# yangao07/LAMSA

Hardware: AMD Instinct MI355X
Metric: aligned Gbase/s, 10 kbp ONT-error reads (12%: sub/ins/del 4% each), -T ont2d vs GRCh37-sized stand-in; inputs resident in HBM when the timed region starts (upload excluded: see pcie_inclusive_*) (higher is better)
Workload: dtype int32

## Files before the change

### lamsa_amd/csrc/hp_align_api.hip

```cpp
#include <hip/hip_runtime.h>
#include <algorithm>
#include <atomic>
#include <map>
#include <mutex>
#include <stdlib.h>
#include <string.h>
#include <time.h>
#include "hp_phase.h"
#include "hp_handle.h"
#include "hp_hostprep.h"

using namespace hp;

#ifndef HP_WAVES_PER_SIMD
#define HP_WAVES_PER_SIMD 4
#endif
__global__ __launch_bounds__(64, HP_WAVES_PER_SIMD) void k_align_batch(AlignArgs a)
{
    __shared__ int32_t lds[HP_BOTH_LDS_WORDS];
    const int slot = blockIdx.x;
    for (;;) {
        int u = 0;
        if (wv::leader()) u = atomicAdd(a.counter, 1);
        u = wv::uni(u);
        if (u >= a.n_units) break;
        align_read(a, a.order ? a.order[u] : u, slot, (HP_L int32_t *)lds);
    }
}

#ifndef HP_CHAIN_WAVES_PER_SIMD
#define HP_CHAIN_WAVES_PER_SIMD 4
#endif
#ifndef HP_FILL_WAVES_PER_SIMD
#define HP_FILL_WAVES_PER_SIMD 7
#endif
template <int WORDS, int WPS>
__global__ __launch_bounds__(64, WPS) void k_chain1(const PhaseArgs *ap)
{
    const PhaseArgs &a = *ap;
    constexpr bool ctx_lds = ph_ctx_in_lds(WORDS, WPS);
    __shared__ alignas(16) int32_t lds[WORDS + (ctx_lds ? PH_CTX_BYTES / 4 : 0)];
    ReadCtx &r = *(ctx_lds ? (ReadCtx *)(lds + WORDS) : (ReadCtx *)(a.slab + (size_t)blockIdx.x * a.slab_per_wave));
    for (;;) {
        int u = 0;
        if (wv::leader()) u = atomicAdd(&a.ctl->q_head[0], 1);
        u = wv::uni(u);
        if (u >= a.n_reads) break;
        phase_chain1(a, a.order ? a.order[u] : u, blockIdx.x, (HP_L int32_t *)lds, WORDS, r);
    }
    drain_stamp(a, 0);
}
template <int WORDS, int WPS>
__global__ __launch_bounds__(64, WPS) void k_chain2(const PhaseArgs *ap)
{
    const PhaseArgs &a = *ap;
    constexpr bool ctx_lds = ph_ctx_in_lds(WORDS, WPS);
    __shared__ alignas(16) int32_t lds[WORDS + (ctx_lds ? PH_CTX_BYTES / 4 : 0)];
    ReadCtx &r = *(ctx_lds ? (ReadCtx *)(lds + WORDS) : (ReadCtx *)(a.slab + (size_t)blockIdx.x * a.slab_per_wave));
    for (;;) {
        int u = 0;
        if (wv::leader()) u = atomicAdd(&a.ctl->q_head[2], 1);
        u = wv::uni(u);
        if (u >= a.n_reads) break;
        phase_chain2(a, a.order ? a.order[u] : u, blockIdx.x, (HP_L int32_t *)lds, WORDS, r);
    }
    drain_stamp(a, 2);
}
typedef void (*ChainKernel)(const PhaseArgs *);
struct ChainShape { ChainKernel k1, k2; int lds_words, waves_per_simd; };
static const ChainShape g_chain_shapes[3] = {
    {k_chain1<HP_CHAIN_LDS_WORDS, HP_CHAIN_WAVES_PER_SIMD>, k_chain2<HP_CHAIN_LDS_WORDS, HP_CHAIN_WAVES_PER_SIMD>, HP_CHAIN_LDS_WORDS, HP_CHAIN_WAVES_PER_SIMD},
    {k_chain1<3392, 3>, k_chain2<3392, 3>, 3392, 3},
    {k_chain1<5120, 2>, k_chain2<5120, 2>, 5120, 2},
};
__global__ __launch_bounds__(64, HP_FILL_WAVES_PER_SIMD) void k_fill(const PhaseArgs *ap, int round)
{
    const PhaseArgs &a = *ap;
    __shared__ alignas(16) int32_t lds[HP_LDS_WORDS + PH_CTX_BYTES / 4];
    ReadCtx &r = *(ReadCtx *)(lds + HP_LDS_WORDS);
    int n = 0;
    for (int b = 0; b < PH_NBUCKET; ++b) n += a.ctl->bucket_n[round][b];
    n = wv::uni(n);
    for (;;) {
        int g = 0;
        if (wv::leader()) g = atomicAdd(&a.ctl->q_head[1 + 2 * round], 1);
        g = wv::uni(g);
        if (g >= n) break;
        int b = 0;
        while (b < PH_NBUCKET - 1 && g >= a.ctl->bucket_n[round][b]) { g -= a.ctl->bucket_n[round][b]; ++b; }
        const int u = wv::uni(a.bucket_q[((size_t)round * PH_NBUCKET + b) * a.unit_cap + g]);
        phase_fill(a, round, u, blockIdx.x, (HP_L int32_t *)lds, r);
    }
    drain_stamp(a, 1 + 2 * round);
}
#ifndef HP_FILLDP_WAVES_PER_SIMD
#define HP_FILLDP_WAVES_PER_SIMD 2
#endif
#ifndef HP_LIST_WAVES_PER_SIMD
#define HP_LIST_WAVES_PER_SIMD 4
#endif
__global__ __launch_bounds__(64, HP_LIST_WAVES_PER_SIMD) void k_filllist(const PhaseArgs *ap, int round)
{
    const PhaseArgs &a = *ap;
    __shared__ alignas(16) int32_t lds[PH_CTX_BYTES / 4];
    ReadCtx &r = *(ReadCtx *)lds;
    int n = 0;
    for (int b = 0; b < PH_NBUCKET; ++b) n += a.ctl->bucket_n[round][b];
    n = wv::uni(n);
    for (;;) {
        int g = 0;
        if (wv::leader()) g = atomicAdd(&a.ctl->q_head[5], 1);
        g = wv::uni(g);
        if (g >= n) break;
        int b = 0;
        while (b < PH_NBUCKET - 1 && g >= a.ctl->bucket_n[round][b]) { g -= a.ctl->bucket_n[round][b]; ++b; }
        const int u = wv::uni(a.bucket_q[((size_t)round * PH_NBUCKET + b) * a.unit_cap + g]);
        phase_filllist(a, round, u, blockIdx.x, (HP_L int32_t *)lds, r);
    }
}
__global__ __launch_bounds__(64, 2) void k_filldp_small(const PhaseArgs *ap, int round)
{
    __shared__ int32_t lds[HP_LJ_LDS_WORDS(HP_LJ_QSMALL)];
    const PhaseArgs &a = *ap;
    int n = 0;
    for (int b = 0; b < LJ_NBUCKET; ++b) n += (lj_queue_n(a, round, b) + 63) >> 6;
    n = wv::uni(n);
    for (;;) {
        int g = 0;
        if (wv::leader()) g = atomicAdd(&a.ctl->q_head[6], 1);
        g = wv::uni(g);
        if (g >= n) break;
        int b = 0;
        for (; b < LJ_NBUCKET - 1; ++b) { const int gb = (lj_queue_n(a, round, b) + 63) >> 6; if (g < gb) break; g -= gb; }
        phase_filldp(a, round, b, g * 64, blockIdx.x, (HP_L int32_t *)lds, HP_LJ_QSMALL);
    }
}
__global__ __launch_bounds__(64, HP_WJ_WAVES_PER_SIMD) void k_filldp_wave(const PhaseArgs *ap, int round)
{
    __shared__ int32_t lds[HP_WJ_LDS_WORDS];
    const PhaseArgs &a = *ap;
    int n = 0, n_big = 0;
    for (int b = 0; b < WJ_NBUCKET; ++b) { const int k = wj_queue_n(a, round, b); if (b < WJ_NBIG) n_big += k; else n += k; }
    n = wv::uni(n); n_big = wv::uni(n_big);
    bool own_big = (int)blockIdx.x < a.n_wjb;
    for (;;) {
        int g = 0;
        const bool big = own_big;
        if (wv::leader()) g = atomicAdd(&a.ctl->q_head[big ? 8 : 7], 1);
        g = wv::uni(g);
        if (g >= (big ? n_big : n)) { if (!big) break; own_big = false; continue; }
        phase_wavejob(a, round, g, big, blockIdx.x, (HP_L int32_t *)lds);
    }
}
__global__ __launch_bounds__(64) void k_publish(const PhaseArgs *ap)
{
    const PhaseArgs &a = *ap;
    if (blockIdx.x == 0) publish_diag(a);
    for (;;) {
        int u = 0;
        if (wv::leader()) u = atomicAdd(&a.ctl->q_head[4], 1);
        u = wv::uni(u);
        if (u >= a.n_reads) break;
        phase_publish(a, u);
    }
}

__global__ void k_cig8_expand(const uint8_t *src, int32_t *dst, int64_t n)
{
    for (int64_t i = (int64_t)blockIdx.x * blockDim.x + threadIdx.x; i < n; i += (int64_t)gridDim.x * blockDim.x) { const int b = src[i]; dst[i] = ((b & 63) << 4) | (b >> 6); }
}
__global__ void k_off_widen(const int32_t *src, int64_t *dst, int64_t n)
{
    for (int64_t i = (int64_t)blockIdx.x * blockDim.x + threadIdx.x; i < n; i += (int64_t)gridDim.x * blockDim.x) dst[i] = src[i];
}
#define HP_SCAN_BLOCK 4096
__global__ __launch_bounds__(256) void k_scan_sums(const uint8_t *src, int64_t n, int64_t *sums)
{
    __shared__ int part[256];
    const int64_t b0 = (int64_t)blockIdx.x * HP_SCAN_BLOCK;
    int s = 0;
    for (int i = threadIdx.x; i < HP_SCAN_BLOCK; i += 256) { const int64_t k = b0 + i; s += k < n ? src[k] : 0; }
    part[threadIdx.x] = s;
    __syncthreads();
    for (int st = 128; st > 0; st >>= 1) { if ((int)threadIdx.x < st) part[threadIdx.x] += part[threadIdx.x + st]; __syncthreads(); }
    if (threadIdx.x == 0) sums[blockIdx.x] = part[0];
}
__global__ __launch_bounds__(256) void k_scan_bases(int64_t *sums, int64_t nb)
{
    __shared__ long long tot[256];
    const int64_t per = (nb + 255) / 256, a = (int64_t)threadIdx.x * per, b = a + per < nb ? a + per : nb;
    long long s = 0;
    for (int64_t i = a; i < b; ++i) s += sums[i];
    tot[threadIdx.x] = s;
    __syncthreads();
    if (threadIdx.x == 0) { long long run = 0; for (int t = 0; t < 256; ++t) { const long long v = tot[t]; tot[t] = run; run += v; } }
    __syncthreads();
    long long run = tot[threadIdx.x];
    for (int64_t i = a; i < b; ++i) { const long long v = sums[i]; sums[i] = run; run += v; }
}
__global__ __launch_bounds__(256) void k_scan_apply(const uint8_t *src, int64_t n, const int64_t *bases, int64_t *dst)
{
    __shared__ int part[256];
    const int64_t b0 = (int64_t)blockIdx.x * HP_SCAN_BLOCK + (int64_t)threadIdx.x * 16;
    int v[16], s = 0;
#pragma unroll
    for (int i = 0; i < 16; ++i) { const int64_t k = b0 + i; v[i] = k < n ? src[k] : 0; s += v[i]; }
    part[threadIdx.x] = s;
    __syncthreads();
    if (threadIdx.x == 0) { int run = 0; for (int t = 0; t < 256; ++t) { const int x = part[t]; part[t] = run; run += x; } }
    __syncthreads();
    long long run = bases[blockIdx.x] + part[threadIdx.x];
#pragma unroll
    for (int i = 0; i < 16; ++i) { const int64_t k = b0 + i; if (k < n) dst[k] = run; run += v[i]; }
}

static double now_s() { timespec t; clock_gettime(CLOCK_MONOTONIC, &t); return t.tv_sec + 1e-9 * t.tv_nsec; }
static const bool g_trace = getenv("LAMSA_HP_TRACE") != nullptr;
static const bool g_noshare = getenv("LAMSA_HP_FULL_GRIDS") != nullptr;
static const bool g_nowave = getenv("LAMSA_HP_NO_WAVE_JOBS") != nullptr;
static const bool g_nolane = getenv("LAMSA_HP_NO_LANE_DP") != nullptr;
static const bool g_mono = getenv("LAMSA_HP_ONE_KERNEL") != nullptr;

struct HostBuf {
    void *p = nullptr, *dev = nullptr; size_t cap = 0;
    int ensure(size_t bytes) {
        if (bytes <= cap) return 0;
        if (p) hipHostFree(p);
        p = dev = nullptr; cap = 0;
        size_t want = bytes + bytes / 4 + 256;
        if (hipHostMalloc(&p, want, hipHostMallocMapped) != hipSuccess) { p = nullptr; return -1; }
        if (hipHostGetDevicePointer(&dev, p, 0) != hipSuccess) { hipHostFree(p); p = nullptr; return -1; }
        cap = want;
        return 0;
    }
    void release() { if (p) hipHostFree(p); p = dev = nullptr; cap = 0; }
};

struct OutDev {
    DevBuf buf; HostBuf host; int64_t stream_cap = 0; int n_cap = 0;
    static size_t hdr(int n) { return al256(8 * (size_t)n) + 3 * al256(4 * (size_t)n) + 256 + al256(16 * (size_t)n); }
    int ensure(int n, int64_t cap) { stream_cap = cap; n_cap = n; return buf.ensure(4 * (size_t)cap + 256) || host.ensure(hdr(n) + 256); }
    int64_t *off() const { return (int64_t *)host.dev; }
    int32_t *len(int n) const { return (int32_t *)((char *)host.dev + al256(8 * (size_t)n)); }
    int32_t *st(int n) const { return (int32_t *)((char *)host.dev + al256(8 * (size_t)n) + al256(4 * (size_t)n)); }
    int32_t *tb(int n) const { return (int32_t *)((char *)host.dev + al256(8 * (size_t)n) + 2 * al256(4 * (size_t)n)); }
    unsigned long long *diag(int n) const { return (unsigned long long *)((char *)host.dev + al256(8 * (size_t)n) + 3 * al256(4 * (size_t)n)); }
    const unsigned long long *h_diag(int n) const { return (const unsigned long long *)((const char *)host.p + al256(8 * (size_t)n) + 3 * al256(4 * (size_t)n)); }
    int32_t *work(int n) const { return (int32_t *)((char *)host.dev + al256(8 * (size_t)n) + 3 * al256(4 * (size_t)n) + 256); }
    const int32_t *h_work(int n) const { return (const int32_t *)((const char *)host.p + al256(8 * (size_t)n) + 3 * al256(4 * (size_t)n) + 256); }
    const int64_t *h_off() const { return (const int64_t *)host.p; }
    const int32_t *h_len(int n) const { return (const int32_t *)((const char *)host.p + al256(8 * (size_t)n)); }
    const int32_t *h_st(int n) const { return (const int32_t *)((const char *)host.p + al256(8 * (size_t)n) + al256(4 * (size_t)n)); }
    const int32_t *h_tb(int n) const { return (const int32_t *)((const char *)host.p + al256(8 * (size_t)n) + 2 * al256(4 * (size_t)n)); }
    int32_t *stream(int) const { return (int32_t *)buf.p; }
    void release() { buf.release(); host.release(); }
};

struct Slot {
    DevBuf bin, misc, slab, pers, prof; OutDev out1;
    HostBuf args_host;
    hipEvent_t ep[7] = {nullptr, nullptr, nullptr, nullptr, nullptr, nullptr, nullptr};
    hipStream_t cs = nullptr;
    bool valid = false;
    bool phased = false;
    int32_t n_reads = 0; int64_t n_bases = 0, n_cig = 0, n_hits = 0;
    BatchIn in; const int32_t *d_order = nullptr;
    std::vector<int32_t> order, h_len, h_H; std::vector<uint8_t> h_skip;
    int32_t max_L = 0, max_H = 0;
    int32_t sort_pb = 40, sort_cb = 24;
    hipEvent_t e0 = nullptr, e1 = nullptr;
};

struct AlignState {
    Slot slot[2];
    int fifo[2] = {0, 0}, n_fifo = 0;
    int res_fifo[2] = {0, 0}, n_res = 0;
    DevBuf retry_list;
    OutDev out2;
    HostBuf stream;
    std::vector<int32_t> r_len, r_st, r_tb, r_work; std::vector<int64_t> r_off;
};

static std::map<lamsa_hp_handle *, AlignState *> g_states;
static std::mutex g_states_lock;
static AlignState *state_of(lamsa_hp_handle *h)
{
    std::lock_guard<std::mutex> guard(g_states_lock);
    auto it = g_states.find(h);
    if (it != g_states.end()) return it->second;
    return g_states[h] = new AlignState();
}
extern "C" void lamsa_hp_release_state_(lamsa_hp_handle *h)
{
    AlignState *S = nullptr;
    {
        std::lock_guard<std::mutex> guard(g_states_lock);
        auto it = g_states.find(h);
        if (it == g_states.end()) return;
        S = it->second;
        g_states.erase(it);
    }
    if (h->stream) hipStreamSynchronize(h->stream);
    if (h->stream_b) hipStreamSynchronize(h->stream_b);
    for (Slot &T : S->slot) { T.bin.release(); T.misc.release(); T.slab.release(); T.pers.release(); T.prof.release(); T.args_host.release(); T.out1.release(); for (hipEvent_t e : {T.e0, T.e1, T.ep[0], T.ep[1], T.ep[2], T.ep[3], T.ep[4], T.ep[5], T.ep[6]}) if (e) hipEventDestroy(e); }
    S->retry_list.release(); S->out2.release(); S->stream.release();
    delete S;
}

static int grow(lamsa_hp_handle *h, DevBuf &b, size_t bytes)
{
    if (bytes <= b.cap) return 0;
    if (hipStreamSynchronize(h->stream) != hipSuccess || hipStreamSynchronize(h->stream_b) != hipSuccess) return -1;
    return b.ensure(bytes);
}


static int upload_into(lamsa_hp_handle *h, Slot *S, const lamsa_hp_batch *B)
{
    S->valid = false;
    const double t_0 = now_s();
    const int n = B->n_reads;
    const int64_t n_slots = n ? B->seed_off[n] : 0, n_hits = n_slots ? B->hit_off[n_slots] : 0, n_bases = n ? B->read_off[n] : 0;
    S->h_len.assign((size_t)n, 0); S->h_H.assign((size_t)n, 0); S->h_skip.assign((size_t)n + 1, 0); S->max_L = 0; S->max_H = 0;
    if (n && (B->seed_off[0] != 0 || B->read_off[0] != 0 || (n_slots && B->hit_off[0] != 0))) { h->err = "offsets must start at 0"; return LAMSA_HP_EINVAL; }
    const bool packed_off = B->h_cig_off == nullptr, cig_bytes = B->cig8 != nullptr;
    if (B->n_cig < 0 || (!packed_off && B->n_cig > 0x7fffffffll)) { h->err = "more than 2^31-1 seed CIGAR elements with 32-bit h_cig_off: pass h_cig_off = NULL (CIGARs back to back in hit order) or split the batch"; return LAMSA_HP_EINVAL; }
    if (!cig_bytes && !B->cig && B->n_cig > 0) { h->err = "neither cig nor cig8 given"; return LAMSA_HP_EINVAL; }
    {
        std::atomic<int> bad(0);
        const int64_t sl = h->para.seed_len, ss = h->para.seed_step > 0 ? h->para.seed_step : 1;
        std::atomic<long long> max_pos(0), sum_cig(0);
        hp_parallel_blocks(n, [&](int r0, int r1) {
            long long mp = 0, sc = 0;
            for (int r = r0; r < r1 && !bad.load(std::memory_order_relaxed); ++r) {
                const int64_t L = B->read_off[r + 1] - B->read_off[r], ns = B->seed_off[r + 1] - B->seed_off[r];
                if (L < 0 || L > (1 << 24) || ns < 0) { bad = 1; return; }
                if (ns > HP_MAX_SLOTS) S->h_skip[r] = 1;
                {
                    const int64_t sa = L < sl ? 0 : 1 + (L - sl) / ss;
                    if (B->seed_all[r] != sa || B->last_len[r] != L - sl - (sa - 1) * ss) { bad = 7; return; }
                    if (sa > 32767) S->h_skip[r] = 1;
                }
                int64_t H = 0;
                for (int64_t s = B->seed_off[r]; s < B->seed_off[r + 1]; ++s) {
                    const int64_t m = B->hit_off[s + 1] - B->hit_off[s];
                    if (m < 0 || (m > HP_MAX_HITS_PER_SEED && !S->h_skip[r])) { bad = 2; return; }
                    if (B->seed_id[s] < 1 || B->seed_id[s] > B->seed_all[r] || (s > B->seed_off[r] && B->seed_id[s] <= B->seed_id[s - 1])) { bad = 3; return; }
                    H += m;
                }
                if (H > (1 << 22) && !S->h_skip[r]) { bad = 4; return; }
                for (int64_t i = B->read_off[r]; i < B->read_off[r + 1]; ++i) if (B->read_seq[i] > 4) { bad = 5; return; }
                for (int64_t k = B->hit_off[B->seed_off[r]]; k < B->hit_off[B->seed_off[r + 1]]; ++k) {
                    mp = B->h_pos[k] > mp ? B->h_pos[k] : mp;
                    if (B->h_len_dif[k] < -127 || B->h_len_dif[k] > 127) S->h_skip[r] = 1;
                    if (B->h_chr[k] < 1 || B->h_chr[k] > h->n_seqs || (B->h_strand[k] != 1 && B->h_strand[k] != -1) || B->h_pos[k] < 0 || B->h_pos[k] >= (1ll << 40) ||
                        (!packed_off && (B->h_cig_off[k] < 0 || (int64_t)B->h_cig_off[k] + B->h_cig_n[k] > B->n_cig))) { bad = 6; return; }
                    sc += B->h_cig_n[k];
                }
                S->h_len[r] = (int32_t)L; S->h_H[r] = (int32_t)H;
            }
            long long seen = max_pos.load();
            while (mp > seen && !max_pos.compare_exchange_weak(seen, mp)) { }
            sum_cig += sc;
        });
        static const char *why[] = {"", "read longer than 2^24 bases", "too many hits in one seed", "seed ids must be ascending in [1, seed_all]",
                                    "too many hits in one read", "read base code > 4",
                                    "bad hit record (contig id, strand, position or seed CIGAR range)",
                                    "seed_all / last_len do not match the read length and the handle's seed length and step"};
        if (bad) { h->err = why[bad.load()]; return LAMSA_HP_EINVAL; }
        if (packed_off && sum_cig.load() != B->n_cig) { h->err = "h_cig_off is NULL but the h_cig_n do not add up to n_cig"; return LAMSA_HP_EINVAL; }
        for (int r = 0; r < n; ++r) { if (S->h_skip[r]) { S->h_len[r] = 0; S->h_H[r] = 0; } S->max_L = std::max(S->max_L, S->h_len[r]); S->max_H = std::max(S->max_H, S->h_H[r]); }
        auto bits = [](unsigned long long x) { int b = 0; while (x) { ++b; x >>= 1; } return b; };
        S->sort_pb = bits((unsigned long long)max_pos.load()); S->sort_cb = bits((unsigned long long)(2 * (long long)h->n_seqs + 1));
    }
    const double t_1 = now_s();
    S->order.resize((size_t)n);
    for (int r = 0; r < n; ++r) S->order[r] = r;
    {
        std::vector<double> cost((size_t)n);
        for (int r = 0; r < n; ++r) cost[r] = (double)S->h_H[r] * S->h_H[r] / 64.0 + (double)S->h_len[r] * (2.0 * h->para.band_w + 1) / 16.0;
        std::stable_sort(S->order.begin(), S->order.end(), [&](int x, int y) { return cost[x] > cost[y]; });
    }
    size_t off = 0;
    auto place = [&](size_t bytes) { size_t o = off; off = al256(off + bytes + 16); return o; };
    const size_t o_roff = place(8 * ((size_t)n + 1)), o_rseq = place((size_t)n_bases), o_sall = place(4 * (size_t)n), o_last = place(4 * (size_t)n),
                 o_soff = place(8 * ((size_t)n + 1)), o_sid = place(4 * (size_t)n_slots), o_hoff = place(8 * ((size_t)n_slots + 1)),
                 o_pos = place(8 * (size_t)n_hits), o_chr = place(4 * (size_t)n_hits), o_coff = place(8 * (size_t)n_hits), o_nm = place(2 * (size_t)n_hits),
                 o_ld = place(2 * (size_t)n_hits), o_st = place((size_t)n_hits), o_cn = place((size_t)n_hits), o_cig = place(4 * (size_t)B->n_cig), o_ord = place(4 * (size_t)n),
                 o_stage = place(packed_off ? 8 * ((size_t)n_hits / HP_SCAN_BLOCK + 2) : 4 * (size_t)n_hits), o_cig8 = place(cig_bytes ? (size_t)B->n_cig : 0), o_skip = place((size_t)n);
    const double t_3 = now_s();
    if (S->bin.ensure(off)) { h->err = "hipMalloc(batch)"; return LAMSA_HP_ENOMEM; }
    char *d = (char *)S->bin.p;
    hipStream_t s = h->copy_stream;
    static const int64_t zero64 = 0;
#define UP(o, src, bytes) do { if ((bytes) > 0) HIPCHK(h, hipMemcpyAsync(d + (o), (src), (bytes), hipMemcpyHostToDevice, s), LAMSA_HP_EKERNEL); } while (0)
    if (n) { UP(o_roff, B->read_off, 8 * ((size_t)n + 1)); UP(o_soff, B->seed_off, 8 * ((size_t)n + 1)); }
    else { UP(o_roff, &zero64, 8); UP(o_soff, &zero64, 8); }
    UP(o_rseq, B->read_seq, (size_t)n_bases); UP(o_sall, B->seed_all, 4 * (size_t)n); UP(o_last, B->last_len, 4 * (size_t)n);
    UP(o_sid, B->seed_id, 4 * (size_t)n_slots);
    if (n_slots) UP(o_hoff, B->hit_off, 8 * ((size_t)n_slots + 1)); else UP(o_hoff, &zero64, 8);
    UP(o_pos, B->h_pos, 8 * (size_t)n_hits); UP(o_chr, B->h_chr, 4 * (size_t)n_hits);
    if (!packed_off) UP(o_stage, B->h_cig_off, 4 * (size_t)n_hits);
    UP(o_nm, B->h_nm, 2 * (size_t)n_hits); UP(o_ld, B->h_len_dif, 2 * (size_t)n_hits); UP(o_st, B->h_strand, (size_t)n_hits); UP(o_cn, B->h_cig_n, (size_t)n_hits);
    if (cig_bytes) UP(o_cig8, B->cig8, (size_t)B->n_cig); else UP(o_cig, B->cig, 4 * (size_t)B->n_cig);
    UP(o_ord, S->order.data(), 4 * (size_t)n); UP(o_skip, S->h_skip.data(), (size_t)n);
#undef UP
    if (cig_bytes && B->n_cig > 0) hipLaunchKernelGGL(k_cig8_expand, dim3(2048), dim3(256), 0, s, (const uint8_t *)(d + o_cig8), (int32_t *)(d + o_cig), (int64_t)B->n_cig);
    if (n_hits > 0) {
        if (!packed_off) hipLaunchKernelGGL(k_off_widen, dim3(2048), dim3(256), 0, s, (const int32_t *)(d + o_stage), (int64_t *)(d + o_coff), (int64_t)n_hits);
        else {
            const int64_t nb = (n_hits + HP_SCAN_BLOCK - 1) / HP_SCAN_BLOCK;
            hipLaunchKernelGGL(k_scan_sums, dim3((unsigned)nb), dim3(256), 0, s, (const uint8_t *)(d + o_cn), (int64_t)n_hits, (int64_t *)(d + o_stage));
            hipLaunchKernelGGL(k_scan_bases, dim3(1), dim3(256), 0, s, (int64_t *)(d + o_stage), nb);
            hipLaunchKernelGGL(k_scan_apply, dim3((unsigned)nb), dim3(256), 0, s, (const uint8_t *)(d + o_cn), (int64_t)n_hits, (const int64_t *)(d + o_stage), (int64_t *)(d + o_coff));
        }
    }
    HIPCHK(h, hipGetLastError(), LAMSA_HP_EKERNEL);
    HIPCHK(h, hipStreamSynchronize(s), LAMSA_HP_EKERNEL);
    if (g_trace) fprintf(stderr, "[lamsa_hp] upload: validate %.1f ms, order %.1f ms, copy %.1f ms (%.2f GB on the device)\n", 1e3 * (t_1 - t_0), 1e3 * (t_3 - t_1), 1e3 * (now_s() - t_3), off / 1e9);
    BatchIn &in = S->in;
    in.n_reads = n; in.read_skip = (const uint8_t *)(d + o_skip); in.read_off = (const int64_t *)(d + o_roff); in.read_seq = (const uint8_t *)(d + o_rseq);
    in.seed_all = (const int32_t *)(d + o_sall); in.last_len = (const int32_t *)(d + o_last); in.seed_off = (const int64_t *)(d + o_soff);
    in.seed_id = (const int32_t *)(d + o_sid); in.hit_off = (const int64_t *)(d + o_hoff); in.h_pos = (const int64_t *)(d + o_pos);
    in.h_chr = (const int32_t *)(d + o_chr); in.h_cig_off = (const int64_t *)(d + o_coff); in.h_nm = (const int16_t *)(d + o_nm);
    in.h_len_dif = (const int16_t *)(d + o_ld); in.h_strand = (const int8_t *)(d + o_st); in.h_cig_n = (const uint8_t *)(d + o_cn);
    in.cig = (const int32_t *)(d + o_cig);
    S->d_order = (const int32_t *)(d + o_ord);
    S->n_reads = n; S->n_bases = n_bases; S->n_cig = B->n_cig; S->n_hits = n_hits;
    S->valid = true;
    return LAMSA_HP_OK;
}

static int cap_waves(int n_waves, size_t slab_per_wave, int n_cu)
{
    static const size_t budget = []() { size_t f = 0, t = 0; if (hipMemGetInfo(&f, &t) != hipSuccess || t == 0) { t = (size_t)288 << 30; f = t; } return std::min(t / 4, f / 3); }();
    if (slab_per_wave * (size_t)n_waves <= budget) return n_waves;
    size_t fit = budget / (slab_per_wave ? slab_per_wave : 1);
    if (n_cu > 0 && fit >= (size_t)n_cu) fit -= fit % (size_t)n_cu;
    return fit < 1 ? 1 : (int)fit;
}

#ifdef HP_PROF
static void prof_report(Slot &T, const long long *d_prof, int n)
{
    if (!d_prof) return;
    {
        std::vector<long long> pr((size_t)n * 64);
        hipMemcpy(pr.data(), d_prof, sizeof(long long) * pr.size(), hipMemcpyDeviceToHost);
        if (const char *dump = getenv("LAMSA_HP_PROF_DUMP")) {
            if (FILE *fp = fopen(dump, "wb")) {
                for (int r = 0; r < n; ++r) { long long hl[2] = {T.h_H[r], T.h_len[r]}; fwrite(hl, 8, 2, fp); fwrite(&pr[(size_t)r * 64], 8, 64, fp); }
                fclose(fp);
            }
        }
        std::vector<int> idx((size_t)n); for (int i = 0; i < n; ++i) idx[i] = i;
        auto tot = [&](int r) { long long t = 0; for (int k = 0; k < 6; ++k) t += pr[(size_t)r * 64 + k]; return t; };
        std::sort(idx.begin(), idx.end(), [&](int x, int y) { return tot(x) > tot(y); });
        long long sum[64] = {0}; for (int r = 0; r < n; ++r) for (int k = 0; k < 64; ++k) sum[k] += pr[(size_t)r * 64 + k];
        fprintf(stderr, "[HP_PROF] cycles: setup chain1 fill1 chain2 fill2 publish | in chain1: init+minext mainscan track pop-loop bound+flines | o_l H\n");
        fprintf(stderr, "[HP_PROF] SUM  "); for (int k = 0; k < 11; ++k) fprintf(stderr, " %lld", sum[k] / 1000000); fprintf(stderr, " (Mcycles) targets %lld trips %lld init_Mcyc %lld\n", sum[11], sum[12], sum[13] / 1000000);
#ifdef HP_PROF_TRACK
        fprintf(stderr, "[HP_PROF] branch tracking (-DHP_PROF_TRACK: the line_build stamps below are off): marking pass, image build and write-back %lld Mcyc; %lld seeds visited; %lld tracks, %lld Mcyc in them, %lld steps up; "
                        "%lld arrivals at a node with several sons, %lld Mcyc in cut_branch\n", sum[16] / 1000000, sum[19], sum[18], sum[17] / 1000000, sum[20], sum[21], sum[22] / 1000000);
#endif
#ifdef HP_PROF_EDGE
        fprintf(stderr, "[HP_PROF] main pass (-DHP_PROF_EDGE: the line_build stamps below are off), Mcyc: dp_cluster_lds load+pack %lld, MIN extension %lld, target loop %lld, write-back %lld; cluster_lane %lld; build_sons %lld\n",
                sum[16] / 1000000, sum[17] / 1000000, sum[18] / 1000000, sum[19] / 1000000, sum[20] / 1000000, sum[21] / 1000000);
#else
        fprintf(stderr, "[HP_PROF] line_build: %lld lines (%lld without a gap), %lld anchors, %lld gaps | Mcyc: anchor walk %lld, gap list %lld, gaps in lanes %lld, gaps one by one %lld, assembly %lld\n",
                sum[21], sum[22], sum[12], sum[23], sum[16] / 1000000, sum[17] / 1000000, sum[18] / 1000000, sum[19] / 1000000, sum[20] / 1000000);
#endif
        fprintf(stderr, "[HP_PROF] gaps: %lld in lines with fewer than HP_GAP_MIN gaps (%lld lines with gaps); lane gaps: %lld hits scanned, %lld refused (range too long or too many active hits)\n", sum[54], sum[55], sum[11], sum[13]);
        { const char *nm[] = {"ksw_global", "ksw_extend", "backtrack", "ref_fetch", "head_fix", "frag_extend", "split_mapping", "tail_fix", "res_split", "res_aux", "mini_line_regs", "sort index"};
          for (int k = 0; k < 12; ++k) fprintf(stderr, "[HP_PROF] %-16s %8lld Mcyc %10lld calls\n", nm[k], sum[24 + 2 * k] / 1000000, sum[25 + 2 * k]);
#ifdef HP_PROF_FILL
          fprintf(stderr, "[HP_PROF] in frags_merge: boundary repair (merge_cigar_full) %lld Mcyc %lld calls; junctions through split_mapping %lld Mcyc %lld calls; fragments of several seeds %lld Mcyc %lld calls; 64-step gathers %lld Mcyc %lld\n", sum[16] / 1000000, sum[17], sum[18] / 1000000, sum[19], sum[20] / 1000000, sum[21], sum[22] / 1000000, sum[23]);
#endif
          fprintf(stderr, "[HP_PROF] direction-matrix bytes in HBM %lld (%lld jobs); hits passed through nodes_per_init %lld (%lld calls)\n", sum[52], sum[53], sum[54], sum[55]);
          fprintf(stderr, "[HP_PROF] chain_first start: seed loop %lld, node_set loop %lld, min_extend %lld Mcyc (%lld reads with a MIN pass)\n", sum[56] / 1000000, sum[57] / 1000000, sum[58] / 1000000, sum[59]);
          fprintf(stderr, "[HP_PROF] query <= 62: ksw_extend %lld Mcyc %lld calls, ksw_global %lld Mcyc %lld calls\n", sum[60] / 1000000, sum[61], sum[62] / 1000000, sum[63]);
          const char *bn[] = {"[bi_extend total]", "[bi_extend after left ext]", "17-32", "33-64", "65-128", "129-256", "257-512", ">512"};
          for (int k = 0; k < 2; ++k) fprintf(stderr, "[HP_PROF] ksw_extend qlen %-8s %8lld Mcyc %10lld calls\n", bn[k], sum[48 + 2 * k] / 1000000, sum[49 + 2 * k]); }
        {
            std::vector<long long> pd((size_t)n * 64);
            hipMemcpy(pd.data(), d_prof + ((size_t)n + 1) * 64, sizeof(long long) * pd.size(), hipMemcpyDeviceToHost);
            long long sd[64] = {0}; for (int r = 0; r < n; ++r) for (int k = 0; k < 64; ++k) sd[k] += pd[(size_t)r * 64 + k];
            const char *cn[] = {"one set, q <= 62", "packed, one set", "packed, two sets", "band 1 set slides", "band 2 sets slides", "band 4 sets slides", "int32 sets", "LDS / HBM rows",
                                "band 1 set fixed", "band 2 sets fixed", "band 4 sets fixed"};
            for (int c = 0; c < 11; ++c) fprintf(stderr, "[HP_PROF] wave jobs, ksw_extend %-18s %8lld Mcyc %10lld Mcells %9lld calls %10lld rows\n", cn[c], sd[4 * c] / 1000000, sd[4 * c + 1] / 1000000, sd[4 * c + 2], sd[4 * c + 3]);
            fprintf(stderr, "[HP_PROF] wave jobs, junctions of the class 'band 2 sets fixed': %lld jobs, wj_run %lld Mcyc of which staging %lld; ksw_bi_extend %lld Mcyc of which after the left extension %lld; "
                            "in ksw_extend_band<2>: setup and first fill %lld, rows %lld, backtrack %lld Mcyc\n",
                    sd[51], sd[50] / 1000000, sd[49] / 1000000, sd[47] / 1000000, sd[48] / 1000000, sd[44] / 1000000, sd[45] / 1000000, sd[46] / 1000000);
        }
        for (int q = 0; q < 8 && q < n; ++q) { int r = idx[q]; fprintf(stderr, "[HP_PROF] read %d L=%d:", r, T.h_len[r]); for (int k = 0; k < 11; ++k) fprintf(stderr, " %lld", pr[(size_t)r * 64 + k] / 1000000); fprintf(stderr, " | o_l %lld H %lld | targets %lld trips %lld init_Mcyc %lld\n", pr[(size_t)r * 64 + 14], pr[(size_t)r * 64 + 15], pr[(size_t)r * 64 + 11], pr[(size_t)r * 64 + 12], pr[(size_t)r * 64 + 13] / 1000000); }
    }
}
#endif

struct PhasedLayout { size_t bytes, o[15]; int unit_cap, lj_cap, wj_cap; int64_t fl_cap, line_cap, job_cap; };
static PhasedLayout phased_layout(int n, int64_t n_hits, int64_t n_bases, int64_t stream_cap)
{
    PhasedLayout Y;
    const size_t n_ent = (size_t)n_hits + (size_t)n + 1;
    Y.unit_cap = 8 * n + 1024;
    Y.fl_cap = 4 * n_hits + 2304 * (int64_t)n + 4096; Y.line_cap = stream_cap + 64 * (int64_t)Y.unit_cap;
    Y.job_cap = std::min<int64_t>(0x7fffff00ll, 4096 + 256 * (int64_t)n + 2 * n_bases);
    Y.lj_cap = (int)std::min<int64_t>(0x3fffffffll, 1024 + 16 * (int64_t)n + n_bases / 100);
    Y.wj_cap = (int)std::min<int64_t>(0x3fffffffll, 1024 + 32 * (int64_t)n + n_bases / 200);
    size_t off = 0;
    auto place = [&](size_t bytes) { size_t o = off; off = al256(off + bytes + 16); return o; };
    const size_t sz[15] = {sizeof(PhaseArgs), sizeof(PhaseCtl), sizeof(RdMeta) * ((size_t)n + 1), sizeof(NodeS) * n_ent, 4 * n_ent, 8 * n_ent, sizeof(UnitRec) * 2 * (size_t)Y.unit_cap,
                           4 * 2 * (size_t)PH_NBUCKET * Y.unit_cap, 4 * (size_t)Y.fl_cap, 4 * (size_t)Y.line_cap, 4 * (size_t)Y.job_cap, sizeof(LjRec) * (size_t)Y.lj_cap, 4 * (size_t)LJ_NBUCKET * Y.lj_cap,
                           sizeof(WjRec) * (size_t)Y.wj_cap, 4 * (size_t)WJ_NBUCKET * Y.wj_cap};
    for (int k = 0; k < 15; ++k) Y.o[k] = place(sz[k]);
    Y.bytes = off;
    return Y;
}

struct SlabPlan { size_t chain, fill, wj, wjb, wjb_off; int w_chain, w_fill, w_dp, w_wj, n_wjb, shape; size_t bytes; };
static int chain_shape(const lamsa_hp_para &P, int64_t n_reads, int64_t n_bases)
{
    static const int force = getenv("LAMSA_HP_CHAIN_SHAPE") ? atoi(getenv("LAMSA_HP_CHAIN_SHAPE")) : -1;
    if (force >= 0 && force < 3) return force;
    const int64_t mean_L = n_reads > 0 ? n_bases / n_reads : 0, ss = P.seed_step > 0 ? P.seed_step : 1;
    const int64_t est = mean_L / ss * 2 / 3;
    for (int k = 0; k < 2; ++k) if (est <= g_chain_shapes[k].lds_words / 5) return k;
    return 2;
}
static SlabPlan slab_plan(lamsa_hp_handle *h, int max_L, int max_H, bool shared = false, int shape = 0)
{
    SlabPlan Q;
    Q.shape = shape;
    const lamsa_hp_para &P = h->para;
    Q.chain = al256(((size_t)256 << 10) + 128 * (size_t)max_L + 424 * (size_t)max_H);
    Q.fill = al256(fill_slab_bytes(max_L, h->result_tags, sizeof(cig_t) * 3 * HP_LJ_CIG * 64 + (size_t)HP_LJ_QSMALL * HP_LJ_TSMALL * 64 + 64));
    { static const int kb = getenv("LAMSA_HP_WJ_SLAB_KB") ? atoi(getenv("LAMSA_HP_WJ_SLAB_KB")) : 0;
      Q.wj = ((size_t)(kb > 0 ? kb : 1024) << 10) + 33 * 256; }
    Q.wjb = al256((size_t)wj_need(&P, WJ_HEAD, max_L, max_L + 2 * P.hash_step + 64) + ((size_t)64 << 10)) + 33 * 256;
    if (Q.wjb < Q.wj) Q.wjb = Q.wj;
    if (g_nowave) Q.fill = std::max(Q.fill, al256(read_slab_bytes(P.band_w, max_L, max_H, 1, h->result_tags)));
    if (h->scratch_limit) { const size_t lim = al256(h->scratch_limit); Q.chain = std::min(Q.chain, lim); Q.fill = std::min(Q.fill, lim); Q.wj = std::min(Q.wj, lim); Q.wjb = std::min(Q.wjb, lim); }
    int pc = 0, pf = 0, pd = 0, pw = 0;
    if (hipOccupancyMaxActiveBlocksPerMultiprocessor(&pc, g_chain_shapes[shape].k1, 64, 0) != hipSuccess || pc < 1) pc = 4 * g_chain_shapes[shape].waves_per_simd;
    if (hipOccupancyMaxActiveBlocksPerMultiprocessor(&pf, k_fill, 64, 0) != hipSuccess || pf < 1) pf = 4;
    if (hipOccupancyMaxActiveBlocksPerMultiprocessor(&pd, k_filldp_small, 64, 0) != hipSuccess || pd < 1) pd = 4;
    if (hipOccupancyMaxActiveBlocksPerMultiprocessor(&pw, k_filldp_wave, 64, 0) != hipSuccess || pw < 1) pw = 4;
    if (shared && !g_noshare) { pc = std::min(pc, 8); pf = std::min(pf, 16); pw = std::min(pw, 16); }
    { static const int cf = getenv("LAMSA_HP_FILL_PER_CU") ? atoi(getenv("LAMSA_HP_FILL_PER_CU")) : 0, cc = getenv("LAMSA_HP_CHAIN_PER_CU") ? atoi(getenv("LAMSA_HP_CHAIN_PER_CU")) : 0,
                       cw = getenv("LAMSA_HP_WJ_PER_CU") ? atoi(getenv("LAMSA_HP_WJ_PER_CU")) : 0;
      if (cf > 0 && cf < pf) pf = cf;
      if (cc > 0 && cc < pc) pc = cc;
      if (cw > 0 && cw < pw) pw = cw; }
    Q.w_chain = cap_waves(h->n_cu * pc, Q.chain, h->n_cu); Q.w_fill = cap_waves(h->n_cu * pf, Q.fill, h->n_cu);
    Q.w_dp = std::min(h->n_cu * pd, Q.w_fill); Q.w_wj = cap_waves(h->n_cu * pw, Q.wj, h->n_cu);
    { const size_t budget_big = (size_t)12 << 30; size_t nb = budget_big / Q.wjb; if (nb < 1) nb = 1; Q.n_wjb = (int)std::min<size_t>(nb, (size_t)Q.w_wj); }
    Q.wjb_off = al256(Q.wj * (size_t)Q.w_wj);
    const size_t wj_bytes = Q.wjb_off + Q.wjb * (size_t)Q.n_wjb;
    Q.bytes = std::max(std::max(Q.chain * (size_t)Q.w_chain, Q.fill * (size_t)Q.w_fill), wj_bytes);
    return Q;
}

static int launch_phased(lamsa_hp_handle *h, AlignState *S, Slot &T, Slot &Ln, OutDev &O, hipEvent_t e0, hipEvent_t e1)
{
    const int n = T.n_reads;
    const int64_t n_hits = T.n_hits;
    const SlabPlan Q = slab_plan(h, T.max_L, T.max_H, S->n_fifo + S->n_res > 0, chain_shape(h->para, T.n_reads, T.n_bases));
    const int w_chain = Q.w_chain, w_fill = Q.w_fill, w_dp = Q.w_dp, w_wj = Q.w_wj;
    const PhasedLayout Y = phased_layout(n, n_hits, T.n_bases, O.stream_cap);
    const int unit_cap = Y.unit_cap, lj_cap = Y.lj_cap; const int64_t fl_cap = Y.fl_cap, line_cap = Y.line_cap, job_cap = Y.job_cap;
    const size_t off = Y.bytes, o_args = Y.o[0], o_ctl = Y.o[1], o_meta = Y.o[2], o_nd = Y.o[3], o_ns = Y.o[4], o_sx = Y.o[5], o_un = Y.o[6], o_bq = Y.o[7], o_fl = Y.o[8], o_ln = Y.o[9],
                 o_jb = Y.o[10], o_lj = Y.o[11], o_lq = Y.o[12], o_wj = Y.o[13], o_wq = Y.o[14];
    if (grow(h, Ln.slab, Q.bytes) || grow(h, Ln.pers, off) || Ln.misc.ensure(256)) { h->err = "hipMalloc(slab)"; return LAMSA_HP_ENOMEM; }
    char *d = (char *)Ln.pers.p;
    PhaseArgs a;
    a.P = h->para;
    a.ref.pac = h->d_pac; a.ref.l_pac = h->l_pac; a.ref.n_seqs = h->n_seqs; a.ref.seq_off = h->d_seq_off; a.ref.seq_len = h->d_seq_len;
    a.in = T.in; a.in.tags = h->result_tags;
    a.out.read_out_off = O.off(); a.out.read_out_len = O.len(n); a.out.read_status = O.st(n); a.out.read_tbases = O.tb(n); a.out.read_work = O.work(n); a.out.stream = O.stream(n);
    a.out.stream_cap = O.stream_cap; a.out.cursor = (unsigned long long *)((char *)Ln.misc.p + 64); a.out.diag = O.diag(n);
    a.slab = (char *)Ln.slab.p; a.slab_per_wave = Q.chain; a.slab_fill = Q.fill; a.slab_wj = Q.wj; a.slab_wjb = Q.wjb; a.wjb_off = Q.wjb_off; a.n_wjb = Q.n_wjb; a.sort_pb = T.sort_pb; a.sort_cb = T.sort_cb;
    a.order = T.d_order; a.n_reads = n; a.prof = nullptr;
#ifdef HP_PROF
    if (Ln.prof.ensure(sizeof(long long) * 64 * 2 * ((size_t)n + 1))) { h->err = "hipMalloc(prof)"; return LAMSA_HP_ENOMEM; }
    a.prof = (long long *)Ln.prof.p;
    HIPCHK(h, hipMemsetAsync(Ln.prof.p, 0, sizeof(long long) * 64 * 2 * ((size_t)n + 1), Ln.cs), LAMSA_HP_EKERNEL);
#endif
    a.g_nd = (NodeS *)(d + o_nd); a.g_nseed = (int32_t *)(d + o_ns); a.g_sidx = (int32_t *)(d + o_sx); a.meta = (RdMeta *)(d + o_meta);
    a.units = (UnitRec *)(d + o_un); a.unit_cap = unit_cap; a.bucket_q = (int32_t *)(d + o_bq);
    a.fl_base = (int32_t *)(d + o_fl); a.fl_cap = fl_cap; a.line_base = (int32_t *)(d + o_ln); a.line_cap = line_cap; a.ctl = (PhaseCtl *)(d + o_ctl);
    a.job_base = (int32_t *)(d + o_jb); a.job_cap = job_cap;
    a.ljobs = (LjRec *)(d + o_lj); a.lj_bucket = (int32_t *)(d + o_lq); a.lj_cap = g_nolane ? 0 : lj_cap;
    a.wjobs = (WjRec *)(d + o_wj); a.wj_bucket = (int32_t *)(d + o_wq); a.wj_cap = g_nowave ? 0 : Y.wj_cap;
    const bool list = !g_nolane || !g_nowave;
    hipStream_t s = Ln.cs;
    HIPCHK(h, hipMemsetAsync(Ln.misc.p, 0, 128, s), LAMSA_HP_EKERNEL);
    HIPCHK(h, hipMemsetAsync(d + o_ctl, 0, (o_meta - o_ctl) + sizeof(RdMeta) * ((size_t)n + 1), s), LAMSA_HP_EKERNEL);
    if (Ln.args_host.ensure(sizeof a)) { h->err = "hipHostMalloc(args)"; return LAMSA_HP_ENOMEM; }
    memcpy(Ln.args_host.p, &a, sizeof a);
    HIPCHK(h, hipMemcpyAsync(d + o_args, Ln.args_host.p, sizeof a, hipMemcpyHostToDevice, s), LAMSA_HP_EKERNEL);
    const PhaseArgs *da = (const PhaseArgs *)(d + o_args);
    HIPCHK(h, hipEventRecord(e0, s), LAMSA_HP_EKERNEL);
    hipLaunchKernelGGL(g_chain_shapes[Q.shape].k1, dim3(std::min(w_chain, n)), dim3(64), 0, s, da);
    HIPCHK(h, hipEventRecord(Ln.ep[0], s), LAMSA_HP_EKERNEL);
    if (list) {
        hipLaunchKernelGGL(k_filllist, dim3(w_fill), dim3(64), 0, s, da, 0);
        HIPCHK(h, hipEventRecord(Ln.ep[5], s), LAMSA_HP_EKERNEL);
        if (!g_nowave) hipLaunchKernelGGL(k_filldp_wave, dim3(w_wj), dim3(64), 0, s, da, 0);
        HIPCHK(h, hipEventRecord(Ln.ep[6], s), LAMSA_HP_EKERNEL);
        if (!g_nolane) hipLaunchKernelGGL(k_filldp_small, dim3(w_dp), dim3(64), 0, s, da, 0);
    } else { HIPCHK(h, hipEventRecord(Ln.ep[5], s), LAMSA_HP_EKERNEL); HIPCHK(h, hipEventRecord(Ln.ep[6], s), LAMSA_HP_EKERNEL); }
    HIPCHK(h, hipEventRecord(Ln.ep[4], s), LAMSA_HP_EKERNEL);
    hipLaunchKernelGGL(k_fill, dim3(w_fill), dim3(64), 0, s, da, 0);
    HIPCHK(h, hipEventRecord(Ln.ep[1], s), LAMSA_HP_EKERNEL);
    hipLaunchKernelGGL(g_chain_shapes[Q.shape].k2, dim3(std::min(w_chain, n)), dim3(64), 0, s, da);
    HIPCHK(h, hipEventRecord(Ln.ep[2], s), LAMSA_HP_EKERNEL);
    if (list) {
        HIPCHK(h, hipMemsetAsync(&((PhaseCtl *)(d + o_ctl))->q_head[5], 0, 16, s), LAMSA_HP_EKERNEL);
        hipLaunchKernelGGL(k_filllist, dim3(w_fill), dim3(64), 0, s, da, 1);
        if (!g_nowave) hipLaunchKernelGGL(k_filldp_wave, dim3(w_wj), dim3(64), 0, s, da, 1);
        if (!g_nolane) hipLaunchKernelGGL(k_filldp_small, dim3(w_dp), dim3(64), 0, s, da, 1);
    }
    hipLaunchKernelGGL(k_fill, dim3(w_fill), dim3(64), 0, s, da, 1);
    HIPCHK(h, hipEventRecord(Ln.ep[3], s), LAMSA_HP_EKERNEL);
    hipLaunchKernelGGL(k_publish, dim3(std::min(h->n_cu * 8, n)), dim3(64), 0, s, da);
    HIPCHK(h, hipGetLastError(), LAMSA_HP_EKERNEL);
    HIPCHK(h, hipEventRecord(e1, s), LAMSA_HP_EKERNEL);
    Ln.phased = true;
    return LAMSA_HP_OK;
}

static int launch_align(lamsa_hp_handle *h, AlignState *S, Slot &T, Slot &Ln, OutDev &O, const int32_t *d_order, int n_units, int scale, int max_L, int max_H,
                        hipEvent_t e0, hipEvent_t e1, bool wait)
{
    size_t slab_per_wave = al256(read_slab_bytes(h->para.band_w, max_L, max_H, scale, h->result_tags));
    if (scale == 1 && h->scratch_limit && slab_per_wave > h->scratch_limit) slab_per_wave = al256(h->scratch_limit);
    int per_cu = 0;
    if (hipOccupancyMaxActiveBlocksPerMultiprocessor(&per_cu, k_align_batch, 64, 0) != hipSuccess || per_cu < 1) per_cu = 4;
    int n_waves = h->n_cu * per_cu;
    if (n_waves > n_units) n_waves = n_units;
    n_waves = cap_waves(n_waves, slab_per_wave, h->n_cu);
    if (grow(h, Ln.slab, slab_per_wave * (size_t)n_waves) || Ln.misc.ensure(256)) { h->err = "hipMalloc(slab)"; return LAMSA_HP_ENOMEM; }
    const int n = T.n_reads;
    AlignArgs a;
    a.P = h->para;
    a.ref.pac = h->d_pac; a.ref.l_pac = h->l_pac; a.ref.n_seqs = h->n_seqs; a.ref.seq_off = h->d_seq_off; a.ref.seq_len = h->d_seq_len;
    a.in = T.in; a.in.tags = h->result_tags;
    a.out.read_out_off = O.off(); a.out.read_out_len = O.len(n); a.out.read_status = O.st(n); a.out.read_tbases = O.tb(n); a.out.read_work = O.work(n); a.out.stream = O.stream(n);
    a.out.stream_cap = O.stream_cap; a.out.cursor = (unsigned long long *)((char *)Ln.misc.p + 64); a.out.diag = nullptr;
    a.slab = (char *)Ln.slab.p; a.slab_per_wave = slab_per_wave; a.counter = (int32_t *)Ln.misc.p;
    a.order = d_order; a.n_units = n_units; a.scale = scale; a.prof = nullptr; a.sort_pb = T.sort_pb; a.sort_cb = T.sort_cb;
    hipStream_t s = Ln.cs;
    HIPCHK(h, hipMemsetAsync(Ln.misc.p, 0, 128, s), LAMSA_HP_EKERNEL);
    HIPCHK(h, hipEventRecord(e0, s), LAMSA_HP_EKERNEL);
    hipLaunchKernelGGL(k_align_batch, dim3(n_waves), dim3(64), 0, s, a);
    HIPCHK(h, hipGetLastError(), LAMSA_HP_EKERNEL);
    HIPCHK(h, hipEventRecord(e1, s), LAMSA_HP_EKERNEL);
    if (wait) HIPCHK(h, hipStreamSynchronize(s), LAMSA_HP_EKERNEL);
#ifdef HP_PROF
    prof_report(T, a.prof, n);
#endif
    return LAMSA_HP_OK;
}

static int slot_events(lamsa_hp_handle *h, Slot &Ln)
{
    Ln.cs = &Ln == &state_of(h)->slot[1] ? h->stream_b : h->stream;
    if (!Ln.e0) HIPCHK(h, hipEventCreate(&Ln.e0), LAMSA_HP_EKERNEL);
    if (!Ln.e1) HIPCHK(h, hipEventCreate(&Ln.e1), LAMSA_HP_EKERNEL);
    for (hipEvent_t &e : Ln.ep) if (!e) HIPCHK(h, hipEventCreate(&e), LAMSA_HP_EKERNEL);
    return LAMSA_HP_OK;
}

static int start_main(lamsa_hp_handle *h, AlignState *S, Slot &T, Slot &Ln)
{
    int rc = slot_events(h, Ln);
    if (rc) return rc;
    const int n = T.n_reads;
    if (n == 0) return LAMSA_HP_OK;
    if (Ln.out1.ensure(n, batch_out_cap(n, T.n_bases, h->result_tags))) { h->err = "hipMalloc(out)"; return LAMSA_HP_ENOMEM; }
    Ln.phased = false;
    if (!g_mono) return launch_phased(h, S, T, Ln, Ln.out1, Ln.e0, Ln.e1);
    return launch_align(h, S, T, Ln, Ln.out1, T.d_order, n, 1, T.max_L, T.max_H, Ln.e0, Ln.e1, false);
}

#define DL(dst, src, bytes) HIPCHK(h, hipMemcpyAsync((dst), (src), (bytes), hipMemcpyDeviceToHost, h->copy_stream), LAMSA_HP_EKERNEL)
#define DLSYNC() HIPCHK(h, hipStreamSynchronize(h->copy_stream), LAMSA_HP_EKERNEL)

static int finish_main(lamsa_hp_handle *h, AlignState *S, Slot &T, Slot &Ln, lamsa_hp_result *R)
{
    const int n = T.n_reads;
    for (float &v : h->kernel_ms) v = 0;
    S->r_st.assign((size_t)n + 1, 0); S->r_off.assign((size_t)n + 1, 0); S->r_len.assign((size_t)n + 1, 0); S->r_tb.assign((size_t)n + 1, 0); S->r_work.assign(4 * (size_t)n + 4, 0);
    if (S->stream.ensure(64)) { h->err = "hipHostMalloc(results)"; return LAMSA_HP_ENOMEM; }
    if (n == 0) {
        if (R) { R->stream = (const int32_t *)S->stream.p; R->stream_words = 0; R->read_off = S->r_off.data(); R->read_len = S->r_len.data(); R->read_status = S->r_st.data(); R->read_tbases = S->r_tb.data(); R->read_work = S->r_work.data(); }
        return LAMSA_HP_OK;
    }
    const double t_0 = now_s();
    HIPCHK(h, hipEventSynchronize(Ln.e1), LAMSA_HP_EKERNEL);
    const double t_1 = now_s();
    hipEventElapsedTime(&h->kernel_ms[0], Ln.e0, Ln.e1);
    if (Ln.phased) {
        hipEvent_t ev[6] = {Ln.e0, Ln.ep[0], Ln.ep[1], Ln.ep[2], Ln.ep[3], Ln.e1};
        for (int k = 0; k < 5; ++k) hipEventElapsedTime(&h->kernel_ms[2 + k], ev[k], ev[k + 1]);
        const unsigned long long *dg = Ln.out1.h_diag(n);
        for (int k = 0; k < 4; ++k) h->kernel_ms[7 + k] = dg[2 * k + 1] >= dg[2 * k] && dg[2 * k + 1] ? (float)((double)(dg[2 * k + 1] - dg[2 * k]) * 1e-5) : 0.f;
        h->kernel_ms[11] = (float)dg[8]; h->kernel_ms[12] = (float)dg[9];
        hipEventElapsedTime(&h->kernel_ms[13], Ln.ep[0], Ln.ep[4]);
        hipEventElapsedTime(&h->kernel_ms[14], Ln.ep[0], Ln.ep[5]);
        hipEventElapsedTime(&h->kernel_ms[15], Ln.ep[5], Ln.ep[6]);
        h->kernel_ms[16] = (float)dg[12]; h->kernel_ms[17] = (float)((double)dg[13] * 1e-6); h->kernel_ms[18] = (float)dg[14]; h->kernel_ms[19] = (float)((double)dg[15] * 4e-6); h->kernel_ms[20] = (float)((double)dg[16] * 1e-6);
#ifdef HP_PROF
        prof_report(T, (const long long *)Ln.prof.p, n);
#endif
    }
    memcpy(S->r_off.data(), Ln.out1.h_off(), 8 * (size_t)n); memcpy(S->r_len.data(), Ln.out1.h_len(n), 4 * (size_t)n);
    memcpy(S->r_st.data(), Ln.out1.h_st(n), 4 * (size_t)n); memcpy(S->r_tb.data(), Ln.out1.h_tb(n), 4 * (size_t)n); memcpy(S->r_work.data(), Ln.out1.h_work(n), 16 * (size_t)n);
    unsigned long long used1 = 0;
    for (int r = 0; r < n; ++r) if (S->r_off[r] >= 0 && (unsigned long long)(S->r_off[r] + S->r_len[r]) > used1) used1 = (unsigned long long)(S->r_off[r] + S->r_len[r]);
    if ((int64_t)used1 > Ln.out1.stream_cap) used1 = (unsigned long long)Ln.out1.stream_cap;
    std::vector<int32_t> again;
    for (int r = 0; r < n; ++r) if ((S->r_st[r] & LAMSA_HP_ST_OVERFLOW) || S->r_off[r] < 0) again.push_back(r);
#ifdef HP_CHAIN_STOP
    again.clear();
#endif
    unsigned long long used2 = 0;
    if (!again.empty()) {
        int mL = 0, mH = 0; int64_t cap2 = 1024;
        for (int r : again) { mL = std::max(mL, T.h_len[r]); mH = std::max(mH, T.h_H[r]); cap2 += read_out_cap(T.h_len[r], 8, h->result_tags); }
        if (grow(h, S->out2.buf, 4 * (size_t)cap2 + 256) || S->out2.host.ensure(OutDev::hdr(n) + 256) || grow(h, S->retry_list, 4 * again.size())) { h->err = "hipMalloc(retry)"; return LAMSA_HP_ENOMEM; }
        S->out2.stream_cap = cap2;
        HIPCHK(h, hipMemcpyAsync(S->retry_list.p, again.data(), 4 * again.size(), hipMemcpyHostToDevice, Ln.cs), LAMSA_HP_EKERNEL);
        int rc = launch_align(h, S, T, Ln, S->out2, (const int32_t *)S->retry_list.p, (int)again.size(), 8, mL, mH, h->ev0, h->ev1, true);
        if (rc) return rc;
        hipEventElapsedTime(&h->kernel_ms[1], h->ev0, h->ev1);
        const int64_t *off2 = S->out2.h_off(); const int32_t *len2 = S->out2.h_len(n), *st2 = S->out2.h_st(n), *tb2 = S->out2.h_tb(n), *wk2 = S->out2.h_work(n);
        for (int r : again) if (off2[r] >= 0 && (unsigned long long)(off2[r] + len2[r]) > used2) used2 = (unsigned long long)(off2[r] + len2[r]);
        if ((int64_t)used2 > cap2) used2 = (unsigned long long)cap2;
        for (int r : again) { S->r_st[r] = st2[r]; S->r_len[r] = len2[r]; S->r_tb[r] = tb2[r]; for (int q = 0; q < 4; ++q) S->r_work[4 * r + q] = wk2[4 * r + q]; S->r_off[r] = off2[r] < 0 ? -1 : (int64_t)used1 + off2[r]; }
    }
    for (int r = 0; r < n; ++r) if (S->r_off[r] < 0) { S->r_off[r] = 0; S->r_len[r] = 0; S->r_st[r] |= LAMSA_HP_ST_OVERFLOW; }
    if (!R) return LAMSA_HP_OK;
    if (S->stream.ensure(4 * (size_t)(used1 + used2) + 64)) { h->err = "hipHostMalloc(results)"; return LAMSA_HP_ENOMEM; }
    int32_t *hs = (int32_t *)S->stream.p;
    if (used1) DL(hs, Ln.out1.stream(n), 4 * (size_t)used1);
    if (used2) DL(hs + used1, S->out2.stream(n), 4 * (size_t)used2);
    DLSYNC();
    if (g_trace) fprintf(stderr, "[lamsa_hp] collect: waited %.1f ms for the kernel (%.1f ms), results %.1f ms (%.2f GB)\n", 1e3 * (t_1 - t_0), h->kernel_ms[0], 1e3 * (now_s() - t_1), 4e-9 * (double)(used1 + used2));
    R->stream = hs; R->stream_words = (int64_t)(used1 + used2); R->read_off = S->r_off.data(); R->read_len = S->r_len.data(); R->read_status = S->r_st.data(); R->read_tbases = S->r_tb.data(); R->read_work = S->r_work.data();
    return LAMSA_HP_OK;
}
#undef DL
#undef DLSYNC

static int check_batch_args(lamsa_hp_handle *h, const lamsa_hp_batch *B)
{
    if (!h || !B || B->n_reads < 0) return LAMSA_HP_EINVAL;
    if (!h->d_pac) { h->err = "handle was created without a reference"; return LAMSA_HP_EINVAL; }
    HIPCHK(h, hipSetDevice(h->device), LAMSA_HP_ENODEV);
    return LAMSA_HP_OK;
}

extern "C" int lamsa_hp_upload_batch(lamsa_hp_handle *h, const lamsa_hp_batch *B)
{
    int rc = check_batch_args(h, B);
    if (rc) return rc;
    AlignState *S = state_of(h);
    if (S->n_fifo || S->n_res) { h->err = "batches are in flight: collect them first"; return LAMSA_HP_EINVAL; }
    return upload_into(h, &S->slot[0], B);
}

extern "C" int lamsa_hp_run_uploaded(lamsa_hp_handle *h, lamsa_hp_result *R)
{
    if (!h) return LAMSA_HP_EINVAL;
    AlignState *S = state_of(h);
    if (S->n_fifo) { h->err = "submitted batches are in flight: collect them first"; return LAMSA_HP_EINVAL; }
    if (!S->slot[0].valid) { h->err = "no batch uploaded"; return LAMSA_HP_EINVAL; }
    HIPCHK(h, hipSetDevice(h->device), LAMSA_HP_ENODEV);
    if (S->n_res) { h->err = "runs of the resident batch are in flight: finish them first"; return LAMSA_HP_EINVAL; }
    int rc = start_main(h, S, S->slot[0], S->slot[0]);
    if (rc) return rc;
    return finish_main(h, S, S->slot[0], S->slot[0], R);
}

extern "C" int lamsa_hp_start_uploaded(lamsa_hp_handle *h)
{
    if (!h) return LAMSA_HP_EINVAL;
    AlignState *S = state_of(h);
    if (S->n_fifo) { h->err = "submitted batches are in flight: collect them first"; return LAMSA_HP_EINVAL; }
    if (!S->slot[0].valid) { h->err = "no batch uploaded"; return LAMSA_HP_EINVAL; }
    if (S->n_res >= 2) { h->err = "two runs are already in flight: finish one first"; return LAMSA_HP_EINVAL; }
    HIPCHK(h, hipSetDevice(h->device), LAMSA_HP_ENODEV);
    const int k = S->n_res == 1 ? 1 - S->res_fifo[0] : 0;
    S->slot[1].valid = false;
    const int rc = start_main(h, S, S->slot[0], S->slot[k]);
    if (rc) return rc;
    S->res_fifo[S->n_res++] = k;
    return LAMSA_HP_OK;
}

extern "C" int lamsa_hp_finish_uploaded(lamsa_hp_handle *h, lamsa_hp_result *R)
{
    if (!h) return LAMSA_HP_EINVAL;
    AlignState *S = state_of(h);
    if (S->n_res == 0) { h->err = "no run in flight"; return LAMSA_HP_EINVAL; }
    HIPCHK(h, hipSetDevice(h->device), LAMSA_HP_ENODEV);
    const int k = S->res_fifo[0];
    S->res_fifo[0] = S->res_fifo[1]; --S->n_res;
    return finish_main(h, S, S->slot[0], S->slot[k], R);
}

extern "C" int lamsa_hp_align_batch(lamsa_hp_handle *h, const lamsa_hp_batch *B, lamsa_hp_result *R)
{
    int rc = lamsa_hp_upload_batch(h, B);
    if (rc) return rc;
    return lamsa_hp_run_uploaded(h, R);
}

extern "C" int lamsa_hp_submit_batch(lamsa_hp_handle *h, const lamsa_hp_batch *B)
{
    int rc = check_batch_args(h, B);
    if (rc) return rc;
    AlignState *S = state_of(h);
    if (S->n_res) { h->err = "runs of the resident batch are in flight: finish them first"; return LAMSA_HP_EINVAL; }
    if (S->n_fifo >= 2) { h->err = "two batches are already in flight: collect one first"; return LAMSA_HP_EINVAL; }
    const int k = S->n_fifo == 1 ? 1 - S->fifo[0] : 0;
    rc = upload_into(h, &S->slot[k], B);
    if (rc) return rc;
    const double t_s = now_s();
    rc = start_main(h, S, S->slot[k], S->slot[k]);
    if (g_trace) fprintf(stderr, "[lamsa_hp] submit: launch queued in %.1f ms (scratch and output buffers are allocated on first use)\n", 1e3 * (now_s() - t_s));
    if (rc) { S->slot[k].valid = false; return rc; }
    S->fifo[S->n_fifo++] = k;
    return LAMSA_HP_OK;
}

extern "C" int lamsa_hp_collect_batch(lamsa_hp_handle *h, lamsa_hp_result *R)
{
    if (!h) return LAMSA_HP_EINVAL;
    AlignState *S = state_of(h);
    if (S->n_fifo == 0) { h->err = "no batch in flight"; return LAMSA_HP_EINVAL; }
    HIPCHK(h, hipSetDevice(h->device), LAMSA_HP_ENODEV);
    const int k = S->fifo[0];
    S->fifo[0] = S->fifo[1]; --S->n_fifo;
    const int rc = finish_main(h, S, S->slot[k], S->slot[k], R);
    S->slot[k].valid = false;
    return rc;
}

extern "C" void *lamsa_hp_host_alloc(size_t bytes)
{
    void *p = nullptr;
    if (hipHostMalloc(&p, bytes ? bytes : 1, hipHostMallocDefault) != hipSuccess) return nullptr;
    return p;
}
extern "C" void lamsa_hp_host_free(void *p) { if (p) hipHostFree(p); }

extern "C" int lamsa_hp_reserve(lamsa_hp_handle *h, int32_t n_reads, int64_t n_bases, int64_t n_hits, int64_t n_cig, int32_t max_read_len, int32_t max_hits_per_read)
{
    if (!h || n_reads < 0 || n_bases < 0 || n_hits < 0 || n_cig < 0) return LAMSA_HP_EINVAL;
    HIPCHK(h, hipSetDevice(h->device), LAMSA_HP_ENODEV);
    AlignState *S = state_of(h);
    if (S->n_fifo || S->n_res) { h->err = "batches are in flight"; return LAMSA_HP_EINVAL; }
    const SlabPlan Q = slab_plan(h, max_read_len, max_hits_per_read, false, chain_shape(h->para, n_reads, n_bases));
    const int64_t cap = batch_out_cap(n_reads, n_bases, h->result_tags);
    const PhasedLayout Y = phased_layout(n_reads, n_hits, n_bases, cap);
    const size_t in_bytes = (size_t)n_bases + 16 * (size_t)n_reads * 4 + 32 * ((size_t)n_hits + n_reads) + 8 * (size_t)n_hits + 5 * (size_t)n_cig + 64 * 256 + 4096;
    for (Slot &T : S->slot) {
        int rc = slot_events(h, T);
        if (rc) return rc;
        if (T.slab.ensure(Q.bytes) || T.pers.ensure(Y.bytes) || T.misc.ensure(256) || T.bin.ensure(in_bytes) || T.out1.ensure(n_reads, cap)) {
            for (Slot &U : S->slot) { U.slab.release(); U.pers.release(); U.bin.release(); U.out1.release(); }
            h->err = "hipMalloc(reserve)"; return LAMSA_HP_ENOMEM;
        }
    }
    return LAMSA_HP_OK;
}

extern "C" int lamsa_hp_set_scratch_limit(lamsa_hp_handle *h, size_t bytes)
{
    if (!h || (bytes && bytes < ((size_t)64 << 10))) return LAMSA_HP_EINVAL;
    h->scratch_limit = bytes;
    return LAMSA_HP_OK;
}

extern "C" int lamsa_hp_set_result_tags(lamsa_hp_handle *h, int flags)
{
    if (!h) return LAMSA_HP_EINVAL;
    if (!result_tags_valid(flags)) { h->err = "result tags: an unknown item, or LAMSA_HP_TAG_SUMMARY (no CIGAR is shipped) with an item that lists or splits"; return LAMSA_HP_EINVAL; }
    AlignState *S = state_of(h);
    if (S->n_fifo || S->n_res) { h->err = "batches are in flight: collect them first"; return LAMSA_HP_EINVAL; }
    h->result_tags = flags;
    return LAMSA_HP_OK;
}
```

### lamsa_amd/csrc/hp_api.hip

```cpp
#include <hip/hip_runtime.h>
#include <stdio.h>
#include <stdlib.h>
#include <string.h>
#include <math.h>
#include <vector>
#include <string>
#include "hp_dp_batch.h"
#include "hp_wavejob.h"

using namespace hp;

__global__ __launch_bounds__(64) void k_dp_batch(DpBatchArgs a)
{
    __shared__ int32_t lds[HP_LDS_WORDS];
    const int slot = blockIdx.x;
    for (;;) {
        int job = 0;
        if (wv::leader()) job = atomicAdd(a.counter, 1);
        job = wv::uni(job);
        if (job >= a.n_jobs) break;
        dp_run_job(a, job, slot, (HP_L int32_t *)lds);
    }
}

__global__ __launch_bounds__(64, 1) void k_dp_batch_lane(DpBatchArgs a, const uint8_t *pac, const int64_t *tk)
{
    __shared__ int32_t lds[HP_LJ_LDS_WORDS(HP_LJ_QCAP)];
    const lamsa_hp_para *P = &a.P;
    char *slab = a.slab + (size_t)blockIdx.x * a.slab_per_wave;
    cig_t *cbuf = (cig_t *)slab;
    uint8_t *zbuf = (uint8_t *)(slab + sizeof(cig_t) * 3 * HP_LJ_CIG * 64);
    for (;;) {
        int g = 0;
        if (wv::leader()) g = atomicAdd(a.counter, 1);
        g = wv::uni(g);
        if (g * 64 >= a.n_jobs) break;
        wv::sync();
        WAVE_FOR(l) {
            const int job = g * 64 + l;
            if (job < a.n_jobs) {
                LaneJob J;
                J.q = (const HP_G uint8_t *)(a.seq + a.q_off[job]); J.qs = 1; J.qcomp = 0; J.qlen = a.qlen[job]; J.pac = (const HP_G uint8_t *)pac; J.tk = tk[job]; J.ts = 1; J.tlen = a.tlen[job];
                J.z = (HP_G uint8_t *)zbuf; J.zl = l; J.zs = HP_LJ_QCAP; J.cells = 0; J.row = (HP_L int32_t *)lds + l; J.qrow = (HP_L uint8_t *)((HP_L int32_t *)lds + (HP_LJ_QCAP + 2) * 64) + l; J.rev = 0;
                lj_stage_query(J);
                LCig out, Lc, Rc;
                out.c = cbuf + (size_t)l * 3 * HP_LJ_CIG; out.n = 0; Lc.c = out.c + HP_LJ_CIG; Lc.n = 0; Rc.c = Lc.c + HP_LJ_CIG; Rc.n = 0;
                int sc = 0, qle = 0, tle = 0;
                const int kind = a.kind[job];
                if (kind == 4) sc = lj_global(P, J, P->del_gapo, P->del_gape, P->ins_gapo, P->ins_gape, a.w[job], &out);
                else if (kind == 5) sc = lj_extend(P, J, a.w[job], a.h0[job], &qle, &tle, &out);
                else sc = lj_bi_extend(P, J, a.h0[job], a.h0[job], Lc, Rc, out);
                a.score[job] = sc; a.qle[job] = qle; a.tle[job] = tle; a.status[job] = 0; a.cig_n[job] = out.n;
                cig_t *dst = a.cig + a.cig_cap_off[job];
                for (int k = 0; k < out.n; ++k) dst[k] = out.c[k];
            }
        }
        wv::sync();
    }
}
__global__ __launch_bounds__(64, HP_WJ_WAVES_PER_SIMD) void k_dp_batch_wave(DpBatchArgs a, const uint8_t *pac, const int64_t *tk)
{
    __shared__ int32_t lds[HP_WJ_LDS_WORDS];
    for (;;) {
        int job = 0;
        if (wv::leader()) job = atomicAdd(a.counter, 1);
        job = wv::uni(job);
        if (job >= a.n_jobs) break;
        Ctx cx;
        cx.P = &a.P; cx.lds = (HP_L int32_t *)lds; cx.lds_words = HP_WJ_LDS_WORDS; cx.status = 0; cx.n_cells = 0; cx.lds_epoch = 0; cx.prof = nullptr;
        arena_init(cx.tmp, a.slab + (size_t)blockIdx.x * a.slab_per_wave, a.slab_per_wave);
        const int type = wv::uni(a.kind[job]) - 7, qlen = wv::uni(a.qlen[job]), tlen = wv::uni(a.tlen[job]);
        const bool back = type == WJ_HEAD;
        CigV out; cig_bind(out, a.cig + a.cig_cap_off[job], (int)(a.cig_cap_off[job + 1] - a.cig_cap_off[job]));
        WjOut o;
        wj_run(cx, a.seq, pac, type, 0, a.q_off[job] + (back && qlen > 0 ? qlen - 1 : 0), back ? -1 : 1, qlen, tk[job] + (back && tlen > 0 ? tlen - 1 : 0), back ? -1 : 1, tlen,
               wv::uni(a.w[job]), wv::uni(a.h0[job]), out, o);
        if (wv::leader()) { a.score[job] = o.score; a.qle[job] = o.qle; a.tle[job] = o.tle; a.status[job] = cx.status; a.cig_n[job] = out.n; }
        wv::sync();
    }
}

#include "hp_handle.h"

#include "hp_para.h"

extern "C" int lamsa_hp_create(lamsa_hp_handle **out, const lamsa_hp_para *para, const lamsa_hp_ref *ref, int device_id)
{
    if (!out || !para) return LAMSA_HP_EINVAL;
    *out = nullptr;
    int n_dev = 0;
    if (hipGetDeviceCount(&n_dev) != hipSuccess || n_dev <= 0 || device_id < 0 || device_id >= n_dev) return LAMSA_HP_ENODEV;
    if (hipSetDevice(device_id) != hipSuccess) return LAMSA_HP_ENODEV;
    lamsa_hp_handle *h = new lamsa_hp_handle();
    h->device = device_id; h->para = *para;
    hipDeviceProp_t prop;
    if (hipGetDeviceProperties(&prop, device_id) == hipSuccess) h->n_cu = prop.multiProcessorCount;
    if (hipStreamCreateWithFlags(&h->stream, hipStreamNonBlocking) != hipSuccess || hipStreamCreateWithFlags(&h->copy_stream, hipStreamNonBlocking) != hipSuccess || hipStreamCreateWithFlags(&h->stream_b, hipStreamNonBlocking) != hipSuccess || hipEventCreate(&h->ev0) != hipSuccess || hipEventCreate(&h->ev1) != hipSuccess) { delete h; return LAMSA_HP_ENODEV; }
    if (ref && ref->pac) {
        size_t pb = (size_t)(ref->l_pac / 4 + 1);
        h->l_pac = ref->l_pac; h->n_seqs = ref->n_seqs;
        if (hipMalloc((void **)&h->d_pac, pb + 16) != hipSuccess ||
            hipMalloc((void **)&h->d_seq_off, sizeof(int64_t) * (size_t)(ref->n_seqs + 1)) != hipSuccess ||
            hipMalloc((void **)&h->d_seq_len, sizeof(int32_t) * (size_t)(ref->n_seqs + 1)) != hipSuccess) { lamsa_hp_destroy(h); return LAMSA_HP_ENOMEM; }
        hipMemcpy(h->d_pac, ref->pac, pb, hipMemcpyHostToDevice);
        hipMemcpy(h->d_seq_off, ref->seq_offset, sizeof(int64_t) * (size_t)ref->n_seqs, hipMemcpyHostToDevice);
        hipMemcpy(h->d_seq_len, ref->seq_len, sizeof(int32_t) * (size_t)ref->n_seqs, hipMemcpyHostToDevice);
    }
    *out = h;
    return LAMSA_HP_OK;
}

extern "C" void lamsa_hp_release_state_(lamsa_hp_handle *h);
extern "C" void lamsa_hp_destroy(lamsa_hp_handle *h)
{
    if (!h) return;
    hipSetDevice(h->device);
    lamsa_hp_release_state_(h);
    if (h->d_pac) hipFree(h->d_pac);
    if (h->d_seq_off) hipFree(h->d_seq_off);
    if (h->d_seq_len) hipFree(h->d_seq_len);
    h->in.release(); h->out.release(); h->slab.release(); h->misc.release(); h->pac2.release();
    if (h->ev0) hipEventDestroy(h->ev0);
    if (h->ev1) hipEventDestroy(h->ev1);
    if (h->stream) hipStreamDestroy(h->stream);
    if (h->copy_stream) hipStreamDestroy(h->copy_stream);
    if (h->stream_b) hipStreamDestroy(h->stream_b);
    delete h;
}

extern "C" const char *lamsa_hp_last_error(const lamsa_hp_handle *h) { return h ? h->err.c_str() : "null handle"; }
extern "C" float lamsa_hp_last_kernel_ms(const lamsa_hp_handle *h, int which) { return (h && which >= 0 && which < 24) ? h->kernel_ms[which] : -1.f; }


extern "C" int lamsa_hp_dp_batch(lamsa_hp_handle *h, const lamsa_hp_dp_jobs *J, lamsa_hp_dp_out *O)
{
    if (!h || !J || !O || J->n_jobs < 0) return LAMSA_HP_EINVAL;
    HIPCHK(h, hipSetDevice(h->device), LAMSA_HP_ENODEV);
    const int n = J->n_jobs;
    std::vector<int64_t> cap_off((size_t)n + 1, 0);
    size_t z_need = 4096;
    for (int i = 0; i < n; ++i) {
        int ql = J->qlen[i], tl = J->tlen[i];
        if (ql < 0) ql = 0;
        if (tl < 0) tl = 0;
        if (J->q_off[i] < 0 || J->t_off[i] < 0 || J->q_off[i] + ql > J->seq_bytes || J->t_off[i] + tl > J->seq_bytes) { h->err = "dp job sequence out of range"; return LAMSA_HP_EINVAL; }
        cap_off[i + 1] = cap_off[i] + ql + tl + (J->kind[i] >= 8 ? 72 : 8);
        size_t wmax = (size_t)(abs(ql - tl) + 3 > (J->kind[i] == 2 ? h->para.band_w : J->w[i]) ? abs(ql - tl) + 3 : (J->kind[i] == 2 ? h->para.band_w : J->w[i]));
        size_t ncol = (size_t)ql < 2 * wmax + 1 ? (size_t)ql : 2 * wmax + 1;
        if (ql <= HP_PK_QMAX(2) && ncol < 128) ncol = 128;
        size_t need = 2 * 4 * ((size_t)ql + 18) + 8 * ((size_t)tl + 17) + ncol * tl + 64 + 3 * 4 * ((size_t)ql + tl + 24) + 1024;
        if (need > z_need) z_need = need;
    }
    int cls = 0;
    std::vector<int32_t> kind_v;
    std::vector<uint8_t> pac; std::vector<int64_t> tkv;
    if (n > 0 && J->kind[0] >= 4) {
        cls = J->kind[0] >= 8 ? 2 : 1;
        for (int i = 0; i < n; ++i) {
            const int k = J->kind[i];
            if (k < 4 || k == 7 || k > 11 || (k >= 8) != (cls == 2)) { h->err = "dp batch mixes job classes"; return LAMSA_HP_EINVAL; }
            if (cls == 1 && (J->qlen[i] < 0 || J->qlen[i] > HP_LJ_QCAP || J->tlen[i] < 0 || J->tlen[i] > HP_LJ_TCAP || (k != 4 && J->h0[i] <= 0))) { h->err = "dp job beyond the lane routines' buffers"; return LAMSA_HP_EINVAL; }
            if (cls == 2 && (J->qlen[i] < 0 || J->tlen[i] < 0 || (k != 9 && J->h0[i] <= 0))) { h->err = "dp job with a negative length or without a start score"; return LAMSA_HP_EINVAL; }
        }
        if (cls == 1 && !lj_params_ok(&h->para)) {
            kind_v.assign(J->kind, J->kind + n);
            for (int i = 0; i < n; ++i) kind_v[i] -= 4;
            cls = 0;
        } else {
            int64_t tot = 0;
            for (int i = 0; i < n; ++i) tot += J->tlen[i];
            pac.assign((size_t)tot / 4 + 16, 0); tkv.assign((size_t)n + 1, 0);
            int64_t k = 0;
            for (int i = 0; i < n; ++i) {
                tkv[i] = k;
                for (int j = 0; j < J->tlen[i]; ++j, ++k) {
                    const uint8_t b = J->seq[J->t_off[i] + j];
                    if (b > 3) { h->err = "these routines read the target 2 bits per base: no N"; return LAMSA_HP_EINVAL; }
                    pac[(size_t)(k >> 2)] |= (uint8_t)(b << ((~k & 3) << 1));
                }
            }
            if (cls == 1) z_need = sizeof(cig_t) * 3 * HP_LJ_CIG * 64 + (size_t)HP_LJ_QCAP * HP_LJ_TCAP * 64 + 64;
        }
    }
    const int32_t *kind_src = kind_v.empty() ? J->kind : kind_v.data();
    size_t slab_per_wave = al256(z_need);
    int n_waves = h->n_cu * (cls == 1 ? 3 : (cls == 2 ? 16 : 8));
    if (cls == 2) {
        size_t zz = 4096;
        for (int i = 0; i < n; ++i) {
            const size_t ql = (size_t)J->qlen[i], tl = (size_t)J->tlen[i];
            const size_t wmax = std::max<size_t>((size_t)abs((int)ql - (int)tl) + 3, (size_t)std::max(J->w[i], h->para.band_w));
            const size_t ncol = std::max<size_t>(std::min(ql, 2 * wmax + 1), 256);
            zz = std::max(zz, 2 * (ql + tl + 64) + 2 * 4 * (ql + 18) + 8 * (tl + 17) + ncol * tl + 64 + 4 * 4 * (ql + tl + 72) + 4096);
        }
        slab_per_wave = al256(zz);
    }
    if (n_waves > n) n_waves = n > 0 ? n : 1;
    while (n_waves > 1 && slab_per_wave * (size_t)n_waves > ((size_t)64 << 30)) n_waves /= 2;

    size_t o_seq = 0, o_qoff = al256((size_t)J->seq_bytes + 16), o_toff = o_qoff + al256(8 * (size_t)n), o_cap = o_toff + al256(8 * (size_t)n),
           o_ql = o_cap + al256(8 * ((size_t)n + 1)), o_tl = o_ql + al256(4 * (size_t)n), o_kind = o_tl + al256(4 * (size_t)n),
           o_w = o_kind + al256(4 * (size_t)n), o_h0 = o_w + al256(4 * (size_t)n), in_bytes = o_h0 + al256(4 * (size_t)n);
    if (h->in.ensure(in_bytes)) { h->err = "hipMalloc(in)"; return LAMSA_HP_ENOMEM; }
    size_t o_score = 0, o_qle = al256(4 * (size_t)n), o_tle = 2 * o_qle, o_st = 3 * o_qle, o_cn = 4 * o_qle, o_cig = 5 * o_qle, out_bytes = o_cig + al256(4 * (size_t)cap_off[n] + 16);
    if (h->out.ensure(out_bytes)) { h->err = "hipMalloc(out)"; return LAMSA_HP_ENOMEM; }
    if (h->slab.ensure(slab_per_wave * (size_t)n_waves)) { h->err = "hipMalloc(slab)"; return LAMSA_HP_ENOMEM; }
    if (h->misc.ensure(256)) { h->err = "hipMalloc(misc)"; return LAMSA_HP_ENOMEM; }
    char *din = (char *)h->in.p, *dout = (char *)h->out.p;
    hipStream_t s = h->stream;
    if (n > 0) {
        HIPCHK(h, hipMemcpyAsync(din + o_seq, J->seq, (size_t)J->seq_bytes, hipMemcpyHostToDevice, s), LAMSA_HP_EKERNEL);
        HIPCHK(h, hipMemcpyAsync(din + o_qoff, J->q_off, 8 * (size_t)n, hipMemcpyHostToDevice, s), LAMSA_HP_EKERNEL);
        HIPCHK(h, hipMemcpyAsync(din + o_toff, J->t_off, 8 * (size_t)n, hipMemcpyHostToDevice, s), LAMSA_HP_EKERNEL);
        HIPCHK(h, hipMemcpyAsync(din + o_cap, cap_off.data(), 8 * ((size_t)n + 1), hipMemcpyHostToDevice, s), LAMSA_HP_EKERNEL);
        HIPCHK(h, hipMemcpyAsync(din + o_ql, J->qlen, 4 * (size_t)n, hipMemcpyHostToDevice, s), LAMSA_HP_EKERNEL);
        HIPCHK(h, hipMemcpyAsync(din + o_tl, J->tlen, 4 * (size_t)n, hipMemcpyHostToDevice, s), LAMSA_HP_EKERNEL);
        HIPCHK(h, hipMemcpyAsync(din + o_kind, kind_src, 4 * (size_t)n, hipMemcpyHostToDevice, s), LAMSA_HP_EKERNEL);
        HIPCHK(h, hipMemcpyAsync(din + o_w, J->w, 4 * (size_t)n, hipMemcpyHostToDevice, s), LAMSA_HP_EKERNEL);
        HIPCHK(h, hipMemcpyAsync(din + o_h0, J->h0, 4 * (size_t)n, hipMemcpyHostToDevice, s), LAMSA_HP_EKERNEL);
    }
    HIPCHK(h, hipMemsetAsync(h->misc.p, 0, 256, s), LAMSA_HP_EKERNEL);

    DpBatchArgs a;
    a.P = h->para; a.n_jobs = n;
    a.seq = (const uint8_t *)(din + o_seq); a.q_off = (const int64_t *)(din + o_qoff); a.t_off = (const int64_t *)(din + o_toff);
    a.qlen = (const int32_t *)(din + o_ql); a.tlen = (const int32_t *)(din + o_tl); a.kind = (const int32_t *)(din + o_kind);
    a.w = (const int32_t *)(din + o_w); a.h0 = (const int32_t *)(din + o_h0);
    a.score = (int32_t *)(dout + o_score); a.qle = (int32_t *)(dout + o_qle); a.tle = (int32_t *)(dout + o_tle);
    a.status = (int32_t *)(dout + o_st); a.cig_n = (int32_t *)(dout + o_cn);
    a.cig_cap_off = (const int64_t *)(din + o_cap); a.cig = (cig_t *)(dout + o_cig);
    a.slab = (char *)h->slab.p; a.slab_per_wave = slab_per_wave; a.counter = (int32_t *)h->misc.p;

    HIPCHK(h, hipEventRecord(h->ev0, s), LAMSA_HP_EKERNEL);
    if (n > 0 && cls == 0) hipLaunchKernelGGL(k_dp_batch, dim3(n_waves), dim3(64), 0, s, a);
    else if (n > 0) {
        const size_t pb = al256(pac.size()), tb = al256(8 * ((size_t)n + 1));
        if (h->pac2.ensure(pb + tb)) { h->err = "hipMalloc(pac)"; return LAMSA_HP_ENOMEM; }
        HIPCHK(h, hipMemcpy(h->pac2.p, pac.data(), pac.size(), hipMemcpyHostToDevice), LAMSA_HP_EKERNEL);
        HIPCHK(h, hipMemcpy((char *)h->pac2.p + pb, tkv.data(), 8 * ((size_t)n + 1), hipMemcpyHostToDevice), LAMSA_HP_EKERNEL);
        if (cls == 1) hipLaunchKernelGGL(k_dp_batch_lane, dim3(n_waves), dim3(64), 0, s, a, (const uint8_t *)h->pac2.p, (const int64_t *)((char *)h->pac2.p + pb));
        else hipLaunchKernelGGL(k_dp_batch_wave, dim3(n_waves), dim3(64), 0, s, a, (const uint8_t *)h->pac2.p, (const int64_t *)((char *)h->pac2.p + pb));
    }
    HIPCHK(h, hipGetLastError(), LAMSA_HP_EKERNEL);
    HIPCHK(h, hipEventRecord(h->ev1, s), LAMSA_HP_EKERNEL);

    h->h_score.assign((size_t)n, 0); h->h_qle.assign((size_t)n, 0); h->h_tle.assign((size_t)n, 0); h->h_status.assign((size_t)n, 0);
    std::vector<int32_t> cn((size_t)n, 0), raw((size_t)cap_off[n] + 4, 0);
    if (n > 0) {
        HIPCHK(h, hipMemcpyAsync(h->h_score.data(), dout + o_score, 4 * (size_t)n, hipMemcpyDeviceToHost, s), LAMSA_HP_EKERNEL);
        HIPCHK(h, hipMemcpyAsync(h->h_qle.data(), dout + o_qle, 4 * (size_t)n, hipMemcpyDeviceToHost, s), LAMSA_HP_EKERNEL);
        HIPCHK(h, hipMemcpyAsync(h->h_tle.data(), dout + o_tle, 4 * (size_t)n, hipMemcpyDeviceToHost, s), LAMSA_HP_EKERNEL);
        HIPCHK(h, hipMemcpyAsync(h->h_status.data(), dout + o_st, 4 * (size_t)n, hipMemcpyDeviceToHost, s), LAMSA_HP_EKERNEL);
        HIPCHK(h, hipMemcpyAsync(cn.data(), dout + o_cn, 4 * (size_t)n, hipMemcpyDeviceToHost, s), LAMSA_HP_EKERNEL);
        HIPCHK(h, hipMemcpyAsync(raw.data(), dout + o_cig, 4 * (size_t)cap_off[n], hipMemcpyDeviceToHost, s), LAMSA_HP_EKERNEL);
    }
    HIPCHK(h, hipStreamSynchronize(s), LAMSA_HP_EKERNEL);
    hipEventElapsedTime(&h->kernel_ms[0], h->ev0, h->ev1);
    h->h_i64.assign((size_t)n + 1, 0);
    h->h_cig.clear();
    for (int i = 0; i < n; ++i) {
        h->h_i64[i] = (int64_t)h->h_cig.size();
        h->h_cig.insert(h->h_cig.end(), raw.begin() + cap_off[i], raw.begin() + cap_off[i] + cn[i]);
    }
    h->h_i64[n] = (int64_t)h->h_cig.size();
    if (h->h_cig.empty()) h->h_cig.push_back(0);
    O->score = h->h_score.data(); O->qle = h->h_qle.data(); O->tle = h->h_tle.data(); O->status = h->h_status.data();
    O->cig_off = h->h_i64.data(); O->cigar = h->h_cig.data();
    return LAMSA_HP_OK;
}
```

### lamsa_amd/csrc/hp_core.h

```cpp
#pragma once
#include <hp/wave.h>
#include "../../include/lamsa_hp.h"

namespace hp {

typedef int32_t cig_t;
enum { C_M = 0, C_I = 1, C_D = 2, C_N = 3, C_S = 4, C_H = 5, C_EQ = 7, C_X = 8 };
enum { ST_OVERFLOW = LAMSA_HP_ST_OVERFLOW, ST_REFEXIT = LAMSA_HP_ST_REFEXIT, ST_UNSUPPORTED = LAMSA_HP_ST_UNSUPPORTED,
       ST_DEAD = ST_OVERFLOW | ST_REFEXIT | ST_UNSUPPORTED };

#define HP_NEG_INF (-0x40000000)

struct Arena {
    char *base; size_t cap, top;
};
HP_INL void arena_init(Arena &a, void *base, size_t cap) { a.base = (char *)base; a.cap = cap; a.top = 0; }
HP_INL size_t arena_mark(const Arena &a) { return a.top; }
HP_INL void arena_release(Arena &a, size_t m) { a.top = m; }

#ifndef HP_LDS_CELLS
#define HP_LDS_CELLS 512
#endif
#ifndef HP_LDS_Z_BYTES
#define HP_LDS_Z_BYTES 512
#endif
#define HP_LDS_WORDS (2 * HP_LDS_CELLS + HP_LDS_CELLS / 4 + HP_LDS_Z_BYTES / 4)
#ifndef HP_CHAIN_LDS_WORDS
#define HP_CHAIN_LDS_WORDS 2432
#endif
#define HP_BOTH_LDS_WORDS (HP_CHAIN_LDS_WORDS > HP_LDS_WORDS ? HP_CHAIN_LDS_WORDS : HP_LDS_WORDS)
#define HP_LANE_STRIP_WORDS HP_CHAIN_LDS_WORDS

struct Ctx {
    const lamsa_hp_para *P;
    HP_L int32_t *lds;
    int lds_words;
    Arena tmp;
    int status;
    long long n_cells;
    long long *prof;
    long long *prof_dp = nullptr;
    int lds_epoch;
};
#if defined(HP_PROF_EDGE) && (defined(HP_PROF_TRACK) || defined(HP_PROF_FILL))
#error "-DHP_PROF_EDGE, -DHP_PROF_TRACK and -DHP_PROF_FILL all use prof slots 16 .. 23: one of them per build"
#endif
#ifdef HP_PROF_FILL
#define HP_PROF_CHAIN_ON 0
#define HP_TADD_FILL(cx, slot, v) HP_TADD(cx, slot, v)
#else
#define HP_PROF_CHAIN_ON 1
#define HP_TADD_FILL(cx, slot, v) do { } while (0)
#endif
#ifdef HP_PROF
#define HP_T0(v) const long long v = wv::clock()
#define HP_TADD(cx, slot, v) do { if ((cx).prof) { (cx).prof[slot] += wv::clock() - (v); (cx).prof[(slot) + 1] += 1; } } while (0)
#else
#define HP_T0(v) do { } while (0)
#define HP_TADD(cx, slot, v) do { } while (0)
#endif

#ifndef HP_DPLOG
#define HP_DPLOG(kind, qlen, tlen, w, cells) do { } while (0)
#endif
#ifndef HP_STAT
#define HP_STAT(i) do { } while (0)
#endif
#ifndef HP_STAT_ADD
#define HP_STAT_ADD(i, n) ((void)0)
#endif
#ifndef HP_STAT_MAX
#define HP_STAT_MAX(i, v) ((void)0)
#endif
#ifdef HP_STAT_SLOTS
static_assert(HP_STAT_SLOTS >= 97, "the array of the path counters ends before the last slot the device sources use");
#define HP_STATX_ADD(i, n) HP_STAT_ADD(i, n)
#define HP_STATX_MAX(i, v) HP_STAT_MAX(i, v)
#else
#define HP_STATX_ADD(i, n) ((void)0)
#define HP_STATX_MAX(i, v) ((void)0)
#endif

HP_INL void *arena_alloc(Ctx &cx, size_t bytes) {
    size_t b = (bytes + 15) & ~(size_t)15;
    if (cx.tmp.top + b > cx.tmp.cap) { cx.status |= ST_OVERFLOW; return nullptr; }
    void *p = cx.tmp.base + cx.tmp.top;
    cx.tmp.top += b;
    return p;
}

struct CigV { cig_t *c; int n, cap; };
HP_INL void cig_bind(CigV &v, cig_t *mem, int cap) { v.c = mem; v.n = 0; v.cap = mem ? cap : 0; }
HP_INL bool cig_alloc(Ctx &cx, CigV &v, int cap) {
    cig_t *m = (cig_t *)arena_alloc(cx, (size_t)cap * sizeof(cig_t));
    cig_bind(v, m, cap);
    return m != nullptr;
}
HP_INL void cig_raw_push(Ctx &cx, CigV &v, cig_t w) {
    if (v.n >= v.cap) { cx.status |= ST_OVERFLOW; return; }
    v.c[v.n++] = w;
}
HP_INL void cig_push0(Ctx &cx, CigV &v, cig_t w) {
    if (v.n > 0 && (v.c[v.n - 1] & 0xf) == (w & 0xf)) { v.c[v.n - 1] += (w >> 4) << 4; return; }
    cig_raw_push(cx, v, w);
}
HP_INL void cig_push1(Ctx &cx, CigV &v, cig_t w) { if ((w >> 4) == 0) return; cig_push0(cx, v, w); }
HP_FN void cig_pushv(Ctx &cx, CigV &v, const cig_t *c, int n) {
    if (n == 0) return;
    const HP_G cig_t *src = (const HP_G cig_t *)c;
    HP_G cig_t *dst = (HP_G cig_t *)v.c;
    const int vn = v.n;
    int j = 0;
    if (vn > 0) {
        const cig_t last = dst[vn - 1], c0 = src[0];
        if ((last & 0xf) == (c0 & 0xf)) { dst[vn - 1] = last + ((c0 >> 4) << 4); j = 1; }
        else if (((last & 0xf) == C_I && (c0 & 0xf) == C_S) || ((last & 0xf) == C_S && (c0 & 0xf) == C_I)) {
            dst[vn - 1] = (((last >> 4) + (c0 >> 4)) << 4) | C_S; j = 1;
        }
    }
    const int m = n - j;
    if (vn + m > v.cap) { cx.status |= ST_OVERFLOW; return; }
    for (int b0 = 0; b0 < m; b0 += 64) { WAVE_FOR(l) { const int i = b0 + l; if (i < m) dst[vn + i] = src[j + i]; } }
    v.n = vn + m;
    wv::sync();
}
HP_FN void cig_pushw(Ctx &cx, CigV &v, cig_t w) {
    if (v.n > 0) {
        const cig_t last = v.c[v.n - 1];
        if ((last & 0xf) == (w & 0xf)) { v.c[v.n - 1] = last + ((w >> 4) << 4); return; }
        if (((last & 0xf) == C_I && (w & 0xf) == C_S) || ((last & 0xf) == C_S && (w & 0xf) == C_I)) { v.c[v.n - 1] = (((last >> 4) + (w >> 4)) << 4) | C_S; return; }
    }
    if (v.n + 1 > v.cap) { cx.status |= ST_OVERFLOW; return; }
    v.c[v.n++] = w;
}
HP_FN void cig_invert(cig_t *c, int n) {
    HP_G cig_t *g = (HP_G cig_t *)c;
    for (int b0 = 0; b0 < n / 2; b0 += 64) {
        WAVE_FOR(l) { const int a = b0 + l; if (a < n / 2) { const cig_t x = g[a], y = g[n - 1 - a]; g[a] = y; g[n - 1 - a] = x; } }
    }
    wv::sync();
}
HP_FN int cig_readlen(const cig_t *c, int n) {
    const HP_G cig_t *g = (const HP_G cig_t *)c;
    int tot = 0;
    for (int b0 = 0; b0 < n; b0 += 64) {
        wv::Lane<int> x;
        WAVE_FOR(l) { const int i = b0 + l; int v = 0; if (i < n) { const cig_t w = g[i]; const int op = w & 0xf; if (op == C_M || op == C_I || op == C_S) v = w >> 4; } x[l] = v; }
        tot += wv::reduce_sum(x);
    }
    return tot;
}
HP_FN int cig_reflen(const cig_t *c, int n) {
    const HP_G cig_t *g = (const HP_G cig_t *)c;
    int tot = 0;
    for (int b0 = 0; b0 < n; b0 += 64) {
        wv::Lane<int> x;
        WAVE_FOR(l) { const int i = b0 + l; int v = 0; if (i < n) { const cig_t w = g[i]; const int op = w & 0xf; if (op == C_M || op == C_D || op == C_H) v = w >> 4; } x[l] = v; }
        tot += wv::reduce_sum(x);
    }
    return tot;
}

struct Seq { const uint8_t *p; int stride; };
HP_INL int seq_at(const Seq &s, int i) { return s.p[(long)i * s.stride]; }
HP_INL Seq seq_fwd(const uint8_t *p) { Seq s; s.p = p; s.stride = 1; return s; }
HP_INL Seq seq_rev(const uint8_t *p, int len) { Seq s; s.p = p + (len > 0 ? len - 1 : 0); s.stride = -1; return s; }

HP_INL int sub_score(const lamsa_hp_para *P, int t, int q) { return (t > 3 || q > 3) ? -1 : (t == q ? P->match : -P->mis); }

HP_INL int iabs(int x) { return x < 0 ? -x : x; }
HP_INL int imin(int a, int b) { return a < b ? a : b; }
HP_INL int imax(int a, int b) { return a > b ? a : b; }

}
```

### lamsa_amd/csrc/hp_lanedp.h

```cpp
#pragma once
#include "hp_fill.h"

namespace hp {

#define HP_LJ_QCAP 160
#define HP_LJ_TCAP 256
#define HP_LJ_QSMALL 64
#define HP_LJ_TSMALL 160
#define HP_LJ_CIG  (HP_LJ_QCAP + HP_LJ_TCAP + 8)
#define HP_LJ_LDS_WORDS(qcap) (((qcap) + 2) * 64 + ((qcap) + 2) * 16)
#define HP_LJ_NEG (-20000)

struct LCig { cig_t *c; int n; };
HP_INL void lc_push0(LCig &v, cig_t w) { if (v.n > 0 && (v.c[v.n - 1] & 0xf) == (w & 0xf)) v.c[v.n - 1] += (w >> 4) << 4; else v.c[v.n++] = w; }
HP_INL void lc_push1(LCig &v, cig_t w) { if ((w >> 4) != 0) lc_push0(v, w); }
HP_INL void lc_pushv(LCig &v, const cig_t *c, int n)
{
    if (n == 0) return;
    int j = 0;
    if (v.n > 0) {
        const cig_t last = v.c[v.n - 1], c0 = c[0];
        if ((last & 0xf) == (c0 & 0xf)) { v.c[v.n - 1] = last + ((c0 >> 4) << 4); j = 1; }
        else if (((last & 0xf) == C_I && (c0 & 0xf) == C_S) || ((last & 0xf) == C_S && (c0 & 0xf) == C_I)) { v.c[v.n - 1] = (((last >> 4) + (c0 >> 4)) << 4) | C_S; j = 1; }
    }
    for (; j < n; ++j) v.c[v.n++] = c[j];
}
HP_INL void lc_invert(LCig &v) { for (int a = 0, b = v.n - 1; a < b; ++a, --b) { const cig_t t = v.c[a]; v.c[a] = v.c[b]; v.c[b] = t; } }

struct LaneJob {
    const HP_G uint8_t *q; int qs, qcomp, qlen;
    const HP_G uint8_t *pac; int64_t tk; int ts, tlen;
    HP_G uint8_t *z; int zl, zs;
    HP_L int32_t *row; HP_L uint8_t *qrow;
    int rev;
    long long cells;
};
HP_INL int lj_qbase(const LaneJob &J, int j) { const int c = J.q[(long)j * J.qs]; return J.qcomp ? (c < 4 ? 3 - c : 4) : c; }
HP_INL int lj_t(const LaneJob &J, int i) { const int64_t k = J.tk + (int64_t)i * J.ts; return J.pac[k >> 2] >> ((~k & 3) << 1) & 3; }
HP_INL void lj_stage_query(LaneJob &J) { for (int j = 0; j < J.qlen; ++j) J.qrow[j * 64] = (uint8_t)lj_qbase(J, j); J.rev = 0; }
HP_INL int lj_q(const LaneJob &J, int j) { return J.qrow[(J.rev ? J.qlen - 1 - j : j) * 64]; }
HP_INL LaneJob lj_rev(const LaneJob &J)
{
    LaneJob R = J;
    R.rev = !J.rev;
    R.tk = J.tk + (int64_t)(J.tlen > 0 ? J.tlen - 1 : 0) * J.ts; R.ts = -J.ts;
    return R;
}
HP_INL int lj_sub(int sc_match, int sc_mis, int t, int q) { const int v = t == q ? sc_match : sc_mis; return q > 3 ? -1 : v; }
HP_INL int lj_pack(int h, int e) { return (int)(((unsigned)e << 16) | ((unsigned)h & 0xffffu)); }
HP_INL int lj_h(int w) { return (int)(short)(w & 0xffff); }
HP_INL int lj_e(int w) { return w >> 16; }

HP_INL void lj_backtrack(const LaneJob &J, int n_col, int w, int i, int k, LCig &out)
{
    int which = 0;
    out.n = 0;
    while (i >= 0 && k >= 0) {
        const int off = i > w ? i - w : 0;
        which = J.z[((size_t)i * J.zs + (k - off)) * 64 + J.zl] >> (which << 1) & 3;
        if (which == 0) { lc_push0(out, 1 << 4 | C_M); --i; --k; }
        else if (which == 1) { lc_push0(out, 1 << 4 | C_D); --i; }
        else { lc_push0(out, 1 << 4 | C_I); --k; }
    }
    if (i >= 0) lc_push0(out, (i + 1) << 4 | C_D);
    if (k >= 0) lc_push0(out, (k + 1) << 4 | C_I);
    lc_invert(out);
}

HP_HD bool lj_params_ok(const lamsa_hp_para *P)
{
    int mx = P->match;
    const int v[] = {P->mis, P->ins_gapo, P->ins_gape, P->del_gapo, P->del_gape, P->ins_ext_o, P->ins_ext_e, P->del_ext_o, P->del_ext_e, 1};
    for (int i = 0; i < 10; ++i) mx = v[i] > mx ? v[i] : mx;
    return mx > 0 && mx * (HP_LJ_QCAP + HP_LJ_TCAP + 8) < 10000 && P->match > 0 && P->mis >= 0;
}

HP_INL int lj_global(const lamsa_hp_para *P, LaneJob &J, int o_del, int e_del, int o_ins, int e_ins, int w, LCig *out)
{
    const int qlen = J.qlen, tlen = J.tlen;
    { const int d = iabs(qlen - tlen) + 3; if (w < d) w = d; }
    const int oe_del = o_del + e_del, oe_ins = o_ins + e_ins;
    const int n_col = qlen < 2 * w + 1 ? qlen : 2 * w + 1;
    const int sc_match = P->match, sc_mis = 0 - P->mis;
    HP_L int32_t *row = J.row;
    int i, j;
    row[0] = lj_pack(0, HP_LJ_NEG);
    for (j = 1; j <= qlen && j <= w; ++j) row[j * 64] = lj_pack(-(o_ins + e_ins * j), HP_LJ_NEG);
    for (; j <= qlen; ++j) row[j * 64] = lj_pack(HP_LJ_NEG, HP_LJ_NEG);
    int t_next = tlen > 0 ? lj_t(J, 0) : 0;
    for (i = 0; i < tlen; ++i) {
        int f = HP_LJ_NEG, h1;
        const int ti = t_next;
        if (i + 1 < tlen) t_next = lj_t(J, i + 1);
        const int beg = i > w ? i - w : 0;
        const int end = i + w + 1 < qlen ? i + w + 1 : qlen;
        h1 = beg == 0 ? -(o_del + e_del * (i + 1)) : HP_LJ_NEG;
        J.cells += end > beg ? end - beg : 0;
        int wj = beg < end ? row[beg * 64] : 0, qj = beg < end ? lj_q(J, beg) : 0;
        for (j = beg; j < end; ++j) {
            const int wn = row[(j + 1) * 64], qn = lj_q(J, j + 1 < qlen ? j + 1 : j);
            int m = lj_h(wj), e = lj_e(wj), h, t, dir;
            m += lj_sub(sc_match, sc_mis, ti, qj);
            dir = m >= e ? 0 : 1; h = m >= e ? m : e;
            dir = h >= f ? dir : 2; h = h >= f ? h : f;
            t = m - oe_del; e -= e_del;
            if (e > t) dir |= 1 << 2; else e = t;
            row[j * 64] = lj_pack(h1, e);
            h1 = h;
            t = m - oe_ins; f -= e_ins;
            if (f > t) dir |= 2 << 4; else f = t;
            if (out) J.z[((size_t)i * J.zs + (j - beg)) * 64 + J.zl] = (uint8_t)dir;
            wj = wn; qj = qn;
        }
        row[end * 64] = lj_pack(h1, HP_LJ_NEG);
    }
    const int score = lj_h(row[qlen * 64]);
    if (out) {
        i = tlen - 1;
        const int k = (i + w + 1 < qlen ? i + w + 1 : qlen) - 1;
        lj_backtrack(J, n_col, w, i, k, *out);
    }
    return score;
}

HP_INL int lj_extend(const lamsa_hp_para *P, LaneJob &J, int w, int h0, int *qle, int *tle, LCig *out)
{
    const int qlen = J.qlen, tlen = J.tlen;
    const int o_ins = P->ins_ext_o, e_ins = P->ins_ext_e, o_del = P->del_ext_o, e_del = P->del_ext_e;
    const int end_bonus = P->end_bonus, zdrop = P->zdrop;
    const int oe_del = o_del + e_del, oe_ins = o_ins + e_ins;
    const int sc_match = P->match, sc_mis = 0 - P->mis;
    int i, j, k, beg, end, max, max_i, max_j, max_ie, gscore;
    HP_L int32_t *row = J.row;
    {
        int hp = h0;
        row[0] = lj_pack(h0, 0);
        for (j = 1; j <= qlen + 1; ++j) {
            int hv = 0;
            if (j == 1) hv = h0 > oe_ins ? h0 - oe_ins : 0;
            else if (j <= qlen && hp > e_ins) hv = hp - e_ins;
            row[j * 64] = lj_pack(hv, 0);
            hp = hv;
        }
    }
    {
        int mx = P->match > 0 ? P->match : 0;
        if (-P->mis > mx) mx = -P->mis;
        int max_ins = (int)((double)(qlen * mx + end_bonus - o_ins) / e_ins + 1.);
        max_ins = max_ins > 1 ? max_ins : 1;
        w = w < max_ins ? w : max_ins;
        int max_del = (int)((double)(qlen * mx + end_bonus - o_del) / e_del + 1.);
        max_del = max_del > 1 ? max_del : 1;
        w = w < max_del ? w : max_del;
    }
    const int n_col = qlen < 2 * w + 1 ? qlen : 2 * w + 1;
    max = h0; max_i = max_j = -1; max_ie = -1; gscore = -1;
    beg = 0; end = qlen;
    int t_next = tlen > 0 ? lj_t(J, 0) : 0;
    for (i = 0; i < tlen; ++i) {
        int t, f = 0, h1, m = 0, mj = -1;
        const int ti = t_next;
        if (i + 1 < tlen) t_next = lj_t(J, i + 1);
        const int d_beg = i > w ? i - w : 0;
        if (beg < i - w) beg = i - w;
        if (end > i + w + 1) end = i + w + 1;
        if (end > qlen) end = qlen;
        if (beg == 0) { h1 = h0 - (o_del + e_del * (i + 1)); if (h1 < 0) h1 = 0; }
        else h1 = 0;
        J.cells += end > beg ? end - beg : 0;
        if (out) {
            const int c_hi = d_beg + n_col;
            for (j = d_beg; j < beg && j < c_hi; ++j) J.z[((size_t)i * J.zs + (j - d_beg)) * 64 + J.zl] = 255;
            for (j = end > d_beg ? end : d_beg; j < c_hi; ++j) J.z[((size_t)i * J.zs + (j - d_beg)) * 64 + J.zl] = 255;
        }
        int wj = beg < end ? row[beg * 64] : 0, qj = beg < end ? lj_q(J, beg) : 0;
        for (j = beg; j < end; ++j) {
            const int wn = row[(j + 1) * 64], qn = lj_q(J, j + 1 < qlen ? j + 1 : j);
            int M = lj_h(wj), e = lj_e(wj), h, dir;
            M = M ? M + lj_sub(sc_match, sc_mis, ti, qj) : 0;
            dir = M > e ? 0 : 1; h = M > e ? M : e;
            dir = h > f ? dir : 2; h = h > f ? h : f;
            mj = m > h ? mj : j;
            m = m > h ? m : h;
            t = M - oe_del; t = t > 0 ? t : 0; e -= e_del;
            if (e > t) dir |= 1 << 2; else e = t;
            row[j * 64] = lj_pack(h1, e);
            h1 = h;
            t = M - oe_ins; t = t > 0 ? t : 0; f -= e_ins;
            if (f > t) dir |= 2 << 4; else f = t;
            if (out) J.z[((size_t)i * J.zs + (j - d_beg)) * 64 + J.zl] = (uint8_t)dir;
            wj = wn; qj = qn;
        }
        row[end * 64] = lj_pack(h1, 0);
        if (j == qlen) {
            max_ie = gscore > h1 ? max_ie : i;
            gscore = gscore > h1 ? gscore : h1;
        }
        if (m == 0) break;
        if (m > max) { max = m; max_i = i; max_j = mj; }
        else if (zdrop > 0) {
            if (i - max_i > mj - max_j) { if (max - m - ((i - max_i) - (mj - max_j)) * e_del > zdrop) break; }
            else { if (max - m - ((mj - max_j) - (i - max_i)) * e_ins > zdrop) break; }
        }
        for (j = beg; j < end && row[j * 64] == 0; ++j) { }
        beg = j;
        for (j = end; j >= beg && row[j * 64] == 0; --j) { }
        end = j + 2 < qlen ? j + 2 : qlen;
    }
    if (gscore <= 0 || gscore <= max - end_bonus) { i = max_i; k = max_j; }
    else { i = max_ie; k = qlen - 1; }
    *qle = k + 1; *tle = i + 1;
    if (out) lj_backtrack(J, n_col, w, i, k, *out);
    return max;
}

HP_INL int lj_bi_extend(const lamsa_hp_para *P, LaneJob &J, int lh0, int rh0, LCig &L, LCig &R, LCig &out)
{
    const int qlen = J.qlen, tlen = J.tlen;
    int res, lqe, lte, rqe, rte;
    out.n = 0; L.n = 0; R.n = 0;
    const int w = iabs(qlen - tlen) + 3 > P->band_w ? iabs(qlen - tlen) + 3 : P->band_w;
    lj_extend(P, J, w, lh0, &lqe, &lte, &L);
    res = lqe == qlen ? 0 : (lte == tlen ? 1 : 2);
    if (res < 2) {
        lc_pushv(out, L.c, L.n);
        lc_push1(out, res == 0 ? ((tlen - lte) << 4) | C_D : ((qlen - lqe) << 4) | C_I);
        return 0;
    }
    if (bi_near_diag(P, qlen, tlen) && ((lqe << 1 > qlen) || (lte << 1 > tlen))) {
        lj_global(P, J, P->del_gapo, P->del_gape, P->ins_gapo, P->ins_gape, P->band_w, &out);
        return 0;
    }
    LaneJob Rj = lj_rev(J);
    lj_extend(P, Rj, w, rh0, &rqe, &rte, &R);
    J.cells = Rj.cells;
    res = rqe == qlen ? 0 : (rte == tlen ? 1 : 2);
    if (res < 2) {
        lc_push1(R, res == 0 ? ((tlen - rte) << 4) | C_D : ((qlen - rqe) << 4) | C_I);
        lc_invert(R);
        lc_pushv(out, R.c, R.n);
        return 0;
    }
    if (bi_near_diag(P, qlen, tlen) && ((rqe << 1 > qlen) || (rte << 1 > tlen))) {
        lj_global(P, J, P->del_gapo, P->del_gape, P->ins_gapo, P->ins_gape, P->band_w, &out);
        return 0;
    }
    lc_invert(R);
    {
        const int Sn = qlen - lqe - rqe, Hn = tlen - lte - rte, half = P->split_len / 2;
        if (iabs(Sn) >= half || iabs(Hn) >= half || iabs(Sn - Hn) >= half) {
            lc_pushv(out, L.c, L.n);
            lc_push0(out, (cig_t)((uint32_t)Sn << 4) | C_S);
            lc_push0(out, (cig_t)((uint32_t)Hn << 4) | C_H);
            lc_pushv(out, R.c, R.n);
        } else {
            LCig g; g.c = L.c; g.n = 0;
            lj_global(P, J, P->del_gapo, P->del_gape, P->ins_gapo, P->ins_gape, P->band_w, &g);
            lc_pushv(out, g.c, g.n);
        }
    }
    return (qlen - lqe - rqe) >= P->split_len ? 1 : 0;
}

}
```

### lamsa_amd/csrc/hp_phase.h

```cpp
#pragma once
#include "hp_align.h"
#include "hp_lanedp.h"
#include "hp_wavejob.h"

namespace hp {

struct RdMeta {
    int64_t fl_off[2];
    int32_t fl_n[2], fl_tot[2], fl_nfrag[2];
    int32_t unit_base[2];
    int32_t status;
    int32_t tbases;
    int32_t cells, pairs;
    int32_t cs_words, pad_;
};

struct UnitRec {
    int32_t read, line;
    int64_t out_off;
    int32_t out_len, n_reg;
    int32_t pad[2];
};

enum { PH_NBUCKET = 8 };

struct alignas(128) PhaseCtl {
    alignas(128) int32_t q_head[12];
    alignas(128) int32_t n_units[2];
    int32_t bucket_n[2][PH_NBUCKET];
    alignas(128) unsigned long long fl_cursor;
    alignas(128) unsigned long long line_cursor;
    alignas(128) unsigned long long job_cursor;
    alignas(128) int32_t lj_n[2]; int32_t lj_bucket_n[2][24];
    alignas(128) int32_t wj_n[2]; int32_t wj_bucket_n[2][WJ_NBUCKET];
    alignas(128) unsigned long long wj_bytes;
    alignas(128) unsigned long long wj_cells;
    alignas(128) unsigned long long t_first_inv[4], t_last[4];
};

struct LjRec;
struct PhaseArgs {
    lamsa_hp_para P;
    RefView ref;
    BatchIn in;
    BatchOut out;
    char *slab; size_t slab_per_wave;
    int32_t sort_pb, sort_cb;
    const int32_t *order;
    int32_t n_reads;
    long long *prof;
    NodeS *g_nd; int32_t *g_nseed; int32_t *g_sidx;
    RdMeta *meta;
    UnitRec *units; int32_t unit_cap;
    int32_t *bucket_q;
    int32_t *fl_base; int64_t fl_cap;
    int32_t *line_base; int64_t line_cap;
    int32_t *job_base; int64_t job_cap;
    struct LjRec *ljobs; int32_t *lj_bucket; int32_t lj_cap;
    WjRec *wjobs; int32_t *wj_bucket; int32_t wj_cap;
    size_t slab_fill, slab_wj;
    size_t slab_wjb, wjb_off; int32_t n_wjb;
    PhaseCtl *ctl;
};

HP_INL void drain_stamp(const PhaseArgs &a, int k)
{
    if (wv::leader()) { const unsigned long long now = wv::wall(); atomicMax(&a.ctl->t_first_inv[k], ~now); atomicMax(&a.ctl->t_last[k], now); }
}

HP_INL void meta_flag(const PhaseArgs &a, int rd, const ReadCtx &r)
{
    if (wv::leader()) {
        const long long tb = r.t_bases, nc = r.cx.n_cells, np = r.n_pairs, cw = r.cs_words;
        if (r.cx.status) atomicOr(&a.meta[rd].status, r.cx.status);
        if (tb > 0) atomicAdd(&a.meta[rd].tbases, (int)(tb > 0x3fffffffLL ? 0x3fffffffLL : tb));
        if (nc > 0) atomicAdd(&a.meta[rd].cells, (int)(nc > 0x3fffffffLL ? 0x3fffffffLL : nc));
        if (np > 0) atomicAdd(&a.meta[rd].pairs, (int)(np > 0x3fffffffLL ? 0x3fffffffLL : np));
        if (cw > 0) atomicAdd(&a.meta[rd].cs_words, (int)(cw > 0x3fffffffLL ? 0x3fffffffLL : cw));
    }
}

HP_FN void units_push(const PhaseArgs &a, ReadCtx &r, int rd, int round, const FLines &F, const FlStore &fs)
{
    RdMeta &M = a.meta[rd];
    int base = 0;
    if (wv::leader()) base = atomicAdd(&a.ctl->n_units[round], F.n);
    base = wv::uni(base);
    if (base + F.n > a.unit_cap) { r.cx.status |= ST_OVERFLOW; return; }
    M.fl_off[round] = fs.got_off; M.fl_n[round] = F.n; M.fl_tot[round] = fs.got_tot; M.fl_nfrag[round] = F.nfrag; M.unit_base[round] = base;
    const lamsa_hp_para *P = r.cx.P;
    const int tiles = (2 * P->band_w + 1 + 63) / 64;
    for (int j = 0; j < F.n; ++j) {
        const int f0 = F.frag_off[j], f1 = F.frag_off[j + 1];
        const int n_seed = F.fr_seed_off[f1] - F.fr_seed_off[f0];
        const int sa = r.seed_id[r.n_seed[F.fr_seed[F.fr_seed_off[f0]]]], sb = r.seed_id[r.n_seed[F.fr_seed[F.fr_seed_off[f1] - 1]]];
        const int s_lo = sa < sb ? sa : sb, s_hi = sa < sb ? sb : sa;
        long long ext = (long long)(s_lo - 1 + r.seed_all - s_hi) * P->seed_step;
        if (ext < 0) ext = 0;
        const long long cost = ext * tiles * 8 + (long long)n_seed * 64;
        int b = 0;
        for (long long c = cost >> 10; c > 0 && b < PH_NBUCKET - 1; c >>= 1) ++b;
        const int bucket = PH_NBUCKET - 1 - b;
        UnitRec &U = a.units[(size_t)round * a.unit_cap + base + j];
        U.read = rd; U.line = j; U.out_off = 0; U.out_len = 0; U.n_reg = 0;
        int at = 0;
        if (wv::leader()) at = atomicAdd(&a.ctl->bucket_n[round][bucket], 1);
        at = wv::uni(at);
        a.bucket_q[((size_t)round * PH_NBUCKET + bucket) * a.unit_cap + at] = base + j;
    }
}

HP_INL void pers_bind(ReadCtx &r, const PhaseArgs &a, int rd)
{
    const int64_t pb = r.hb + rd;
    r.nd = a.g_nd + pb; r.n_seed = a.g_nseed + pb;
    r.srt = a.g_sidx + 2 * pb; r.rnk = a.g_sidx + 2 * pb + (r.H + 1);
}

#ifdef HP_PROF
#define PH_T0() const long long ph_t0_ = wv::clock()
#define PH_TADD(k) do { if (r.prof) r.prof[k] += wv::clock() - ph_t0_; } while (0)
#define PH_TMID(k, v) do { if (r.prof) { const long long now_ = wv::clock(); r.prof[k] += now_ - v; v = now_; } } while (0)
#else
#define PH_T0() do { } while (0)
#define PH_TADD(k) do { } while (0)
#define PH_TMID(k, v) do { } while (0)
#endif

enum { PH_CTX_BYTES = 512 };
static_assert(sizeof(ReadCtx) <= PH_CTX_BYTES, "the read context must fit its per-wave block");
constexpr bool ph_ctx_in_lds(int words, int waves_per_simd)
{
    return 4 * waves_per_simd * (((size_t)words * 4 + PH_CTX_BYTES + 511) / 512 * 512) <= 160 * 1024;
}
static_assert(PH_CTX_BYTES % 512 == 0, "the LDS block of a wave is sized in units of 512 bytes");
static_assert(28 * (4 * HP_LDS_WORDS + PH_CTX_BYTES) <= 160 * 1024, "DP rows + read context of 7 waves per SIMD must fit the CU's LDS");
struct ChainOut { FLines F; FlStore fs; };

HP_NOINL void phase_chain1(const PhaseArgs &a, int rd, int wave_slot, HP_L int32_t *lds, int lds_words, ReadCtx &r)
{
#ifdef HP_PROF
    long long ph_t_ = wv::clock();
#endif
    if (a.in.read_skip && a.in.read_skip[rd]) { if (wv::leader()) atomicOr(&a.meta[rd].status, ST_UNSUPPORTED); return; }
    read_bind(r, a.P, a.ref, a.in, rd, a.slab + (size_t)wave_slot * a.slab_per_wave + PH_CTX_BYTES, a.slab_per_wave - PH_CTX_BYTES, lds, a.prof, lds_words);
    pers_bind(r, a, rd);
    Ctx &cx = r.cx;
    const int H = r.H, c = H + 1;
    ChainOut *co = (ChainOut *)arena_alloc(cx, sizeof(ChainOut));
    int32_t *nm = (int32_t *)arena_alloc(cx, sizeof(int32_t) * 10 * (size_t)c);
    const size_t sort_mark = arena_mark(cx.tmp);
    uint64_t *sort_work = (uint64_t *)arena_alloc(cx, sizeof(uint64_t) * (size_t)c);
    if (co && nm && sort_work) {
        int32_t *sidx = a.g_sidx + 2 * (r.hb + rd);
        { HP_T0(t_sort_);
        sort_read_hits(r.h_pos, r.h_chr, r.h_strand, H, sidx, sidx + c, sort_work, (HP_L uint64_t *)lds, lds_words / 2, a.sort_pb, a.sort_cb);
        HP_TADD(cx, 46, t_sort_); }
        arena_release(cx.tmp, sort_mark);
        aux_bind(r, nm);
        nodes_fill(r);
        PH_TMID(0, ph_t_);
        FLines &F = co->F;
        FlStore &fs = co->fs; fs.base = a.fl_base; fs.cap = a.fl_cap; fs.cursor = &a.ctl->fl_cursor; fs.got_off = 0; fs.got_tot = 0;
#if defined(HP_CHAIN_STOP) && HP_CHAIN_STOP == 0
        const bool ok1 = true; F.n = 0; F.nfrag = 0;
#else
        const bool ok1 = chain_first(r, F, &fs);
#endif
        PH_TMID(1, ph_t_);
        if (ok1 && F.n > 0) units_push(a, r, rd, 0, F, fs);
        else if (!ok1 && !(cx.status & (ST_REFEXIT | ST_OVERFLOW))) cx.status |= ST_OVERFLOW;
    }
    meta_flag(a, rd, r);
}

#ifdef HP_PH_CTX_SHARED
HP_INL ReadCtx &ph_frame_ctx()
{
    alignas(16) static thread_local unsigned char blk[PH_CTX_BYTES];
    static thread_local bool born = false;
    if (!born) { for (int i = 0; i < PH_CTX_BYTES; ++i) blk[i] = 0xa5; born = true; }
    return *reinterpret_cast<ReadCtx *>(blk);
}
#define PH_FRAME_CTX(r) ReadCtx &r = ph_frame_ctx()
#else
#define PH_FRAME_CTX(r) ReadCtx r##_frame_; ReadCtx &r = r##_frame_
#endif
HP_FN void phase_chain1(const PhaseArgs &a, int rd, int wave_slot, HP_L int32_t *lds, int lds_words = HP_CHAIN_LDS_WORDS)
{
    PH_FRAME_CTX(r);
    phase_chain1(a, rd, wave_slot, lds, lds_words, r);
}

struct FillLoc { FLines F; OutBuf o; Regs G; };

HP_NOINL void phase_fill(const PhaseArgs &a, int round, int u, int wave_slot, HP_L int32_t *lds, ReadCtx &r)
{
    UnitRec &U = a.units[(size_t)round * a.unit_cap + u];
    const int rd = U.read, line = U.line;
    RdMeta &M = a.meta[rd];
    if (*(volatile int32_t *)&M.status & ST_DEAD) return;
    PH_T0();
    read_bind(r, a.P, a.ref, a.in, rd, a.slab + (size_t)wave_slot * a.slab_fill, a.slab_fill, lds, a.prof, HP_LDS_WORDS);
    pers_bind(r, a, rd);
    Ctx &cx = r.cx;
    FillLoc *fl = (FillLoc *)arena_alloc(cx, sizeof(FillLoc));
    if (!fl) { meta_flag(a, rd, r); return; }
    FLines &F = fl->F;
    F.n = M.fl_n[round]; F.nfrag = M.fl_nfrag[round];
    flines_bind(F, a.fl_base + M.fl_off[round], F.n, M.fl_tot[round]);
    F.jarena = a.job_base;
    const int tags = fill_tags(a.in.tags);
    OutBuf &o = fl->o; o.n = 0; o.cap = line_out_cap(r.L, tags);
    o.w = (int32_t *)arena_alloc(cx, sizeof(int32_t) * (size_t)o.cap);
    r.rc_read = (uint8_t *)arena_alloc(cx, (size_t)r.L + 16);
    const LineBufs b = line_bufs(cx, r.L, 1, tags);
    LineRes *la = b.la;
    int n_reg = 0;
    if (o.w && r.rc_read && la) {
        const bool ok = fill_line(r, F, line, *la, b.cur_buf, b.cur_cap, b.rec_buf, b.rec_cap);
        if (!ok && !(cx.status & (ST_REFEXIT | ST_OVERFLOW))) cx.status |= ST_OVERFLOW;
        if (ok) {
            out_line(cx, o, *la);
            if (round == 0 && la->tol_score >= 0) {
                Regs &G = fl->G; G.n = 0; G.m = 0;
                const size_t mark = arena_mark(cx.tmp);
                G.beg = (int32_t *)arena_alloc(cx, sizeof(int32_t) * 2 * HP_REC_MAX); G.end = G.beg ? G.beg + HP_REC_MAX : nullptr;
                G.rb = (RegB *)arena_alloc(cx, sizeof(RegB) * 2 * HP_REC_MAX); G.re = G.rb ? G.rb + HP_REC_MAX : nullptr;
                if (G.beg && G.rb) {
                    for (int k = 0; k <= la->cur_res_n; ++k) regs_push(r, G, HP_REC_MAX, la->rec[k]);
                    for (int k = 0; k < G.n; ++k) out_reg(cx, o, G, k);
                    n_reg = G.n;
                }
                arena_release(cx.tmp, mark);
            }
        }
    }
    if (!(cx.status & (ST_REFEXIT | ST_OVERFLOW))) {
        unsigned long long off = 0;
        if (wv::leader()) off = atomicAdd(&a.ctl->line_cursor, (unsigned long long)o.n);
        off = (unsigned long long)wv::uni64((long long)off);
        if ((int64_t)(off + (unsigned long long)o.n) <= a.line_cap) {
            wv::sync();
            out_copy((HP_G int32_t *)(a.line_base + off), (const HP_G int32_t *)o.w, o.n);
            U.out_off = (int64_t)off; U.out_len = o.n; U.n_reg = n_reg;
        } else cx.status |= ST_OVERFLOW;
    }
    PH_TADD(round == 0 ? 2 : 4);
    meta_flag(a, rd, r);
}

HP_FN void phase_fill(const PhaseArgs &a, int round, int u, int wave_slot, HP_L int32_t *lds)
{
    PH_FRAME_CTX(r);
    phase_fill(a, round, u, wave_slot, lds, r);
}

struct LjRec { int64_t qaddr, tk, slot; int32_t rd; uint16_t tlen; uint8_t qlen; int8_t type_comp; };
enum { LJ_NCLS = HP_LJ_QSMALL / 16, LJ_NBUCKET = 2 * LJ_NCLS };
HP_INL int lj_bucket_of(int type, int qlen)
{
    const int cls = (qlen > 0 ? qlen - 1 : 0) >> 4;
    return (type == 1 ? 0 : LJ_NCLS) + (LJ_NCLS - 1 - cls);
}

HP_NOINL void phase_filllist(const PhaseArgs &a, int round, int u, int wave_slot, HP_L int32_t *lds, ReadCtx &r)
{
    UnitRec &U = a.units[(size_t)round * a.unit_cap + u];
    const int rd = U.read, line = U.line;
    RdMeta &M = a.meta[rd];
    if (*(volatile int32_t *)&M.status & ST_DEAD) return;
    read_bind(r, a.P, a.ref, a.in, rd, a.slab + (size_t)wave_slot * a.slab_fill, a.slab_fill, lds, a.prof, 0);
    pers_bind(r, a, rd);
    const lamsa_hp_para *P = r.cx.P;
    const bool lane_ok = lj_params_ok(P) && a.lj_cap > 0, wave_ok = a.wj_cap > 0;
    if (!lane_ok && !wave_ok) return;
    FLines F;
    F.n = M.fl_n[round]; F.nfrag = M.fl_nfrag[round];
    flines_bind(F, a.fl_base + M.fl_off[round], F.n, M.fl_tot[round]);
    const int f0 = F.frag_off[line], nfr = F.frag_off[line + 1] - f0;
    const int p0 = F.fr_seed_off[f0], np = F.fr_seed_off[f0 + nfr] - p0;
    const int strand = r.h_strand[F.fr_seed[p0]];
    const int n_junc = (nfr - 1) + np, n_cand = n_junc + 2;
    r.flip = strand != 1;
    const int64_t rbase = a.in.read_off[rd];
    long long tb = 0;
    int32_t *frag_of = (int32_t *)arena_alloc(r.cx, sizeof(int32_t) * (size_t)(np + 1));
    if (!frag_of) { r.flip = false; return; }
    {
        HP_G int32_t *g_fo = (HP_G int32_t *)frag_of;
        const HP_G int32_t *g_so = (const HP_G int32_t *)F.fr_seed_off;
        for (int b0 = 0; b0 < nfr; b0 += 64) { WAVE_FOR(l) { const int f = f0 + b0 + l; if (b0 + l < nfr) { for (int q = g_so[f]; q < g_so[f + 1]; ++q) g_fo[q - p0] = f; } } }
        wv::sync();
    }
    long long *cand = (long long *)arena_alloc(r.cx, sizeof(long long) * 4 * (size_t)(n_cand + 64));
    if (!cand) { r.flip = false; return; }
    int n_lb[LJ_NBUCKET], n_wb[WJ_NBUCKET];
#pragma unroll
    for (int b = 0; b < LJ_NBUCKET; ++b) n_lb[b] = 0;
#pragma unroll
    for (int b = 0; b < WJ_NBUCKET; ++b) n_wb[b] = 0;
    for (int c0 = 0; c0 < n_cand; c0 += 64) {
        wv::Lane<int> ty, qo, ql, tl, qrev; wv::Lane<long long> tk, sl;
        WAVE_FOR(l) {
            const int c = c0 + l;
            int type = 0, qoff = 0, qlen = 0, tlen = 0, rev = 0; long long k0 = 0, slot = 0;
            if (c < nfr - 1) {
                const int jf = f0 + c;
                JGeo G; junction_geo(r, F, strand == 1 ? jf + 1 : jf, strand == 1 ? jf : jf + 1, G);
                if (G.cls == JC_MIS) { type = 1; qoff = G.qoff; qlen = G.s_qlen; tlen = G.tl; slot = (F.jt + GS_WORDS * jf) - a.fl_base; k0 = r.ref.seq_off[G.at1_chr - 1] + G.start0; }
            } else if (c < n_junc) {
                const int p = p0 + (c - (nfr - 1));
                const int lo = ((const HP_G int32_t *)frag_of)[p - p0];
                const int fb = F.fr_seed_off[lo], seed_n = F.fr_seed_off[lo + 1] - fb;
                const int ip = p - fb + (strand == 1 ? 1 : -1);
                GapGeo G;
                if (seed_n > 1 && ip >= 0 && ip < seed_n && gap_geo(r, strand == 1, F.fr_seed[fb + ip], F.fr_seed[p], G)) {
                    type = 2; qoff = G.qoff; qlen = G.qlen; tlen = G.tlen; slot = (F.gt + GS_WORDS * p) - a.fl_base; k0 = r.ref.seq_off[G.chr - 1] + G.start0;
                }
            } else if (c < n_cand && wave_ok) {
                const bool head = c == n_junc;
                EndGeo G;
                if (end_geo(r, F, line, strand, head, G) == EG_JOB && G.read_len > 0 && G.ref_len > 0 && G.read_start >= 0 && G.read_start + G.read_len <= r.L) {
                    type = head ? 3 : 4; qlen = G.read_len; tlen = G.ref_len; slot = (F.ht + ES_LINE * line + (head ? 0 : ES_WORDS)) - a.fl_base;
                    qoff = head ? G.read_start + G.read_len - 1 : G.read_start; rev = head;
                    k0 = r.ref.seq_off[G.chr - 1] + G.start0 + (head ? G.ref_len - 1 : 0);
                }
            }
            const bool small = type != 0 && type <= 2 && qlen <= HP_LJ_QSMALL && tlen <= HP_LJ_TSMALL;
            if (type != 0 && !(small ? lane_ok : wave_ok)) type = 0;
            if (type != 0 && !small) type |= 16;
            ty[l] = type; qo[l] = qoff; ql[l] = qlen; tl[l] = tlen; sl[l] = slot; tk[l] = k0; qrev[l] = rev;
        }
        WAVE_FOR(l) {
            const int c = c0 + l;
            if (c < n_cand) { HP_G int32_t *cw = (HP_G int32_t *)cand + 8 * (size_t)c; cw[0] = ty[l]; cw[1] = qo[l]; cw[2] = ql[l]; cw[3] = tl[l] | (qrev[l] << 30); *(HP_G long long *)(cw + 4) = tk[l]; *(HP_G long long *)(cw + 6) = sl[l]; }
        }
#pragma unroll
        for (int b = 0; b < LJ_NBUCKET; ++b) { wv::Lane<int> inb; WAVE_FOR(l) inb[l] = ty[l] != 0 && !(ty[l] & 16) && lj_bucket_of(ty[l], ql[l]) == b; n_lb[b] += __builtin_popcountll(wv::ballot(inb)); }
        { wv::Lane<int> wb; WAVE_FOR(l) wb[l] = (ty[l] & 16) ? wj_bucket_of(P, ty[l] & 15, ql[l], tl[l], wj_need(P, ty[l] & 15, ql[l], tl[l]) > (long long)a.slab_wj) : -1;
#pragma unroll
          for (int b = 0; b < WJ_NBUCKET; ++b) { wv::Lane<int> inb; WAVE_FOR(l) inb[l] = wb[l] == b; n_wb[b] += __builtin_popcountll(wv::ballot(inb)); } }
    }
    int n_l = 0, n_w = 0;
#pragma unroll
    for (int b = 0; b < LJ_NBUCKET; ++b) n_l += n_lb[b];
#pragma unroll
    for (int b = 0; b < WJ_NBUCKET; ++b) n_w += n_wb[b];
    if (n_l + n_w > 0) {
        wv::Lane<int> got;
        WAVE_FOR(l) {
            int v = 0, add = 0; int32_t *ctr = nullptr;
#pragma unroll
            for (int b = 0; b < LJ_NBUCKET; ++b) if (l == b) { add = n_lb[b]; ctr = &a.ctl->lj_bucket_n[round][b]; }
#pragma unroll
            for (int b = 0; b < WJ_NBUCKET; ++b) if (l == LJ_NBUCKET + b) { add = n_wb[b]; ctr = &a.ctl->wj_bucket_n[round][b]; }
            if (l == LJ_NBUCKET + WJ_NBUCKET) { add = n_l; ctr = &a.ctl->lj_n[round]; }
            if (l == LJ_NBUCKET + WJ_NBUCKET + 1) { add = n_w; ctr = &a.ctl->wj_n[round]; }
            if (ctr && add > 0) v = atomicAdd(ctr, add);
            got[l] = v;
        }
        int base_l = wv::bcast(got, LJ_NBUCKET + WJ_NBUCKET), base_w = wv::bcast(got, LJ_NBUCKET + WJ_NBUCKET + 1);
        bool ok_l = n_l > 0 && base_l + n_l <= a.lj_cap, ok_w = n_w > 0 && base_w + n_w <= a.wj_cap;
        int pos_lb[LJ_NBUCKET], pos_wb[WJ_NBUCKET];
#pragma unroll
        for (int b = 0; b < LJ_NBUCKET; ++b) { pos_lb[b] = wv::bcast(got, b); if (n_lb[b] > 0 && pos_lb[b] + n_lb[b] > a.lj_cap) ok_l = false; }
#pragma unroll
        for (int b = 0; b < WJ_NBUCKET; ++b) { pos_wb[b] = wv::bcast(got, LJ_NBUCKET + b); if (n_wb[b] > 0 && pos_wb[b] + n_wb[b] > a.wj_cap) ok_w = false; }
#pragma unroll
        for (int b = 0; b < LJ_NBUCKET; ++b) if (!ok_l && n_lb[b] > 0) { for (int k0 = 0; k0 < n_lb[b]; k0 += 64) { WAVE_FOR(l) { const int k = pos_lb[b] + k0 + l; if (k0 + l < n_lb[b] && k < a.lj_cap) a.lj_bucket[(size_t)b * a.lj_cap + k] = -1; } } }
#pragma unroll
        for (int b = 0; b < WJ_NBUCKET; ++b) if (!ok_w && n_wb[b] > 0) { for (int k0 = 0; k0 < n_wb[b]; k0 += 64) { WAVE_FOR(l) { const int k = pos_wb[b] + k0 + l; if (k0 + l < n_wb[b] && k < a.wj_cap) a.wj_bucket[(size_t)b * a.wj_cap + k] = -1; } } }
        wv::sync();
        for (int c0 = 0; c0 < n_cand && (ok_l || ok_w); c0 += 64) {
            wv::Lane<int> ty, qo, ql, tl, qrev; wv::Lane<long long> tk, sl;
            WAVE_FOR(l) {
                const int c = c0 + l;
                ty[l] = 0; qo[l] = 0; ql[l] = 0; tl[l] = 0; qrev[l] = 0; tk[l] = 0; sl[l] = 0;
                if (c < n_cand) { const HP_G int32_t *cw = (const HP_G int32_t *)cand + 8 * (size_t)c; ty[l] = cw[0]; qo[l] = cw[1]; ql[l] = cw[2]; tl[l] = cw[3] & 0x3fffffff; qrev[l] = (cw[3] >> 30) & 1; tk[l] = *(const HP_G long long *)(cw + 4); sl[l] = *(const HP_G long long *)(cw + 6); }
            }
            wv::Lane<int> has, big, tbl;
            WAVE_FOR(l) { has[l] = ok_l && ty[l] != 0 && !(ty[l] & 16); big[l] = ok_w && (ty[l] & 16) != 0; tbl[l] = (has[l] || big[l]) ? tl[l] : 0; }
            const unsigned long long m = wv::ballot(has), mw = wv::ballot(big);
            if (m) {
                wv::Lane<int> at;
                WAVE_FOR(l) {
                    at[l] = base_l + __builtin_popcountll(m & ((1ull << l) - 1));
                    if (has[l]) {
                        LjRec &J = a.ljobs[at[l]];
                        J.qaddr = strand == 1 ? rbase + qo[l] : rbase + (r.L - 1 - qo[l]);
                        J.tk = tk[l]; J.slot = sl[l]; J.rd = rd; J.qlen = (uint8_t)ql[l]; J.tlen = (uint16_t)tl[l]; J.type_comp = (int8_t)(ty[l] | (strand == 1 ? 0 : 16));
                    }
                }
                base_l += __builtin_popcountll(m);
#pragma unroll
                for (int b = 0; b < LJ_NBUCKET; ++b) {
                    wv::Lane<int> inb;
                    WAVE_FOR(l) inb[l] = has[l] && lj_bucket_of(ty[l], ql[l]) == b;
                    const unsigned long long mb = wv::ballot(inb);
                    if (!mb) continue;
                    WAVE_FOR(l) { if (inb[l]) a.lj_bucket[(size_t)b * a.lj_cap + pos_lb[b] + __builtin_popcountll(mb & ((1ull << l) - 1))] = at[l]; }
                    pos_lb[b] += __builtin_popcountll(mb);
                }
            }
            if (mw) {
                wv::Lane<int> at, bk;
                WAVE_FOR(l) {
                    at[l] = base_w + __builtin_popcountll(mw & ((1ull << l) - 1)); bk[l] = -1;
                    if (big[l]) {
                        const int type = ty[l] & 15;
                        WjRec &J = a.wjobs[at[l]];
                        const int back = qrev[l] ? 1 : 0, comp = strand == 1 ? 0 : 1;
                        J.qaddr = strand == 1 ? rbase + qo[l] : rbase + (r.L - 1 - qo[l]);
                        J.tk = tk[l]; J.slot = sl[l]; J.rd = rd; J.qlen = ql[l]; J.tlen = tl[l];
                        J.type_comp = type | (comp << 4) | ((back ^ comp) << 5) | (back << 6);
                        bk[l] = wj_bucket_of(P, type, ql[l], tl[l], wj_need(P, type, ql[l], tl[l]) > (long long)a.slab_wj);
                    }
                }
                base_w += __builtin_popcountll(mw);
#pragma unroll
                for (int b = 0; b < WJ_NBUCKET; ++b) {
                    wv::Lane<int> inb;
                    WAVE_FOR(l) inb[l] = bk[l] == b;
                    const unsigned long long mb = wv::ballot(inb);
                    if (!mb) continue;
                    WAVE_FOR(l) { if (inb[l]) a.wj_bucket[(size_t)b * a.wj_cap + pos_wb[b] + __builtin_popcountll(mb & ((1ull << l) - 1))] = at[l]; }
                    pos_wb[b] += __builtin_popcountll(mb);
                }
            }
            tb += wv::reduce_sum(tbl);
        }
    }
    r.flip = false;
    r.t_bases = tb;
    meta_flag(a, rd, r);
}

HP_FN void phase_filllist(const PhaseArgs &a, int round, int u, int wave_slot, HP_L int32_t *lds)
{
    PH_FRAME_CTX(r);
    phase_filllist(a, round, u, wave_slot, lds, r);
}

HP_INL int lj_queue_n(const PhaseArgs &a, int round, int b) { const int n = a.ctl->lj_bucket_n[round][b]; return n < a.lj_cap ? n : a.lj_cap; }
HP_INL int wj_queue_n(const PhaseArgs &a, int round, int b) { const int n = a.ctl->wj_bucket_n[round][b]; return n < a.wj_cap ? n : a.wj_cap; }

HP_INL void phase_filldp(const PhaseArgs &a, int round, int bucket, int off, int wave_slot, HP_L int32_t *lds, int qcap)
{
    const lamsa_hp_para *P = &a.P;
    const int n_in = lj_queue_n(a, round, bucket);
    const int cnt = n_in - off < 64 ? n_in - off : 64;
    char *slab = a.slab + (size_t)wave_slot * a.slab_fill;
    cig_t *cbuf = (cig_t *)slab;
    uint8_t *zbuf = (uint8_t *)(slab + sizeof(cig_t) * 3 * HP_LJ_CIG * 64);
    if (sizeof(cig_t) * 3 * HP_LJ_CIG * 64 + (size_t)qcap * HP_LJ_TSMALL * 64 + 64 > a.slab_fill) return;
    const int32_t *bq = a.lj_bucket + (size_t)bucket * a.lj_cap + off;
    wv::Lane<int> nw, rdl, cel; wv::Lane<long long> slotl;
    wv::sync();
    WAVE_FOR(l) {
        nw[l] = 0; rdl[l] = -1; cel[l] = 0; slotl[l] = 0;
        if (l < cnt && bq[l] >= 0) {
            const LjRec R = a.ljobs[bq[l]];
            LaneJob J;
            const int comp = (R.type_comp >> 4) & 1, type = R.type_comp & 15;
            J.q = (const HP_G uint8_t *)(a.in.read_seq + R.qaddr); J.qs = comp ? -1 : 1; J.qcomp = comp; J.qlen = R.qlen; J.pac = (const HP_G uint8_t *)a.ref.pac; J.tk = R.tk; J.ts = 1; J.tlen = R.tlen;
            J.z = (HP_G uint8_t *)zbuf; J.zl = l; J.zs = qcap; J.cells = 0; J.row = lds + l; J.qrow = (HP_L uint8_t *)(lds + (qcap + 2) * 64) + l; J.rev = 0;
            lj_stage_query(J);
            LCig out, Lc, Rc;
            out.c = cbuf + (size_t)l * 3 * HP_LJ_CIG; out.n = 0; Lc.c = out.c + HP_LJ_CIG; Lc.n = 0; Rc.c = Lc.c + HP_LJ_CIG; Rc.n = 0;
            if (type == 1) lj_bi_extend(P, J, 100, 100, Lc, Rc, out);
            else lj_global(P, J, P->del_gapo, P->del_gape, P->ins_gapo, P->ins_gape, P->band_w, &out);
            nw[l] = out.n; rdl[l] = R.rd; cel[l] = (int)J.cells; slotl[l] = R.slot | ((long long)R.tlen << 48);
        }
    }
    wv::Lane<int> pre = nw;
    wv::scan_add_excl(pre);
    const int total = wv::reduce_sum(nw);
    unsigned long long base = 0;
    if (wv::leader()) base = atomicAdd(&a.ctl->job_cursor, (unsigned long long)total);
    base = (unsigned long long)wv::uni64((long long)base);
    if ((int64_t)(base + (unsigned long long)total) > a.job_cap) return;
    WAVE_FOR(l) {
        if (l < cnt && bq[l] >= 0) {
            const cig_t *src = cbuf + (size_t)l * 3 * HP_LJ_CIG;
            int32_t *dst = a.job_base + base + pre[l];
            for (int k = 0; k < nw[l]; ++k) dst[k] = src[k];
            int32_t *slot = a.fl_base + (slotl[l] & 0xffffffffffffll);
            slot[GS_OFF] = (int32_t)(base + pre[l]); slot[GS_N] = nw[l]; slot[GS_TLEN] = (int32_t)(slotl[l] >> 48); slot[GS_HAS] = 1;
            if (cel[l] > 0) atomicAdd(&a.meta[rdl[l]].cells, cel[l]);
        }
    }
    wv::sync();
}

#ifdef HP_WJ_NOINL
HP_NOINL
#else
HP_INL
#endif
void phase_wavejob(const PhaseArgs &a, int round, int g, bool big, int wave_slot, HP_L int32_t *lds)
{
    const int b1 = big ? WJ_NBIG : WJ_NBUCKET;
    int b = big ? 0 : WJ_NBIG;
    for (; b < b1 - 1; ++b) { const int nb = wj_queue_n(a, round, b); if (g < nb) break; g -= nb; }
    const int ji = wv::uni(a.wj_bucket[(size_t)b * a.wj_cap + g]);
    if (ji < 0) return;
    const WjRec R = a.wjobs[ji];
    const int rd = wv::uni(R.rd), type = wv::uni(R.type_comp) & 15, comp = (wv::uni(R.type_comp) >> 4) & 1;
    const int qs = (wv::uni(R.type_comp) >> 5) & 1 ? -1 : 1, ts = (wv::uni(R.type_comp) >> 6) & 1 ? -1 : 1;
    const int qlen = wv::uni(R.qlen), tlen = wv::uni(R.tlen);
    if (*(volatile int32_t *)&a.meta[rd].status & ST_DEAD) return;
    Ctx cx;
    cx.P = &a.P; cx.lds = lds; cx.lds_words = HP_WJ_LDS_WORDS; cx.status = 0; cx.n_cells = 0; cx.lds_epoch = 0; cx.prof = a.prof ? a.prof + (size_t)rd * 64 : nullptr;
    cx.prof_dp = a.prof ? a.prof + ((size_t)a.n_reads + 1 + rd) * 64 : nullptr;
    if (big) arena_init(cx.tmp, a.slab + a.wjb_off + (size_t)wave_slot * a.slab_wjb, a.slab_wjb);
    else arena_init(cx.tmp, a.slab + (size_t)wave_slot * a.slab_wj, a.slab_wj);
    CigV out;
    if (!cig_alloc(cx, out, qlen + tlen + 64)) return;
    WjOut o;
    const lamsa_hp_para *P = &a.P;
    const bool ok = wj_run(cx, a.in.read_seq, a.ref.pac, type, comp, wv::uni64(R.qaddr), qs, qlen, wv::uni64(R.tk), ts, tlen,
                           P->band_w, type == WJ_BI ? 100 : P->seed_len * P->match, out, o);
    if (cx.n_cells > 0 && wv::leader()) { atomicAdd(&a.meta[rd].cells, (int)(cx.n_cells > 0x3fffffffLL ? 0x3fffffffLL : cx.n_cells)); atomicAdd(&a.ctl->wj_cells, (unsigned long long)cx.n_cells); }
    if (!ok) return;
    unsigned long long base = 0;
    if (wv::leader()) base = atomicAdd(&a.ctl->job_cursor, (unsigned long long)out.n);
    base = (unsigned long long)wv::uni64((long long)base);
    if ((int64_t)(base + (unsigned long long)out.n) > a.job_cap) return;
    {
        HP_G int32_t *dst = (HP_G int32_t *)(a.job_base + base);
        const HP_G cig_t *src = (const HP_G cig_t *)out.c;
        for (int b0 = 0; b0 < out.n; b0 += 64) { WAVE_FOR(l) { const int i = b0 + l; if (i < out.n) dst[i] = src[i]; } }
        HP_G int32_t *slot = (HP_G int32_t *)(a.fl_base + wv::uni64(R.slot));
        WAVE_FOR(l) {
            if (type == WJ_BI || type == WJ_GLOBAL) { if (l < GS_WORDS) slot[l] = l == GS_OFF ? (int32_t)base : (l == GS_N ? out.n : (l == GS_TLEN ? tlen : 1)); }
            else if (l < ES_WORDS) slot[l] = l == ES_OFF ? (int32_t)base : (l == ES_N ? out.n : (l == ES_REFLEN ? o.reflen : (l == ES_READLEN ? o.readlen : (l == ES_HAS ? 1 : 0))));
        }
    }
    if (wv::leader()) atomicAdd(&a.ctl->wj_bytes, (unsigned long long)(qlen + (tlen + 3) / 4 + 4 * out.n + 32));
    HP_STAT(9);
    wv::sync();
}

HP_NOINL void phase_chain2(const PhaseArgs &a, int rd, int wave_slot, HP_L int32_t *lds, int lds_words, ReadCtx &r)
{
    RdMeta &M = a.meta[rd];
    if (M.status & ST_DEAD) return;
    PH_T0();
    read_bind(r, a.P, a.ref, a.in, rd, a.slab + (size_t)wave_slot * a.slab_per_wave + PH_CTX_BYTES, a.slab_per_wave - PH_CTX_BYTES, lds, a.prof, lds_words);
    pers_bind(r, a, rd);
    Ctx &cx = r.cx;
    const int H = r.H, c = H + 1;
    ChainOut *co = (ChainOut *)arena_alloc(cx, sizeof(ChainOut));
    Regs *gp = (Regs *)arena_alloc(cx, sizeof(Regs));
    if (!co || !gp) { meta_flag(a, rd, r); return; }
    int32_t *nm = (int32_t *)arena_alloc(cx, sizeof(int32_t) * 10 * (size_t)c);
    const int reg_cap = 256;
    Regs &G = *gp; G.n = 0; G.m = 0;
    G.beg = (int32_t *)arena_alloc(cx, sizeof(int32_t) * 2 * (size_t)reg_cap); G.end = G.beg + reg_cap;
    G.rb = (RegB *)arena_alloc(cx, sizeof(RegB) * 2 * (size_t)reg_cap); G.re = G.rb + reg_cap;
    G.r_beg = (int32_t *)arena_alloc(cx, sizeof(int32_t) * 6 * (size_t)(reg_cap + 2));
    G.r_end = G.r_beg + (reg_cap + 2); G.r_bs = G.r_end + (reg_cap + 2); G.r_bn = G.r_bs + (reg_cap + 2); G.r_es = G.r_bn + (reg_cap + 2); G.r_en = G.r_es + (reg_cap + 2);
    if (nm && G.beg && G.rb && G.r_beg) {
        aux_bind(r, nm);
        for (int j = 0; j < M.fl_n[0]; ++j) {
            const UnitRec &U = a.units[M.unit_base[0] + j];
            const int32_t *w = a.line_base + U.out_off + (U.out_len - PH_REG_WORDS * U.n_reg);
            for (int k = 0; k < U.n_reg; ++k, w += PH_REG_WORDS) {
                if (G.n >= reg_cap) { cx.status |= ST_OVERFLOW; break; }
                reg_read(w, G, G.n++);
            }
        }
        wv::sync();
        if (!(cx.status & ST_OVERFLOW)) {
            regs_remain(r, G, a.P.seed_len, r.L);
            FLines &F = co->F;
            FlStore &fs = co->fs; fs.base = a.fl_base; fs.cap = a.fl_cap; fs.cursor = &a.ctl->fl_cursor; fs.got_off = 0; fs.got_tot = 0;
            const bool ok2 = chain_remain(r, G, F, &fs);
            if (ok2 && F.n > 0) units_push(a, r, rd, 1, F, fs);
            else if (!ok2 && !(cx.status & (ST_REFEXIT | ST_OVERFLOW))) cx.status |= ST_OVERFLOW;
        }
    }
    PH_TADD(3);
    meta_flag(a, rd, r);
}

HP_FN void phase_chain2(const PhaseArgs &a, int rd, int wave_slot, HP_L int32_t *lds, int lds_words = HP_CHAIN_LDS_WORDS)
{
    ReadCtx r;
    phase_chain2(a, rd, wave_slot, lds, lds_words, r);
}

HP_NOINL void phase_publish(const PhaseArgs &a, int rd)
{
    const RdMeta &M = a.meta[rd];
    const int st = M.status;
    const bool dead = (st & ST_DEAD) != 0;
    int n_words = 3;
    if (!dead)
        for (int round = 0; round < 2; ++round)
            for (int j = 0; j < M.fl_n[round]; ++j) { const UnitRec &U = a.units[(size_t)round * a.unit_cap + M.unit_base[round] + j]; n_words += U.out_len - PH_REG_WORDS * U.n_reg; }
    unsigned long long off = 0;
    if (wv::leader()) off = atomicAdd(a.out.cursor, (unsigned long long)n_words);
    off = (unsigned long long)wv::uni64((long long)off);
    if ((int64_t)(off + (unsigned long long)n_words) <= a.out.stream_cap) {
        HP_G int32_t *dst = (HP_G int32_t *)(a.out.stream + off);
        dst[0] = st; dst[1] = dead ? 0 : M.fl_n[0]; dst[2] = dead ? 0 : M.fl_n[1];
        int at = 3;
        if (!dead)
            for (int round = 0; round < 2; ++round)
                for (int j = 0; j < M.fl_n[round]; ++j) {
                    const UnitRec &U = a.units[(size_t)round * a.unit_cap + M.unit_base[round] + j];
                    const int n = U.out_len - PH_REG_WORDS * U.n_reg;
                    out_copy(dst + at, (const HP_G int32_t *)(a.line_base + U.out_off), n);
                    at += n;
                }
        a.out.read_out_off[rd] = (int64_t)off; a.out.read_out_len[rd] = n_words;
    } else { a.out.read_out_off[rd] = -1; a.out.read_out_len[rd] = 0; }
    a.out.read_status[rd] = st;
    if (a.out.read_tbases) a.out.read_tbases[rd] = M.tbases;
    if (a.out.read_work) { a.out.read_work[4 * rd] = M.cells; a.out.read_work[4 * rd + 1] = M.pairs; a.out.read_work[4 * rd + 2] = M.cs_words; a.out.read_work[4 * rd + 3] = 0; }
}

HP_INL void publish_diag(const PhaseArgs &a)
{
    if (a.out.diag && wv::leader()) {
        for (int k = 0; k < 4; ++k) { a.out.diag[2 * k] = ~a.ctl->t_first_inv[k]; a.out.diag[2 * k + 1] = a.ctl->t_last[k]; }
        a.out.diag[8] = (unsigned long long)a.ctl->n_units[0]; a.out.diag[9] = (unsigned long long)a.ctl->n_units[1];
        a.out.diag[10] = a.ctl->fl_cursor; a.out.diag[11] = a.ctl->line_cursor;
        a.out.diag[12] = (unsigned long long)(a.ctl->wj_n[0] + a.ctl->wj_n[1]); a.out.diag[13] = a.ctl->wj_bytes; a.out.diag[14] = (unsigned long long)(a.ctl->lj_n[0] + a.ctl->lj_n[1]);
        a.out.diag[15] = a.ctl->job_cursor; a.out.diag[16] = a.ctl->wj_cells;
    }
}

}
```

Measured before the change: 4.342.

## Split lane DP bi-extend jobs into two stages with deferred re-bucketing

Lane-DP jobs now run in two kernels. The first stage runs only the left extension of bi-extend jobs and finishes the ones that reach an end. Jobs that need more work are re-bucketed into new queues and handled by a second kernel, either as global DP or as the full bi-extend. The aim is to cut SIMD divergence, where a few long lanes hold up a whole wave of 64. In exchange it adds an extra kernel launch, queue atomics, and recomputation for deferred jobs.

```diff
diff --git a/lamsa_amd/csrc/hp_align_api.hip b/lamsa_amd/csrc/hp_align_api.hip
--- a/lamsa_amd/csrc/hp_align_api.hip
+++ b/lamsa_amd/csrc/hp_align_api.hip
@@ -118,22 +118,31 @@
         phase_filllist(a, round, u, blockIdx.x, (HP_L int32_t *)lds, r);
     }
 }
+template <int MODE>
 __global__ __launch_bounds__(64, 2) void k_filldp_small(const PhaseArgs *ap, int round)
 {
     __shared__ int32_t lds[HP_LJ_LDS_WORDS(HP_LJ_QSMALL)];
     const PhaseArgs &a = *ap;
+    constexpr int b0 = MODE == LJ_STAGE2 ? LJ_NORD : 0, b1 = MODE == LJ_STAGE2 ? LJ_NBUCKET : LJ_NORD, head = MODE == LJ_STAGE2 ? 9 : 6;
     int n = 0;
-    for (int b = 0; b < LJ_NBUCKET; ++b) n += (lj_queue_n(a, round, b) + 63) >> 6;
+    for (int b = b0; b < b1; ++b) n += (lj_queue_n(a, round, b) + 63) >> 6;
     n = wv::uni(n);
     for (;;) {
         int g = 0;
-        if (wv::leader()) g = atomicAdd(&a.ctl->q_head[6], 1);
+        if (wv::leader()) g = atomicAdd(&a.ctl->q_head[head], 1);
         g = wv::uni(g);
         if (g >= n) break;
-        int b = 0;
-        for (; b < LJ_NBUCKET - 1; ++b) { const int gb = (lj_queue_n(a, round, b) + 63) >> 6; if (g < gb) break; g -= gb; }
-        phase_filldp(a, round, b, g * 64, blockIdx.x, (HP_L int32_t *)lds, HP_LJ_QSMALL);
-    }
+        int b = b0;
+        for (; b < b1 - 1; ++b) { const int gb = (lj_queue_n(a, round, b) + 63) >> 6; if (g < gb) break; g -= gb; }
+        if (MODE == LJ_STAGE2 && b < LJ_NORD + LJ_NCLS) phase_filldp_run<LJ_STAGE2G>(a, round, b, g * 64, blockIdx.x, (HP_L int32_t *)lds, HP_LJ_QSMALL);
+        else phase_filldp_run<MODE>(a, round, b, g * 64, blockIdx.x, (HP_L int32_t *)lds, HP_LJ_QSMALL);
+    }
+}
+static void launch_filldp(bool stages, int w_dp, hipStream_t s, const PhaseArgs *da, int round)
+{
+    if (!stages) { hipLaunchKernelGGL(k_filldp_small<LJ_ONE>, dim3(w_dp), dim3(64), 0, s, da, round); return; }
+    hipLaunchKernelGGL(k_filldp_small<LJ_STAGE1>, dim3(w_dp), dim3(64), 0, s, da, round);
+    hipLaunchKernelGGL(k_filldp_small<LJ_STAGE2>, dim3(w_dp), dim3(64), 0, s, da, round);
 }
 __global__ __launch_bounds__(64, HP_WJ_WAVES_PER_SIMD) void k_filldp_wave(const PhaseArgs *ap, int round)
 {
@@ -219,6 +228,7 @@
 static const bool g_noshare = getenv("LAMSA_HP_FULL_GRIDS") != nullptr;
 static const bool g_nowave = getenv("LAMSA_HP_NO_WAVE_JOBS") != nullptr;
 static const bool g_nolane = getenv("LAMSA_HP_NO_LANE_DP") != nullptr;
+static const bool g_lane_stages = !(getenv("LAMSA_HP_LANE_STAGES") && atoi(getenv("LAMSA_HP_LANE_STAGES")) == 0);
 static const bool g_mono = getenv("LAMSA_HP_ONE_KERNEL") != nullptr;
 
 struct HostBuf {
@@ -263,6 +273,9 @@
     hipStream_t cs = nullptr;
     bool valid = false;
     bool phased = false;
+#ifdef HP_LJ_STATS
+    const PhaseCtl *ctl_dev = nullptr;
+#endif
     int32_t n_reads = 0; int64_t n_bases = 0, n_cig = 0, n_hits = 0;
     BatchIn in; const int32_t *d_order = nullptr;
     std::vector<int32_t> order, h_len, h_H; std::vector<uint8_t> h_skip;
@@ -543,7 +556,7 @@
     int pc = 0, pf = 0, pd = 0, pw = 0;
     if (hipOccupancyMaxActiveBlocksPerMultiprocessor(&pc, g_chain_shapes[shape].k1, 64, 0) != hipSuccess || pc < 1) pc = 4 * g_chain_shapes[shape].waves_per_simd;
     if (hipOccupancyMaxActiveBlocksPerMultiprocessor(&pf, k_fill, 64, 0) != hipSuccess || pf < 1) pf = 4;
-    if (hipOccupancyMaxActiveBlocksPerMultiprocessor(&pd, k_filldp_small, 64, 0) != hipSuccess || pd < 1) pd = 4;
+    if (hipOccupancyMaxActiveBlocksPerMultiprocessor(&pd, g_lane_stages ? k_filldp_small<LJ_STAGE2> : k_filldp_small<LJ_ONE>, 64, 0) != hipSuccess || pd < 1) pd = 4;
     if (hipOccupancyMaxActiveBlocksPerMultiprocessor(&pw, k_filldp_wave, 64, 0) != hipSuccess || pw < 1) pw = 4;
     if (shared && !g_noshare) { pc = std::min(pc, 8); pf = std::min(pf, 16); pw = std::min(pw, 16); }
     { static const int cf = getenv("LAMSA_HP_FILL_PER_CU") ? atoi(getenv("LAMSA_HP_FILL_PER_CU")) : 0, cc = getenv("LAMSA_HP_CHAIN_PER_CU") ? atoi(getenv("LAMSA_HP_CHAIN_PER_CU")) : 0,
@@ -598,6 +611,7 @@
     if (Ln.args_host.ensure(sizeof a)) { h->err = "hipHostMalloc(args)"; return LAMSA_HP_ENOMEM; }
     memcpy(Ln.args_host.p, &a, sizeof a);
     HIPCHK(h, hipMemcpyAsync(d + o_args, Ln.args_host.p, sizeof a, hipMemcpyHostToDevice, s), LAMSA_HP_EKERNEL);
+    if (!g_lane_stages) HIPCHK(h, hipMemsetAsync(&((PhaseCtl *)(d + o_ctl))->lj_one_stage, 1, 4, s), LAMSA_HP_EKERNEL);
     const PhaseArgs *da = (const PhaseArgs *)(d + o_args);
     HIPCHK(h, hipEventRecord(e0, s), LAMSA_HP_EKERNEL);
     hipLaunchKernelGGL(g_chain_shapes[Q.shape].k1, dim3(std::min(w_chain, n)), dim3(64), 0, s, da);
@@ -607,7 +621,7 @@
         HIPCHK(h, hipEventRecord(Ln.ep[5], s), LAMSA_HP_EKERNEL);
         if (!g_nowave) hipLaunchKernelGGL(k_filldp_wave, dim3(w_wj), dim3(64), 0, s, da, 0);
         HIPCHK(h, hipEventRecord(Ln.ep[6], s), LAMSA_HP_EKERNEL);
-        if (!g_nolane) hipLaunchKernelGGL(k_filldp_small, dim3(w_dp), dim3(64), 0, s, da, 0);
+        if (!g_nolane) launch_filldp(g_lane_stages, w_dp, s, da, 0);
     } else { HIPCHK(h, hipEventRecord(Ln.ep[5], s), LAMSA_HP_EKERNEL); HIPCHK(h, hipEventRecord(Ln.ep[6], s), LAMSA_HP_EKERNEL); }
     HIPCHK(h, hipEventRecord(Ln.ep[4], s), LAMSA_HP_EKERNEL);
     hipLaunchKernelGGL(k_fill, dim3(w_fill), dim3(64), 0, s, da, 0);
@@ -615,10 +629,10 @@
     hipLaunchKernelGGL(g_chain_shapes[Q.shape].k2, dim3(std::min(w_chain, n)), dim3(64), 0, s, da);
     HIPCHK(h, hipEventRecord(Ln.ep[2], s), LAMSA_HP_EKERNEL);
     if (list) {
-        HIPCHK(h, hipMemsetAsync(&((PhaseCtl *)(d + o_ctl))->q_head[5], 0, 16, s), LAMSA_HP_EKERNEL);
+        HIPCHK(h, hipMemsetAsync(&((PhaseCtl *)(d + o_ctl))->q_head[5], 0, 20, s), LAMSA_HP_EKERNEL);
         hipLaunchKernelGGL(k_filllist, dim3(w_fill), dim3(64), 0, s, da, 1);
         if (!g_nowave) hipLaunchKernelGGL(k_filldp_wave, dim3(w_wj), dim3(64), 0, s, da, 1);
-        if (!g_nolane) hipLaunchKernelGGL(k_filldp_small, dim3(w_dp), dim3(64), 0, s, da, 1);
+        if (!g_nolane) launch_filldp(g_lane_stages, w_dp, s, da, 1);
     }
     hipLaunchKernelGGL(k_fill, dim3(w_fill), dim3(64), 0, s, da, 1);
     HIPCHK(h, hipEventRecord(Ln.ep[3], s), LAMSA_HP_EKERNEL);
@@ -626,6 +640,9 @@
     HIPCHK(h, hipGetLastError(), LAMSA_HP_EKERNEL);
     HIPCHK(h, hipEventRecord(e1, s), LAMSA_HP_EKERNEL);
     Ln.phased = true;
+#ifdef HP_LJ_STATS
+    Ln.ctl_dev = (const PhaseCtl *)(d + o_ctl);
+#endif
     return LAMSA_HP_OK;
 }
 
@@ -713,6 +730,16 @@
 #ifdef HP_PROF
         prof_report(T, (const long long *)Ln.prof.p, n);
 #endif
+#ifdef HP_LJ_STATS
+        if (Ln.ctl_dev) {
+            unsigned long long v[LJS_N];
+            if (hipMemcpy(v, Ln.ctl_dev->lj_stat, sizeof v, hipMemcpyDeviceToHost) == hipSuccess) {
+                fprintf(stderr, "lj_stats stages=%d", g_lane_stages ? 1 : 0);
+                for (int k = 0; k < LJS_N; ++k) fprintf(stderr, " %llu", v[k]);
+                fprintf(stderr, "\n");
+            }
+        }
+#endif
     }
     memcpy(S->r_off.data(), Ln.out1.h_off(), 8 * (size_t)n); memcpy(S->r_len.data(), Ln.out1.h_len(n), 4 * (size_t)n);
     memcpy(S->r_st.data(), Ln.out1.h_st(n), 4 * (size_t)n); memcpy(S->r_tb.data(), Ln.out1.h_tb(n), 4 * (size_t)n); memcpy(S->r_work.data(), Ln.out1.h_work(n), 16 * (size_t)n);
@@ -893,3 +920,87 @@
     h->result_tags = flags;
     return LAMSA_HP_OK;
 }
+
+extern "C" int lamsa_hp_dp_batch_staged_(lamsa_hp_handle *h, const lamsa_hp_dp_jobs *J, lamsa_hp_dp_out *O)
+{
+    const int n = J->n_jobs;
+    if (!lj_params_ok(&h->para)) { h->err = "the handle's penalties do not keep the lane routines' 16-bit cells exact"; return LAMSA_HP_EINVAL; }
+    int64_t tot = 0;
+    for (int i = 0; i < n; ++i) {
+        if (J->kind[i] != 12 && J->kind[i] != 13) { h->err = "dp batch mixes job classes"; return LAMSA_HP_EINVAL; }
+        if (J->qlen[i] < 1 || J->qlen[i] > HP_LJ_QSMALL || J->tlen[i] < 0 || J->tlen[i] > HP_LJ_TSMALL) { h->err = "dp job beyond the lane routines' buffers"; return LAMSA_HP_EINVAL; }
+        if (J->q_off[i] < 0 || J->t_off[i] < 0 || J->q_off[i] + J->qlen[i] > J->seq_bytes || J->t_off[i] + J->tlen[i] > J->seq_bytes) { h->err = "dp job sequence out of range"; return LAMSA_HP_EINVAL; }
+        tot += J->tlen[i];
+    }
+    const int lj_cap = n + 1;
+    std::vector<uint8_t> pac((size_t)tot / 4 + 16, 0);
+    std::vector<LjRec> ljv((size_t)lj_cap); std::vector<int32_t> ljq((size_t)LJ_NBUCKET * lj_cap, -1);
+    PhaseCtl ctl; memset((void *)&ctl, 0, sizeof ctl);
+    ctl.lj_one_stage = g_lane_stages ? 0 : 1;
+    int64_t k = 0;
+    for (int i = 0; i < n; ++i) {
+        LjRec &R = ljv[i];
+        const int type = J->kind[i] - 11;
+        R.qaddr = J->q_off[i]; R.tk = k; R.slot = (int64_t)GS_WORDS * i; R.rd = i; R.tlen = (uint16_t)J->tlen[i]; R.qlen = (uint8_t)J->qlen[i]; R.type_comp = (int8_t)type;
+        for (int j = 0; j < J->tlen[i]; ++j, ++k) {
+            const uint8_t b = J->seq[J->t_off[i] + j];
+            if (b > 3) { h->err = "these routines read the target 2 bits per base: no N"; return LAMSA_HP_EINVAL; }
+            pac[(size_t)(k >> 2)] |= (uint8_t)(b << ((~k & 3) << 1));
+        }
+        const int b = lj_bucket_of(type, J->qlen[i]);
+        ljq[(size_t)b * lj_cap + ctl.lj_bucket_n[0][b]++] = i;
+        ++ctl.lj_n[0];
+    }
+    HIPCHK(h, hipSetDevice(h->device), LAMSA_HP_ENODEV);
+    const size_t slab_fill = al256(sizeof(cig_t) * 3 * HP_LJ_CIG * 64 + (size_t)HP_LJ_QSMALL * HP_LJ_TSMALL * 64 + 64);
+    const int w_dp = std::max(1, std::min((n + 63) / 64, h->n_cu * 2));
+    const int64_t job_cap = (int64_t)n * HP_LJ_CIG + 64;
+    size_t off = 0;
+    auto place = [&](size_t bytes) { size_t o = off; off = al256(off + bytes + 16); return o; };
+    const size_t o_args = place(sizeof(PhaseArgs)), o_ctl = place(sizeof(PhaseCtl)), o_meta = place(sizeof(RdMeta) * ((size_t)n + 1)), o_seq = place((size_t)J->seq_bytes), o_pac = place(pac.size()),
+                 o_lj = place(sizeof(LjRec) * (size_t)lj_cap), o_lq = place(4 * ljq.size()), o_fl = place(4 * (size_t)GS_WORDS * ((size_t)n + 1)), o_jb = place(4 * (size_t)job_cap), o_slab = place(slab_fill * (size_t)w_dp);
+    if (h->in.ensure(off)) { h->err = "hipMalloc(in)"; return LAMSA_HP_ENOMEM; }
+    char *d = (char *)h->in.p;
+    hipStream_t s = h->stream;
+    PhaseArgs a; memset((void *)&a, 0, sizeof a);
+    a.P = h->para; a.ctl = (PhaseCtl *)(d + o_ctl); a.in.read_seq = (const uint8_t *)(d + o_seq); a.ref.pac = (const uint8_t *)(d + o_pac); a.meta = (RdMeta *)(d + o_meta);
+    a.ljobs = (LjRec *)(d + o_lj); a.lj_bucket = (int32_t *)(d + o_lq); a.lj_cap = lj_cap; a.fl_base = (int32_t *)(d + o_fl); a.job_base = (int32_t *)(d + o_jb); a.job_cap = job_cap;
+    a.slab = d + o_slab; a.slab_fill = slab_fill; a.n_reads = n;
+    HIPCHK(h, hipMemsetAsync(d, 0, o_slab, s), LAMSA_HP_EKERNEL);
+    HIPCHK(h, hipMemcpyAsync(d + o_args, &a, sizeof a, hipMemcpyHostToDevice, s), LAMSA_HP_EKERNEL);
+    HIPCHK(h, hipMemcpyAsync(d + o_ctl, &ctl, sizeof ctl, hipMemcpyHostToDevice, s), LAMSA_HP_EKERNEL);
+    if (J->seq_bytes > 0) HIPCHK(h, hipMemcpyAsync(d + o_seq, J->seq, (size_t)J->seq_bytes, hipMemcpyHostToDevice, s), LAMSA_HP_EKERNEL);
+    HIPCHK(h, hipMemcpyAsync(d + o_pac, pac.data(), pac.size(), hipMemcpyHostToDevice, s), LAMSA_HP_EKERNEL);
+    HIPCHK(h, hipMemcpyAsync(d + o_lj, ljv.data(), sizeof(LjRec) * ljv.size(), hipMemcpyHostToDevice, s), LAMSA_HP_EKERNEL);
+    HIPCHK(h, hipMemcpyAsync(d + o_lq, ljq.data(), 4 * ljq.size(), hipMemcpyHostToDevice, s), LAMSA_HP_EKERNEL);
+    HIPCHK(h, hipStreamSynchronize(s), LAMSA_HP_EKERNEL);
+    HIPCHK(h, hipEventRecord(h->ev0, s), LAMSA_HP_EKERNEL);
+    if (n > 0) launch_filldp(g_lane_stages, w_dp, s, (const PhaseArgs *)(d + o_args), 0);
+    HIPCHK(h, hipGetLastError(), LAMSA_HP_EKERNEL);
+    HIPCHK(h, hipEventRecord(h->ev1, s), LAMSA_HP_EKERNEL);
+    std::vector<int32_t> fl((size_t)GS_WORDS * ((size_t)n + 1)), jobs((size_t)job_cap); std::vector<RdMeta> meta((size_t)n + 1);
+    HIPCHK(h, hipMemcpyAsync(fl.data(), d + o_fl, 4 * fl.size(), hipMemcpyDeviceToHost, s), LAMSA_HP_EKERNEL);
+    HIPCHK(h, hipMemcpyAsync(jobs.data(), d + o_jb, 4 * jobs.size(), hipMemcpyDeviceToHost, s), LAMSA_HP_EKERNEL);
+    HIPCHK(h, hipMemcpyAsync((void *)meta.data(), d + o_meta, sizeof(RdMeta) * meta.size(), hipMemcpyDeviceToHost, s), LAMSA_HP_EKERNEL);
+    HIPCHK(h, hipMemcpyAsync(ljq.data(), d + o_lq, 4 * ljq.size(), hipMemcpyDeviceToHost, s), LAMSA_HP_EKERNEL);
+    HIPCHK(h, hipMemcpyAsync(&ctl, d + o_ctl, sizeof ctl, hipMemcpyDeviceToHost, s), LAMSA_HP_EKERNEL);
+    HIPCHK(h, hipStreamSynchronize(s), LAMSA_HP_EKERNEL);
+    hipEventElapsedTime(&h->kernel_ms[0], h->ev0, h->ev1);
+    h->h_score.assign((size_t)n, 0); h->h_qle.assign((size_t)n, 0); h->h_tle.assign((size_t)n, 0); h->h_status.assign((size_t)n, 0);
+    h->h_i64.assign((size_t)n + 1, 0); h->h_cig.clear();
+    for (int i = 0; i < n; ++i) {
+        const int32_t *slot = fl.data() + (size_t)GS_WORDS * i;
+        h->h_i64[i] = (int64_t)h->h_cig.size();
+        h->h_qle[i] = meta[i].cells; h->h_status[i] = slot[GS_HAS] ? 0 : 1;
+        if (slot[GS_HAS] && slot[GS_OFF] >= 0 && slot[GS_N] >= 0 && (int64_t)slot[GS_OFF] + slot[GS_N] <= job_cap) h->h_cig.insert(h->h_cig.end(), jobs.begin() + slot[GS_OFF], jobs.begin() + slot[GS_OFF] + slot[GS_N]);
+    }
+    h->h_i64[n] = (int64_t)h->h_cig.size();
+    for (int b = LJ_NORD; b < LJ_NBUCKET; ++b) {
+        const int nq = std::min(ctl.lj_bucket_n[0][b], lj_cap);
+        for (int q = 0; q < nq; ++q) { const int i = ljq[(size_t)b * lj_cap + q]; if (i >= 0 && i < n) h->h_tle[i] = 1; }
+    }
+    if (h->h_cig.empty()) h->h_cig.push_back(0);
+    O->score = h->h_score.data(); O->qle = h->h_qle.data(); O->tle = h->h_tle.data(); O->status = h->h_status.data();
+    O->cig_off = h->h_i64.data(); O->cigar = h->h_cig.data();
+    return LAMSA_HP_OK;
+}
diff --git a/lamsa_amd/csrc/hp_api.hip b/lamsa_amd/csrc/hp_api.hip
--- a/lamsa_amd/csrc/hp_api.hip
+++ b/lamsa_amd/csrc/hp_api.hip
@@ -132,11 +132,13 @@
 extern "C" float lamsa_hp_last_kernel_ms(const lamsa_hp_handle *h, int which) { return (h && which >= 0 && which < 24) ? h->kernel_ms[which] : -1.f; }
 
 
+extern "C" int lamsa_hp_dp_batch_staged_(lamsa_hp_handle *h, const lamsa_hp_dp_jobs *J, lamsa_hp_dp_out *O);
 extern "C" int lamsa_hp_dp_batch(lamsa_hp_handle *h, const lamsa_hp_dp_jobs *J, lamsa_hp_dp_out *O)
 {
     if (!h || !J || !O || J->n_jobs < 0) return LAMSA_HP_EINVAL;
     HIPCHK(h, hipSetDevice(h->device), LAMSA_HP_ENODEV);
     const int n = J->n_jobs;
+    if (n > 0 && J->kind[0] >= 12) return lamsa_hp_dp_batch_staged_(h, J, O);
     std::vector<int64_t> cap_off((size_t)n + 1, 0);
     size_t z_need = 4096;
     for (int i = 0; i < n; ++i) {
diff --git a/lamsa_amd/csrc/hp_core.h b/lamsa_amd/csrc/hp_core.h
--- a/lamsa_amd/csrc/hp_core.h
+++ b/lamsa_amd/csrc/hp_core.h
@@ -73,7 +73,7 @@
 #define HP_STAT_MAX(i, v) ((void)0)
 #endif
 #ifdef HP_STAT_SLOTS
-static_assert(HP_STAT_SLOTS >= 97, "the array of the path counters ends before the last slot the device sources use");
+static_assert(HP_STAT_SLOTS >= 108, "the array of the path counters ends before the last slot the device sources use");
 #define HP_STATX_ADD(i, n) HP_STAT_ADD(i, n)
 #define HP_STATX_MAX(i, v) HP_STAT_MAX(i, v)
 #else
diff --git a/lamsa_amd/csrc/hp_lanedp.h b/lamsa_amd/csrc/hp_lanedp.h
--- a/lamsa_amd/csrc/hp_lanedp.h
+++ b/lamsa_amd/csrc/hp_lanedp.h
@@ -11,6 +11,12 @@
 #define HP_LJ_LDS_WORDS(qcap) (((qcap) + 2) * 64 + ((qcap) + 2) * 16)
 #define HP_LJ_NEG (-20000)
 
+#ifdef HP_LJ_STATS
+#define LJ_PASS(J, k, n) ((J).pc[k] = (int)(n))
+#else
+#define LJ_PASS(J, k, n) ((void)(n))
+#endif
+
 struct LCig { cig_t *c; int n; };
 HP_INL void lc_push0(LCig &v, cig_t w) { if (v.n > 0 && (v.c[v.n - 1] & 0xf) == (w & 0xf)) v.c[v.n - 1] += (w >> 4) << 4; else v.c[v.n++] = w; }
 HP_INL void lc_push1(LCig &v, cig_t w) { if ((w >> 4) != 0) lc_push0(v, w); }
@@ -34,6 +40,10 @@
     HP_L int32_t *row; HP_L uint8_t *qrow;
     int rev;
     long long cells;
+    int exit;
+#ifdef HP_LJ_STATS
+    int pc[5];
+#endif
 };
 HP_INL int lj_qbase(const LaneJob &J, int j) { const int c = J.q[(long)j * J.qs]; return J.qcomp ? (c < 4 ? 3 - c : 4) : c; }
 HP_INL int lj_t(const LaneJob &J, int i) { const int64_t k = J.tk + (int64_t)i * J.ts; return J.pac[k >> 2] >> ((~k & 3) << 1) & 3; }
@@ -214,35 +224,55 @@
     return max;
 }
 
+enum { LJ_X_LEFT = 0, LJ_X_LEFT_GLOBAL, LJ_X_RIGHT, LJ_X_RIGHT_GLOBAL, LJ_X_MID_SH, LJ_X_MID_GLOBAL, LJ_X_MORE };
+
+HP_INL int lj_bi_left(const lamsa_hp_para *P, LaneJob &J, int lh0, LCig &L, LCig &out, int *lqe, int *lte)
+{
+    const int qlen = J.qlen, tlen = J.tlen;
+    out.n = 0; L.n = 0;
+    const int w = iabs(qlen - tlen) + 3 > P->band_w ? iabs(qlen - tlen) + 3 : P->band_w;
+    const long long c0 = J.cells;
+    LJ_PASS(J, 1, 0); LJ_PASS(J, 2, 0); LJ_PASS(J, 3, 0); LJ_PASS(J, 4, 0);
+    lj_extend(P, J, w, lh0, lqe, lte, &L);
+    LJ_PASS(J, 0, J.cells - c0);
+    const int res = *lqe == qlen ? 0 : (*lte == tlen ? 1 : 2);
+    if (res == 2) { J.exit = LJ_X_MORE; return LJ_X_MORE; }
+    lc_pushv(out, L.c, L.n);
+    lc_push1(out, res == 0 ? ((tlen - *lte) << 4) | C_D : ((qlen - *lqe) << 4) | C_I);
+    J.exit = LJ_X_LEFT; HP_STATX_ADD(99, 1);
+    return LJ_X_LEFT;
+}
+
 HP_INL int lj_bi_extend(const lamsa_hp_para *P, LaneJob &J, int lh0, int rh0, LCig &L, LCig &R, LCig &out)
 {
     const int qlen = J.qlen, tlen = J.tlen;
     int res, lqe, lte, rqe, rte;
-    out.n = 0; L.n = 0; R.n = 0;
+    R.n = 0;
     const int w = iabs(qlen - tlen) + 3 > P->band_w ? iabs(qlen - tlen) + 3 : P->band_w;
-    lj_extend(P, J, w, lh0, &lqe, &lte, &L);
-    res = lqe == qlen ? 0 : (lte == tlen ? 1 : 2);
-    if (res < 2) {
-        lc_pushv(out, L.c, L.n);
-        lc_push1(out, res == 0 ? ((tlen - lte) << 4) | C_D : ((qlen - lqe) << 4) | C_I);
-        return 0;
-    }
+    if (lj_bi_left(P, J, lh0, L, out, &lqe, &lte) == LJ_X_LEFT) return 0;
+    const long long c1 = J.cells;
     if (bi_near_diag(P, qlen, tlen) && ((lqe << 1 > qlen) || (lte << 1 > tlen))) {
         lj_global(P, J, P->del_gapo, P->del_gape, P->ins_gapo, P->ins_gape, P->band_w, &out);
+        LJ_PASS(J, 1, J.cells - c1);
+        J.exit = LJ_X_LEFT_GLOBAL; HP_STATX_ADD(100, 1);
         return 0;
     }
     LaneJob Rj = lj_rev(J);
     lj_extend(P, Rj, w, rh0, &rqe, &rte, &R);
+    LJ_PASS(J, 2, Rj.cells - c1);
     J.cells = Rj.cells;
     res = rqe == qlen ? 0 : (rte == tlen ? 1 : 2);
     if (res < 2) {
         lc_push1(R, res == 0 ? ((tlen - rte) << 4) | C_D : ((qlen - rqe) << 4) | C_I);
         lc_invert(R);
         lc_pushv(out, R.c, R.n);
+        J.exit = LJ_X_RIGHT; HP_STATX_ADD(101, 1);
         return 0;
     }
     if (bi_near_diag(P, qlen, tlen) && ((rqe << 1 > qlen) || (rte << 1 > tlen))) {
         lj_global(P, J, P->del_gapo, P->del_gape, P->ins_gapo, P->ins_gape, P->band_w, &out);
+        LJ_PASS(J, 3, J.cells - Rj.cells);
+        J.exit = LJ_X_RIGHT_GLOBAL; HP_STATX_ADD(102, 1);
         return 0;
     }
     lc_invert(R);
@@ -253,10 +283,13 @@
             lc_push0(out, (cig_t)((uint32_t)Sn << 4) | C_S);
             lc_push0(out, (cig_t)((uint32_t)Hn << 4) | C_H);
             lc_pushv(out, R.c, R.n);
+            J.exit = LJ_X_MID_SH; HP_STATX_ADD(103, 1);
         } else {
             LCig g; g.c = L.c; g.n = 0;
             lj_global(P, J, P->del_gapo, P->del_gape, P->ins_gapo, P->ins_gape, P->band_w, &g);
+            LJ_PASS(J, 4, J.cells - Rj.cells);
             lc_pushv(out, g.c, g.n);
+            J.exit = LJ_X_MID_GLOBAL; HP_STATX_ADD(104, 1);
         }
     }
     return (qlen - lqe - rqe) >= P->split_len ? 1 : 0;
diff --git a/lamsa_amd/csrc/hp_phase.h b/lamsa_amd/csrc/hp_phase.h
--- a/lamsa_amd/csrc/hp_phase.h
+++ b/lamsa_amd/csrc/hp_phase.h
@@ -23,11 +23,14 @@
 };
 
 enum { PH_NBUCKET = 8 };
+enum { LJS_T1 = 0, LJS_T2, LJS_EXIT0, LJS_GROUPS = LJS_EXIT0 + 6, LJS_GPASS1, LJS_LP_EXEC = LJS_GPASS1 + 5, LJS_LP_NEED, LJS_THIN_PASSES, LJS_PASSES, LJS_THIN_CELLS, LJS_PASS_CELLS,
+       LJS_T2_PASS_CELLS, LJS_CELLS, LJS_TLEN_SUM, LJS_TLEN_RANGE, LJS_TLEN_MAXSUM, LJS_DEFERRED, LJS_STAGE2, LJS_HARD_FULL, LJS_N };
 
 struct alignas(128) PhaseCtl {
     alignas(128) int32_t q_head[12];
     alignas(128) int32_t n_units[2];
     int32_t bucket_n[2][PH_NBUCKET];
+    int32_t lj_one_stage;
     alignas(128) unsigned long long fl_cursor;
     alignas(128) unsigned long long line_cursor;
     alignas(128) unsigned long long job_cursor;
@@ -36,6 +39,9 @@
     alignas(128) unsigned long long wj_bytes;
     alignas(128) unsigned long long wj_cells;
     alignas(128) unsigned long long t_first_inv[4], t_last[4];
+#ifdef HP_LJ_STATS
+    alignas(128) unsigned long long lj_stat[LJS_N];
+#endif
 };
 
 struct LjRec;
@@ -257,8 +263,9 @@
 }
 
 struct LjRec { int64_t qaddr, tk, slot; int32_t rd; uint16_t tlen; uint8_t qlen; int8_t type_comp; };
-enum { LJ_NCLS = HP_LJ_QSMALL / 16, LJ_NBUCKET = 2 * LJ_NCLS };
-HP_INL int lj_bucket_of(int type, int qlen)
+enum { LJ_NCLS = HP_LJ_QSMALL / 16, LJ_NORD = 2 * LJ_NCLS, LJ_NBUCKET = LJ_NORD + 2 * LJ_NCLS };
+static_assert(LJ_NBUCKET <= 24, "PhaseCtl::lj_bucket_n has 24 queues per round");
+HP_HD int lj_bucket_of(int type, int qlen)
 {
     const int cls = (qlen > 0 ? qlen - 1 : 0) >> 4;
     return (type == 1 ? 0 : LJ_NCLS) + (LJ_NCLS - 1 - cls);
@@ -295,9 +302,9 @@
     }
     long long *cand = (long long *)arena_alloc(r.cx, sizeof(long long) * 4 * (size_t)(n_cand + 64));
     if (!cand) { r.flip = false; return; }
-    int n_lb[LJ_NBUCKET], n_wb[WJ_NBUCKET];
-#pragma unroll
-    for (int b = 0; b < LJ_NBUCKET; ++b) n_lb[b] = 0;
+    int n_lb[LJ_NORD], n_wb[WJ_NBUCKET];
+#pragma unroll
+    for (int b = 0; b < LJ_NORD; ++b) n_lb[b] = 0;
 #pragma unroll
     for (int b = 0; b < WJ_NBUCKET; ++b) n_wb[b] = 0;
     for (int c0 = 0; c0 < n_cand; c0 += 64) {
@@ -337,14 +344,14 @@
             if (c < n_cand) { HP_G int32_t *cw = (HP_G int32_t *)cand + 8 * (size_t)c; cw[0] = ty[l]; cw[1] = qo[l]; cw[2] = ql[l]; cw[3] = tl[l] | (qrev[l] << 30); *(HP_G long long *)(cw + 4) = tk[l]; *(HP_G long long *)(cw + 6) = sl[l]; }
         }
 #pragma unroll
-        for (int b = 0; b < LJ_NBUCKET; ++b) { wv::Lane<int> inb; WAVE_FOR(l) inb[l] = ty[l] != 0 && !(ty[l] & 16) && lj_bucket_of(ty[l], ql[l]) == b; n_lb[b] += __builtin_popcountll(wv::ballot(inb)); }
+        for (int b = 0; b < LJ_NORD; ++b) { wv::Lane<int> inb; WAVE_FOR(l) inb[l] = ty[l] != 0 && !(ty[l] & 16) && lj_bucket_of(ty[l], ql[l]) == b; n_lb[b] += __builtin_popcountll(wv::ballot(inb)); }
         { wv::Lane<int> wb; WAVE_FOR(l) wb[l] = (ty[l] & 16) ? wj_bucket_of(P, ty[l] & 15, ql[l], tl[l], wj_need(P, ty[l] & 15, ql[l], tl[l]) > (long long)a.slab_wj) : -1;
 #pragma unroll
           for (int b = 0; b < WJ_NBUCKET; ++b) { wv::Lane<int> inb; WAVE_FOR(l) inb[l] = wb[l] == b; n_wb[b] += __builtin_popcountll(wv::ballot(inb)); } }
     }
     int n_l = 0, n_w = 0;
 #pragma unroll
-    for (int b = 0; b < LJ_NBUCKET; ++b) n_l += n_lb[b];
+    for (int b = 0; b < LJ_NORD; ++b) n_l += n_lb[b];
 #pragma unroll
     for (int b = 0; b < WJ_NBUCKET; ++b) n_w += n_wb[b];
     if (n_l + n_w > 0) {
@@ -352,23 +359,23 @@
         WAVE_FOR(l) {
             int v = 0, add = 0; int32_t *ctr = nullptr;
 #pragma unroll
-            for (int b = 0; b < LJ_NBUCKET; ++b) if (l == b) { add = n_lb[b]; ctr = &a.ctl->lj_bucket_n[round][b]; }
-#pragma unroll
-            for (int b = 0; b < WJ_NBUCKET; ++b) if (l == LJ_NBUCKET + b) { add = n_wb[b]; ctr = &a.ctl->wj_bucket_n[round][b]; }
-            if (l == LJ_NBUCKET + WJ_NBUCKET) { add = n_l; ctr = &a.ctl->lj_n[round]; }
-            if (l == LJ_NBUCKET + WJ_NBUCKET + 1) { add = n_w; ctr = &a.ctl->wj_n[round]; }
+            for (int b = 0; b < LJ_NORD; ++b) if (l == b) { add = n_lb[b]; ctr = &a.ctl->lj_bucket_n[round][b]; }
+#pragma unroll
+            for (int b = 0; b < WJ_NBUCKET; ++b) if (l == LJ_NORD + b) { add = n_wb[b]; ctr = &a.ctl->wj_bucket_n[round][b]; }
+            if (l == LJ_NORD + WJ_NBUCKET) { add = n_l; ctr = &a.ctl->lj_n[round]; }
+            if (l == LJ_NORD + WJ_NBUCKET + 1) { add = n_w; ctr = &a.ctl->wj_n[round]; }
             if (ctr && add > 0) v = atomicAdd(ctr, add);
             got[l] = v;
         }
-        int base_l = wv::bcast(got, LJ_NBUCKET + WJ_NBUCKET), base_w = wv::bcast(got, LJ_NBUCKET + WJ_NBUCKET + 1);
+        int base_l = wv::bcast(got, LJ_NORD + WJ_NBUCKET), base_w = wv::bcast(got, LJ_NORD + WJ_NBUCKET + 1);
         bool ok_l = n_l > 0 && base_l + n_l <= a.lj_cap, ok_w = n_w > 0 && base_w + n_w <= a.wj_cap;
-        int pos_lb[LJ_NBUCKET], pos_wb[WJ_NBUCKET];
-#pragma unroll
-        for (int b = 0; b < LJ_NBUCKET; ++b) { pos_lb[b] = wv::bcast(got, b); if (n_lb[b] > 0 && pos_lb[b] + n_lb[b] > a.lj_cap) ok_l = false; }
-#pragma unroll
-        for (int b = 0; b < WJ_NBUCKET; ++b) { pos_wb[b] = wv::bcast(got, LJ_NBUCKET + b); if (n_wb[b] > 0 && pos_wb[b] + n_wb[b] > a.wj_cap) ok_w = false; }
-#pragma unroll
-        for (int b = 0; b < LJ_NBUCKET; ++b) if (!ok_l && n_lb[b] > 0) { for (int k0 = 0; k0 < n_lb[b]; k0 += 64) { WAVE_FOR(l) { const int k = pos_lb[b] + k0 + l; if (k0 + l < n_lb[b] && k < a.lj_cap) a.lj_bucket[(size_t)b * a.lj_cap + k] = -1; } } }
+        int pos_lb[LJ_NORD], pos_wb[WJ_NBUCKET];
+#pragma unroll
+        for (int b = 0; b < LJ_NORD; ++b) { pos_lb[b] = wv::bcast(got, b); if (n_lb[b] > 0 && pos_lb[b] + n_lb[b] > a.lj_cap) ok_l = false; }
+#pragma unroll
+        for (int b = 0; b < WJ_NBUCKET; ++b) { pos_wb[b] = wv::bcast(got, LJ_NORD + b); if (n_wb[b] > 0 && pos_wb[b] + n_wb[b] > a.wj_cap) ok_w = false; }
+#pragma unroll
+        for (int b = 0; b < LJ_NORD; ++b) if (!ok_l && n_lb[b] > 0) { for (int k0 = 0; k0 < n_lb[b]; k0 += 64) { WAVE_FOR(l) { const int k = pos_lb[b] + k0 + l; if (k0 + l < n_lb[b] && k < a.lj_cap) a.lj_bucket[(size_t)b * a.lj_cap + k] = -1; } } }
 #pragma unroll
         for (int b = 0; b < WJ_NBUCKET; ++b) if (!ok_w && n_wb[b] > 0) { for (int k0 = 0; k0 < n_wb[b]; k0 += 64) { WAVE_FOR(l) { const int k = pos_wb[b] + k0 + l; if (k0 + l < n_wb[b] && k < a.wj_cap) a.wj_bucket[(size_t)b * a.wj_cap + k] = -1; } } }
         wv::sync();
@@ -394,7 +401,7 @@
                 }
                 base_l += __builtin_popcountll(m);
 #pragma unroll
-                for (int b = 0; b < LJ_NBUCKET; ++b) {
+                for (int b = 0; b < LJ_NORD; ++b) {
                     wv::Lane<int> inb;
                     WAVE_FOR(l) inb[l] = has[l] && lj_bucket_of(ty[l], ql[l]) == b;
                     const unsigned long long mb = wv::ballot(inb);
@@ -442,10 +449,50 @@
     phase_filllist(a, round, u, wave_slot, lds, r);
 }
 
-HP_INL int lj_queue_n(const PhaseArgs &a, int round, int b) { const int n = a.ctl->lj_bucket_n[round][b]; return n < a.lj_cap ? n : a.lj_cap; }
+#ifndef HP_LJ_HARD_CAP_RT
+#define HP_LJ_HARD_CAP_RT(cap) (cap)
+#endif
+HP_INL int lj_queue_n(const PhaseArgs &a, int round, int b) { const int n = a.ctl->lj_bucket_n[round][b], cap = b < LJ_NORD ? a.lj_cap : HP_LJ_HARD_CAP_RT(a.lj_cap); return n < cap ? n : cap; }
 HP_INL int wj_queue_n(const PhaseArgs &a, int round, int b) { const int n = a.ctl->wj_bucket_n[round][b]; return n < a.wj_cap ? n : a.wj_cap; }
 
-HP_INL void phase_filldp(const PhaseArgs &a, int round, int bucket, int off, int wave_slot, HP_L int32_t *lds, int qcap)
+enum { LJ_ONE = 0, LJ_STAGE1 = 1, LJ_STAGE2 = 2, LJ_STAGE2G = 3 };
+#ifdef HP_LJ_STATS
+template <int MODE>
+HP_INL void lj_stats_group(const PhaseArgs &a, const wv::Lane<int> &ex, const wv::Lane<int> &tl, const wv::Lane<int> (&pc)[5], const wv::Lane<int> &more)
+{
+    unsigned long long add[LJS_N];
+    for (int k = 0; k < LJS_N; ++k) add[k] = 0;
+    wv::Lane<int> t;
+    WAVE_FOR(l) t[l] = ex[l] != -1;
+    const int n_act = __builtin_popcountll(wv::ballot(t));
+    if (!n_act) return;
+    WAVE_FOR(l) t[l] = ex[l] == -2;
+    const int n2 = __builtin_popcountll(wv::ballot(t));
+    if (MODE == LJ_ONE || MODE == LJ_STAGE1) { add[LJS_T1] = n_act - n2; add[LJS_T2] = n2; } else add[LJS_STAGE2] = n_act;
+    for (int e = 0; e < 6; ++e) { WAVE_FOR(l) t[l] = ex[l] == e; add[LJS_EXIT0 + e] = __builtin_popcountll(wv::ballot(t)); }
+    add[LJS_DEFERRED] = __builtin_popcountll(wv::ballot(more));
+    for (int k = 0; k < 5; ++k) add[LJS_CELLS] += (unsigned long long)wv::reduce_sum(pc[k]);
+    if (n2 == 0) {
+        int passes = 0;
+        for (int k = 0; k < 5; ++k) {
+            WAVE_FOR(l) t[l] = pc[k][l] > 0;
+            const int n_k = __builtin_popcountll(wv::ballot(t)), mx = wv::reduce_max(pc[k]);
+            if (!n_k) continue;
+            ++passes; add[LJS_LP_NEED] += n_k; add[LJS_PASSES] += 1; add[LJS_PASS_CELLS] += mx;
+            if (n_k < 16) { add[LJS_THIN_PASSES] += 1; add[LJS_THIN_CELLS] += mx; }
+        }
+        if (passes) { add[LJS_GROUPS] = 1; add[LJS_GPASS1 + passes - 1] = 1; add[LJS_LP_EXEC] = 64 * passes; }
+        WAVE_FOR(l) t[l] = tl[l] < 0 ? 0 : tl[l];
+        const int mx = wv::reduce_max(t), sum = wv::reduce_sum(t);
+        WAVE_FOR(l) t[l] = tl[l] < 0 ? -100000 : -tl[l];
+        const int mn = -wv::reduce_max(t);
+        add[LJS_TLEN_SUM] = sum; add[LJS_TLEN_RANGE] = mx - mn; add[LJS_TLEN_MAXSUM] = mx;
+    } else add[LJS_T2_PASS_CELLS] = wv::reduce_max(pc[0]);
+    if (wv::leader()) { for (int k = 0; k < LJS_N; ++k) if (add[k]) atomicAdd(&a.ctl->lj_stat[k], add[k]); }
+}
+#endif
+template <int MODE>
+HP_INL void phase_filldp_run(const PhaseArgs &a, int round, int bucket, int off, int wave_slot, HP_L int32_t *lds, int qcap)
 {
     const lamsa_hp_para *P = &a.P;
     const int n_in = lj_queue_n(a, round, bucket);
@@ -455,24 +502,72 @@
     uint8_t *zbuf = (uint8_t *)(slab + sizeof(cig_t) * 3 * HP_LJ_CIG * 64);
     if (sizeof(cig_t) * 3 * HP_LJ_CIG * 64 + (size_t)qcap * HP_LJ_TSMALL * 64 + 64 > a.slab_fill) return;
     const int32_t *bq = a.lj_bucket + (size_t)bucket * a.lj_cap + off;
-    wv::Lane<int> nw, rdl, cel; wv::Lane<long long> slotl;
+    wv::Lane<int> nw, rdl, cel, more; wv::Lane<long long> slotl;
+#ifdef HP_LJ_STATS
+    wv::Lane<int> s_ex, s_tl, s_pc[5];
+#endif
     wv::sync();
     WAVE_FOR(l) {
-        nw[l] = 0; rdl[l] = -1; cel[l] = 0; slotl[l] = 0;
+        nw[l] = 0; rdl[l] = -1; cel[l] = 0; slotl[l] = 0; more[l] = 0;
+#ifdef HP_LJ_STATS
+        s_ex[l] = -1; s_tl[l] = -1; for (int k = 0; k < 5; ++k) s_pc[k][l] = 0;
+#endif
         if (l < cnt && bq[l] >= 0) {
             const LjRec R = a.ljobs[bq[l]];
             LaneJob J;
             const int comp = (R.type_comp >> 4) & 1, type = R.type_comp & 15;
             J.q = (const HP_G uint8_t *)(a.in.read_seq + R.qaddr); J.qs = comp ? -1 : 1; J.qcomp = comp; J.qlen = R.qlen; J.pac = (const HP_G uint8_t *)a.ref.pac; J.tk = R.tk; J.ts = 1; J.tlen = R.tlen;
-            J.z = (HP_G uint8_t *)zbuf; J.zl = l; J.zs = qcap; J.cells = 0; J.row = lds + l; J.qrow = (HP_L uint8_t *)(lds + (qcap + 2) * 64) + l; J.rev = 0;
+            J.z = (HP_G uint8_t *)zbuf; J.zl = l; J.zs = qcap; J.cells = 0; J.row = lds + l; J.qrow = (HP_L uint8_t *)(lds + (qcap + 2) * 64) + l; J.rev = 0; J.exit = -1;
             lj_stage_query(J);
             LCig out, Lc, Rc;
             out.c = cbuf + (size_t)l * 3 * HP_LJ_CIG; out.n = 0; Lc.c = out.c + HP_LJ_CIG; Lc.n = 0; Rc.c = Lc.c + HP_LJ_CIG; Rc.n = 0;
-            if (type == 1) lj_bi_extend(P, J, 100, 100, Lc, Rc, out);
-            else lj_global(P, J, P->del_gapo, P->del_gape, P->ins_gapo, P->ins_gape, P->band_w, &out);
-            nw[l] = out.n; rdl[l] = R.rd; cel[l] = (int)J.cells; slotl[l] = R.slot | ((long long)R.tlen << 48);
-        }
-    }
+            if (MODE == LJ_ONE || MODE == LJ_STAGE1) HP_STATX_ADD(type == 1 ? 97 : 98, 1);
+            else HP_STATX_ADD(106, 1);
+            if (MODE == LJ_STAGE2G) {
+                J.cells = a.fl_base[R.slot + GS_N];
+                const long long c0 = J.cells;
+                LJ_PASS(J, 0, 0); LJ_PASS(J, 2, 0); LJ_PASS(J, 3, 0); LJ_PASS(J, 4, 0);
+                lj_global(P, J, P->del_gapo, P->del_gape, P->ins_gapo, P->ins_gape, P->band_w, &out);
+                LJ_PASS(J, 1, J.cells - c0);
+                J.exit = LJ_X_LEFT_GLOBAL; HP_STATX_ADD(100, 1);
+            } else if (type != 1) lj_global(P, J, P->del_gapo, P->del_gape, P->ins_gapo, P->ins_gape, P->band_w, &out);
+            else if (MODE == LJ_STAGE1) {
+                int lqe, lte;
+                if (lj_bi_left(P, J, 100, Lc, out, &lqe, &lte) == LJ_X_MORE) more[l] = bi_near_diag(P, J.qlen, J.tlen) && ((lqe << 1 > J.qlen) || (lte << 1 > J.tlen)) ? 1 : 2;
+            } else lj_bi_extend(P, J, 100, 100, Lc, Rc, out);
+            nw[l] = more[l] ? 0 : out.n; cel[l] = (int)J.cells;
+            rdl[l] = R.rd; slotl[l] = R.slot | ((long long)R.tlen << 48);
+#ifdef HP_LJ_STATS
+            s_ex[l] = type == 1 ? J.exit : -2; s_tl[l] = R.tlen; for (int k = 0; k < 5; ++k) s_pc[k][l] = type == 1 ? J.pc[k] : (k == 0 ? (int)J.cells : 0);
+#endif
+        }
+    }
+    if (MODE == LJ_STAGE1) {
+        for (int kind = 1; kind <= 2 && bucket < LJ_NCLS; ++kind) {
+            wv::Lane<int> mk;
+            WAVE_FOR(l) mk[l] = more[l] == kind;
+            const unsigned long long mm = wv::ballot(mk);
+            if (!mm) continue;
+            const int hb = LJ_NORD + (kind - 1) * LJ_NCLS + bucket, n_more = __builtin_popcountll(mm), hcap = HP_LJ_HARD_CAP_RT(a.lj_cap);
+            int pos = 0;
+            if (wv::leader()) pos = atomicAdd(&a.ctl->lj_bucket_n[round][hb], n_more);
+            pos = wv::uni(pos);
+            WAVE_FOR(l) {
+                if (mk[l]) {
+                    const int k = pos + __builtin_popcountll(mm & ((1ull << l) - 1));
+                    if (k < hcap) { a.lj_bucket[(size_t)hb * a.lj_cap + k] = bq[l]; if (kind == 1) a.fl_base[(slotl[l] & 0xffffffffffffll) + GS_N] = cel[l]; }
+                }
+            }
+            HP_STATX_ADD(105, n_more);
+            HP_STATX_ADD(107, pos + n_more > hcap ? (pos < hcap ? pos + n_more - hcap : n_more) : 0);
+#ifdef HP_LJ_STATS
+            if (wv::leader() && pos + n_more > hcap) atomicAdd(&a.ctl->lj_stat[LJS_HARD_FULL], (unsigned long long)(pos < hcap ? pos + n_more - hcap : n_more));
+#endif
+        }
+    }
+#ifdef HP_LJ_STATS
+    lj_stats_group<MODE>(a, s_ex, s_tl, s_pc, more);
+#endif
     wv::Lane<int> pre = nw;
     wv::scan_add_excl(pre);
     const int total = wv::reduce_sum(nw);
@@ -481,7 +576,7 @@
     base = (unsigned long long)wv::uni64((long long)base);
     if ((int64_t)(base + (unsigned long long)total) > a.job_cap) return;
     WAVE_FOR(l) {
-        if (l < cnt && bq[l] >= 0) {
+        if (l < cnt && bq[l] >= 0 && !more[l]) {
             const cig_t *src = cbuf + (size_t)l * 3 * HP_LJ_CIG;
             int32_t *dst = a.job_base + base + pre[l];
             for (int k = 0; k < nw[l]; ++k) dst[k] = src[k];
@@ -491,6 +586,14 @@
         }
     }
     wv::sync();
+}
+
+HP_INL void phase_filldp(const PhaseArgs &a, int round, int bucket, int off, int wave_slot, HP_L int32_t *lds, int qcap)
+{
+    if (a.ctl->lj_one_stage) phase_filldp_run<LJ_ONE>(a, round, bucket, off, wave_slot, lds, qcap);
+    else if (bucket < LJ_NORD) phase_filldp_run<LJ_STAGE1>(a, round, bucket, off, wave_slot, lds, qcap);
+    else if (bucket < LJ_NORD + LJ_NCLS) phase_filldp_run<LJ_STAGE2G>(a, round, bucket, off, wave_slot, lds, qcap);
+    else phase_filldp_run<LJ_STAGE2>(a, round, bucket, off, wave_slot, lds, qcap);
 }
 
 #ifdef HP_WJ_NOINL
```

Result: faster. 4.446, median of 6 (+2.4%).
